# bdaiinstitute/vlfm

Hardware: AMD Instinct MI355X
Metric: env-steps/s (VLM+value-map update), 640x480 RGB-D (higher is better)
Workload: dtype f16 ViT-g (f32 accumulate) + f32 Q-Former (split-f16, 22-bit); f32 confidence + f64 value maps; 1 GPU; configs[1] step x resident envs: BLIP-2 ITC + ValueMap+ObstacleMap+sort_waypoints; envs_per_gpu=256, global_envs=256, map=1000x1000 @ 20 px/m, parallelism=env-sharded x1, tuned_gemms=True, vit_gemm=hip:fc1, attention=hip

## Files before the change

include/vlfm_amd.h:

```cpp
#ifndef VLFM_AMD_H
#define VLFM_AMD_H

#include <stddef.h>
#include <stdint.h>

#ifdef __cplusplus
extern "C" {
#endif

typedef enum {
    VLFM_OK = 0,
    VLFM_ERR_INVALID = -1,
    VLFM_ERR_OUTSIDE_MAP = -2,
    VLFM_ERR_INDEX = -3,
    VLFM_ERR_HIP = -4,
    VLFM_ERR_CAPACITY = -5
} vlfm_status;

enum { VLFM_FUSE_DEFAULT = 0, VLFM_FUSE_REPLACE = 1, VLFM_FUSE_EQUAL_WEIGHTING = 2 };

const char* vlfm_last_error(void);
int vlfm_abi_version(void);

int vlfm_profile_enable(int on);
int vlfm_profile_read(const char* kernel_name, double* mean_ms, int* launches);

int vlfm_host_wait_mode(int blocking);

typedef struct {
    double inv_affine[6];
    int32_t row0, col0;
    int32_t env;
    int32_t reserved;
} vlfm_vm_pose;

int vlfm_value_map_pose_params(const double* h_tf, const double* h_yaw, const int32_t* h_env, int n, int map_size,
                               int pixels_per_meter, int template_size, vlfm_vm_pose* h_out, int* bad_index);

int vlfm_cone_template_host(double fov, double max_depth, int pixels_per_meter, double min_confidence,
                            float* h_conf, int conf_capacity, int64_t* h_poly_xy, int poly_capacity,
                            int* n_poly);

int vlfm_tan_table_host(double fov, int width, double* h_out);

int vlfm_cone_template_build(const float* d_conf, const int64_t* d_poly_xy, int n_poly, int template_size,
                             float* d_template, uint32_t* d_template_bits, void* stream);

typedef struct {
    double tf[12];
    float depth_scale;
    float depth_offset;
    float depth_max;
    float reserved0;
    double fx, fy;
    double min_height, max_height;
    int32_t env;
    int32_t scatter;
} vlfm_ingest_params;

typedef struct {
    uint32_t* d_cells;
    int32_t* d_count;
    int32_t capacity;
    int32_t reserved;
} vlfm_scatter_journal;

int vlfm_depth_ingest_batched(const float* d_depth, int n, int height, int width,
                              const vlfm_ingest_params* d_params,
                              uint32_t* d_colmax_keys ,
                              uint32_t* d_obstacle , int map_size, int pixels_per_meter,
                              int32_t* d_status ,
                              uint32_t* d_hole_bits ,
                              const uint32_t* d_filled_bits ,
                              const vlfm_scatter_journal* journal ,
                              void* stream);

int vlfm_selftest_div_exact(const double* d_numerators, int n, double divisor, int32_t* d_mismatches, void* stream);

size_t vlfm_hole_scratch_bytes(int n, int height, int width, int cap_pts, int cap_contours);
int vlfm_fill_small_holes_batched(const uint32_t* d_hole_bits, const int32_t* d_status, int n, int height, int width,
                                  double area_thresh, void* d_scratch, size_t scratch_bytes, int cap_pts,
                                  int cap_contours, uint32_t* d_filled_bits, int32_t* d_counts,
                                  const vlfm_ingest_params* d_params, uint32_t* d_obstacle, int map_size,
                                  const vlfm_scatter_journal* journal, void* stream);
int vlfm_depth_scatter_holes_batched(const vlfm_ingest_params* d_params, int n, int height, int width,
                                     const uint32_t* d_hole_bits, const uint32_t* d_filled_bits,
                                     const int32_t* d_hole_counts ,
                                     uint32_t* d_obstacle, int map_size, int pixels_per_meter, int32_t* d_status,
                                     const float* d_depth ,
                                     void* stream);

int vlfm_fill_small_holes_rig_batched(const uint32_t* d_hole_bits, const int32_t* d_status, int n, int height, int width,
                                      double area_thresh, void* d_scratch, size_t scratch_bytes, int cap_pts,
                                      int cap_contours, uint32_t* d_filled_bits, int32_t* d_counts,
                                      const vlfm_ingest_params* d_params, uint32_t* d_obstacle, int map_size,
                                      const vlfm_scatter_journal* journal, int32_t* d_slot_undone, int n_envs, void* stream);
int vlfm_depth_scatter_holes_rig_batched(const vlfm_ingest_params* d_params, int n, int height, int width,
                                         const uint32_t* d_hole_bits, const uint32_t* d_filled_bits,
                                         const int32_t* d_hole_counts, uint32_t* d_obstacle, int map_size,
                                         int pixels_per_meter, int32_t* d_status, const float* d_depth,
                                         const int32_t* d_slot_undone, void* stream);

int vlfm_value_map_update_fused_batched(uint32_t* d_colmax_keys, int width, const double* d_tan,
                                        const float* d_template, const uint32_t* d_template_bits, int template_size,
                                        const vlfm_vm_pose* d_pose, const double* d_values, int n,
                                        float* d_conf, double* d_value, int map_size, int channels, int pixels_per_meter,
                                        double min_depth, double max_depth, int use_max_confidence, int fusion_type,
                                        const uint32_t* d_explored_bits, uint32_t* d_written_bits, int32_t* d_counters,
                                        const float* d_conf_quadrant, void* stream);

typedef struct {
    const float* d_template;
    const uint32_t* d_template_bits;
    const float* d_conf_quadrant;
    const double* d_tan;
    float depth_scale;
    float depth_offset;
    int32_t template_size;
    int32_t reserved;
} vlfm_vm_optics;

int vlfm_value_map_update_rig_batched(uint32_t* d_colmax_keys, int width, const vlfm_vm_pose* d_pose,
                                      const vlfm_vm_optics* d_optics, const int32_t* d_slots, int n_slots, int n,
                                      int max_template_size, const double* d_values, float* d_conf, double* d_value,
                                      int map_size, int channels, int pixels_per_meter, int use_max_confidence,
                                      int fusion_type, const uint32_t* d_explored_bits, uint32_t* d_written_bits,
                                      int32_t* d_counters, void* stream);

int vlfm_disc_rows_host(int radius, int32_t* h_halfwidth );
int vlfm_value_map_sort_waypoints_batched(const double* d_value, int map_size, int channels,
                                          const int32_t* d_cells, int m, int radius, const int32_t* d_disc,
                                          int value_is_f32, double* d_out, void* stream);



int vlfm_resample_coeffs_host(int in_size, int out_size, int32_t* h_bounds, int32_t* h_kk, int kk_capacity,
                              int* ksize_out);

int vlfm_resample_coeffs_filter_host(int in_size, int out_size, int filter, int32_t* h_bounds, int32_t* h_kk,
                                     int kk_capacity, int* ksize_out);

int vlfm_preprocess_sam_batched(const uint8_t* d_rgb, int n, int height, int width, int out_h, int out_w,
                                const int32_t* d_hbounds, const int32_t* d_hk, int hksize,
                                const int32_t* d_vbounds, const int32_t* d_vk, int vksize,
                                const float* h_mean3, const float* h_std3, int pad_size, uint8_t* d_tmp, float* d_out,
                                void* stream);

int vlfm_preprocess_rgb_batched(const uint8_t* d_rgb, int n, int height, int width, int out_size,
                                const int32_t* d_hbounds, const int32_t* d_hk, int hksize,
                                const int32_t* d_vbounds, const int32_t* d_vk, int vksize,
                                const float* h_mean3, const float* h_std3, uint8_t* d_tmp, void* d_out,
                                int out_dtype, int patch_size, void* stream);

int vlfm_itc_head_batched(const float* d_proj, int batch, int n_query, int proj_dim,
                          const float* d_text, float* d_out, void* stream);

#define VLFM_ITC_MAX_PROMPTS 8
int vlfm_itc_head_multi(const float* d_proj, int batch, int n_query, int proj_dim, const float* d_text_table, int n_text,
                        const int32_t* d_text_index, int n_prompts, float* d_out, void* stream);

int vlfm_layernorm_bias_f16(const void* d_x, const float* d_channel_bias, const void* d_gamma, const void* d_beta,
                            void* d_y, int rows, int dim, float eps, void* stream);

int vlfm_vit_attention_f16(const void* d_qkv, void* d_out, int batch, int tokens, int heads, int head_dim, float scale,
                           void* stream);

int vlfm_gemm_f16_nt(const void* d_x, const void* d_w, const void* d_bias, void* d_c, int m, int n, int k, int epilogue,
                     void* stream);

int vlfm_gemm_f16_pair_f32_nt(const void* d_x, const void* d_w_pair, const void* d_bias_f32, void* d_out, int m, int n_out, int k,
                              void* stream);

int vlfm_qformer_cross_attention_f32(const void* d_q, const void* d_kv_blocks, void* d_out, int batch, int tokens, int queries,
                                     int heads, int k_block0, int v_block0, int m_total, float scale, void* stream);

int vlfm_gemm_f16_tile_order(int m, int n, int group_m, int* out, int capacity_pairs);
int vlfm_gemm_f16_work_items(int m, int n, int grid, int* out, int capacity_pairs);

int vlfm_split_f32_to_f16_pair(const float* d_src, void* d_hi, void* d_lo, long long count, int* d_overflow, void* stream);
int vlfm_gemm_f32_nt(const float* d_x, const float* d_w, const float* d_bias, const float* d_residual, float* d_c, int m, int n,
                     int k, int activation, int precision, const void* d_w_hi, const void* d_w_lo, int* d_overflow, void* stream);


int vlfm_layernorm_rows_f32(const float* d_x, const float* d_gamma, const float* d_beta, float* d_out, int batch, int height,
                            int width, int channels, int window, float eps, void* stream);
int vlfm_window_reverse_add_f32(float* d_x, const float* d_windows, int batch, int height, int width, int channels, int window,
                                void* stream);
int vlfm_dwconv3x3_nhwc_f32(const float* d_x, const float* d_w9c, const float* d_bias, float* d_out, int batch, int height, int width,
                            int channels, void* stream);
int vlfm_window_attention_f32(const float* d_qkv, const float* d_bias_t, float* d_out, long long windows, int tokens, int heads,
                              float scale, void* stream);
int vlfm_layernorm_rows_shifted_f32(const float* d_x, const float* d_gamma, const float* d_beta, float* d_out, int batch, int height,
                                    int width, int channels, int window, float eps, int shift, int pad_zero, void* stream);
int vlfm_window_reverse_add_shifted_f32(float* d_x, const float* d_windows, int batch, int height, int width, int channels, int window,
                                        int shift, void* stream);
int vlfm_window_attention_masked_f32(const float* d_qkv, const float* d_bias_t, const float* d_mask_t, int windows_per_image, float* d_out,
                                     long long windows, int tokens, int heads, float scale, void* stream);

int vlfm_maxpool2x2_nhwc_f16(const void* d_x, void* d_out, int batch, int height, int width, int channels, void* stream);
int vlfm_conv_nhwc_tile(int pixels, int cin, int cout, int ksize, int* tile_pixels, int* tile_channels);
int vlfm_conv_nhwc_f16(const void* d_x, const void* d_w, const void* d_bias, void* d_out, const void* d_zero, int batch,
                       int height, int width, int cin, int cout, int ksize, int stride, int x_pix_stride,
                       int out_pix_stride, int act, void* stream);

int vlfm_resize_area_tab_host(int ssize, int dsize, int32_t* h_first, int32_t* h_count, float* h_w, int ktaps_capacity);

int vlfm_resize_area_batched(const uint8_t* d_rgb, int n, int height, int width, int out_h, int out_w,
                             const int32_t* d_xfirst, const int32_t* d_xcount, const float* d_xw, int xktaps,
                             const int32_t* d_yfirst, const int32_t* d_ycount, const float* d_yw, int yktaps,
                             void* d_out, int out_dtype, void* stream);

int vlfm_to_tensor_normalize_batched(const uint8_t* d_rgb, int n, int height, int width, const float* h_mean3,
                                     const float* h_std3, float* d_out, void* stream);

size_t vlfm_nms_scratch_bytes(int n);
int vlfm_nms(const float* d_boxes_xyxy, const int32_t* d_order, int n, float iou_threshold, void* d_scratch,
             size_t scratch_bytes, int32_t* d_keep, int32_t* d_num_keep, int max_keep, void* stream);

int vlfm_ms_deform_attn(const float* d_value, const int32_t* d_spatial_shapes, const int32_t* d_level_start,
                        const float* d_sampling_loc, const float* d_attn_weight, int batch, int n_query, int n_heads,
                        int head_dim, int n_levels, int n_points, int total_len, float* d_out, void* stream);
int vlfm_ms_deform_attn_fused(const float* d_value, const int32_t* d_spatial_shapes, const int32_t* d_level_start,
                              const float* d_offsets_logits, const float* d_reference, int batch, int n_query, int n_heads,
                              int head_dim, int n_levels, int n_points, int ref_coords, int total_len, float* d_out, void* stream);

int vlfm_dwconv3x3_f32(const float* d_x, const float* d_w, const float* d_bias, float* d_y, int n, int channels, int height,
                       int width, int stride, int gelu, void* stream);

int vlfm_bias_act_nchw(void* d_y, const void* d_bias, int n, int channels, long long hw, int dtype, int act, void* stream);


size_t vlfm_object_cloud_batch_scratch_bytes(int jobs, int height, int width);
int vlfm_object_cloud_batch_stats(const uint8_t* d_masks, const int32_t* d_erosion, int jobs, int max_erosion, int height, int width,
                                  void* d_scratch, int32_t* d_stats, void* stream);
int vlfm_object_cloud_batch_expand(const float* d_depth, int frames, int height, int width, double min_depth, double max_depth,
                                   double fx, double fy, const void* d_scratch, int scratch_jobs, const int32_t* d_jobs, int n_jobs,
                                   int max_points, const int32_t* d_ranks, int n_ranks, double* d_points, int capacity, void* stream);
size_t vlfm_dbscan_batch_scratch_bytes(int n);
int vlfm_dbscan_largest_cluster_batch(const double* d_points, int capacity, const int64_t* d_jobs, int n_jobs, int max_n, double eps,
                                      int min_points, void* d_scratch, size_t scratch_bytes, double* d_kept, int32_t* d_num_keep,
                                      void* stream);
long long vlfm_object_cloud_launch_count(void);


typedef struct {
    const double* d_rows;
    const int32_t* d_slots;
    double p[3];
    double heading, half_fov, range;
    int32_t n, k, flag_offset, n_slots;
} vlfm_cloud_query;

int vlfm_cloud_cone_flags(const vlfm_cloud_query* d_queries, int n_queries, int max_points, int32_t* d_flags, void* stream);

size_t vlfm_cloud_closest_scratch_bytes(int n_queries, int max_points);
int vlfm_cloud_closest(const vlfm_cloud_query* d_queries, int n_queries, int max_points, void* d_scratch, size_t scratch_bytes,
                       int32_t* d_result, void* stream);
int vlfm_cloud_query_chunk(void);
long long vlfm_cloud_query_launch_count(void);

int vlfm_bits_pack(const uint8_t* d_src, uint32_t* d_dst, int planes, int rows, int cols, void* stream);
int vlfm_bits_unpack(const uint32_t* d_src, uint8_t* d_dst, int planes, int rows, int cols, void* stream);

int vlfm_bits_dilate(const uint32_t* d_src, uint32_t* d_dst, int planes, int rows, int cols, int kernel_w,
                     int kernel_h, void* stream);

int vlfm_find_contours_external(const uint32_t* d_img, int planes, int rows, int cols, int method,
                                uint32_t* d_scratch , int32_t* d_pts, int cap_pts,
                                int32_t* d_starts, int32_t* d_lens, int cap_contours, int32_t* d_counts, void* stream);

size_t vlfm_find_contours_wg_scratch_bytes(int planes, int rows, int cols, int cap_pts);
int vlfm_walk_path_counters(long long* h_out4, int reset);
int vlfm_find_contours_external_wg(const uint32_t* d_img, int planes, int rows, int cols, int method, void* d_scratch,
                                   size_t scratch_bytes, int32_t* d_pts, int cap_pts, int32_t* d_starts, int32_t* d_lens,
                                   int cap_contours, int32_t* d_counts, void* stream);

#define VLFM_FOG_MAX_POLY 80
typedef struct {
    int32_t env;
    int32_t ax, ay;
    int32_t radius;
    int32_t n_poly;
    int32_t reserved;
    double rot_c, rot_s;
    double line_len;
    long long poly[2 * VLFM_FOG_MAX_POLY];
} vlfm_fog_params;

int vlfm_fog_params_host(const int32_t* h_agent_px, const double* h_angle_cv2_deg, const double* h_rot_cs,
                         double fov_deg, double max_line_len, const int32_t* h_env, const int32_t* h_explore, int n,
                         vlfm_fog_params* h_out);

size_t vlfm_obstacle_scratch_bytes(int n_envs, int map_size, int cap_pts, int cap_contours);

int vlfm_obstacle_map_update_batched(const vlfm_fog_params* d_prm, int n, const uint32_t* d_obstacle,
                                     uint32_t* d_navigable, uint32_t* d_explored, int32_t* d_bbox, int n_envs,
                                     int map_size, int kernel_size, int fog_radius, double area_thresh_px,
                                     void* d_scratch, size_t scratch_bytes, int cap_pts, int cap_contours,
                                     double* d_frontiers, int cap_frontiers, int32_t* d_counts, int update_obstacles,
                                     int explore, const int32_t* d_windows, int window_blocks_navigable,
                                     int window_blocks_prepare, void* stream);

int vlfm_obstacle_status(const void* d_scratch, int n_envs, int map_size, int cap_pts, int cap_contours,
                         int32_t* h_out);

enum { VLFM_REDUCE_MAX = 0,
       VLFM_REDUCE_EXPLORE = 1,
       VLFM_REDUCE_PLANE = 2 };
enum { VLFM_PRIM_CIRCLE_FILL = 0,
       VLFM_PRIM_CIRCLE = 1,
       VLFM_PRIM_LINE = 2,
       VLFM_PRIM_POLYLINE = 3 };
#define VLFM_RENDER_FLIP_ROWS 1
#define VLFM_RENDER_UNDER_PATH 2
typedef struct {
    int32_t frame;
    int32_t kind;
    int32_t flags;
    int32_t thickness;
    int32_t x0, y0, x1, y1;
    int32_t vtx_off, n_vtx;
    uint8_t bgr[4];
    int32_t reserved;
} vlfm_render_prim;

size_t vlfm_value_render_scratch_bytes(int n, int map_size);

int vlfm_value_map_render(const double* d_value, int n_envs, int map_size, int channels, const int32_t* d_frames, int n,
                          int reduce_mode, double explore_thresh, const double* d_plane, const uint32_t* d_explored,
                          const uint32_t* d_path, const int32_t* d_prim_off, const vlfm_render_prim* d_prims,
                          const int64_t* d_vtx, int rgb, void* d_scratch, size_t scratch_bytes, uint8_t* d_out,
                          void* stream);

int vlfm_obstacle_map_render(const uint32_t* d_obstacle, const uint32_t* d_navigable, const uint32_t* d_explored,
                             int n_envs, int map_size, const int32_t* d_frames, int n, uint32_t pad_bgr,
                             const uint32_t* d_path, const int32_t* d_prim_off, const vlfm_render_prim* d_prims,
                             const int64_t* d_vtx, int rgb, uint8_t* d_out, void* stream);

int vlfm_traj_append(uint32_t* d_path, int n_envs, int map_size, const int32_t* d_segs, int m, int thickness,
                     void* stream);

int vlfm_circle_polygon_host(const int32_t* h_circles, int n, int64_t* h_xy, int32_t* h_off, int capacity);

int vlfm_jpeg_quant_tables_host(int quality, uint16_t* h_tables);
size_t vlfm_jpeg_scratch_bytes(int n, int H, int W);
int vlfm_jpeg_roundtrip_batched(const uint8_t* d_in, uint8_t* d_out, int n, int H, int W, const uint16_t* h_tables,
                                void* d_scratch, size_t scratch_bytes, void* stream);

int vlfm_jpeg_header_host(int quality, int H, int W, uint8_t* h_out, size_t cap, size_t* len);
size_t vlfm_jpeg_encode_bound(int H, int W);
size_t vlfm_jpeg_encode_scratch_bytes(int n, int H, int W);
int vlfm_jpeg_encode_batched(const uint8_t* d_in, int n, int H, int W, int rgb_order, const uint16_t* h_tables,
                             uint8_t* d_out, size_t capacity, uint32_t* d_lengths, void* d_scratch, size_t scratch_bytes,
                             void* stream);

typedef struct vlfm_jpeg_huff {
    uint32_t limit[16];
    int32_t delta[16];
    uint8_t vals[256];
} vlfm_jpeg_huff;
typedef struct vlfm_jpeg_table_set {
    uint16_t quant[3][64];
    vlfm_jpeg_huff dc[3];
    vlfm_jpeg_huff ac[3];
} vlfm_jpeg_table_set;
typedef struct vlfm_jpeg_frame {
    int32_t height, width, restart_interval, scan_offset, table_set, reserved[3];
} vlfm_jpeg_frame;
enum {
    VLFM_JPEG_BAD_HEADER = 1,
    VLFM_JPEG_BAD_LENGTH = 2,
    VLFM_JPEG_BAD_EOI = 3,
    VLFM_JPEG_BAD_RESTART = 4,
    VLFM_JPEG_BAD_CODE = 5,
    VLFM_JPEG_BAD_SIZE = 6,
    VLFM_JPEG_BAD_INDEX = 7,
    VLFM_JPEG_BAD_BITS = 8
};
int vlfm_jpeg_parse_host(const uint8_t* h_file, size_t len, vlfm_jpeg_frame* frame, vlfm_jpeg_table_set* set);
const char* vlfm_jpeg_parse_reason(int code);
size_t vlfm_jpeg_decode_chunk_bytes(void);
size_t vlfm_jpeg_decode_scratch_bytes(int n, int H, int W, size_t max_file_bytes);
int vlfm_jpeg_decode_batched(const uint8_t* d_files, size_t files_bytes, const int64_t* d_offsets, size_t stride,
                             const int32_t* d_lengths, int n, int H, int W, const vlfm_jpeg_frame* d_frames,
                             const vlfm_jpeg_table_set* d_sets, int n_sets, const uint8_t* d_header, int header_bytes,
                             int max_segments, size_t max_file_bytes, int rgb_order, uint8_t* d_out, int32_t* d_status,
                             void* d_scratch, size_t scratch_bytes, void* stream);

int vlfm_worlds_raycast(const double* d_cameras, int n, const double* d_world_boxes, const int32_t* d_box_counts, int n_worlds,
                        int max_boxes, const int32_t* d_world_of, const double* d_objects, const int32_t* d_env_of, int n_envs,
                        int H, int W, float* d_depth, uint8_t* d_ids, int32_t* d_stats, const int32_t* d_object_colours,
                        const int32_t* d_palette, uint8_t* d_rgb, void* stream);

#define VLFM_GRID_MAX_CELLS 1024
int vlfm_worlds_raycast_grids(const double* d_cameras, int n, const double* d_world_boxes, const int32_t* d_box_counts,
                              int n_worlds, int max_boxes, const int32_t* d_world_of, const double* d_objects,
                              const int32_t* d_env_of, int n_envs, int H, int W, float* d_depth, uint8_t* d_ids, int32_t* d_stats,
                              const int32_t* d_object_colours, const int32_t* d_palette, uint8_t* d_rgb,
                              const uint32_t* d_grid_bits, const double* d_grid_edges, const int32_t* d_grid_dims, int max_nx,
                              int max_ny, void* stream);

int vlfm_geodesic_fields(const double* d_world_boxes, const int32_t* d_box_counts, int n_worlds, int max_boxes,
                         const int32_t* d_world_of, double margin, const double* d_objects, const double* d_sources,
                         const int32_t* d_source_counts, int n, int max_sources, double* d_rects, double* d_nodes,
                         double* d_dist, int32_t* d_counts, void* stream);
int vlfm_geodesic_query(const double* d_points, const int32_t* d_field_of, int m, int n_fields, int n_boxes,
                        const double* d_rects, const double* d_nodes, const double* d_dist, const int32_t* d_counts,
                        const double* d_sources, const int32_t* d_source_counts, int max_sources, double* d_out, void* stream);

enum { VLFM_PLAN_OK = 0, VLFM_PLAN_UNREACHABLE = 1, VLFM_PLAN_TOO_LONG = 2, VLFM_PLAN_INVALID = 3 };
enum { VLFM_PLAN_IN_LDS = 0, VLFM_PLAN_IN_SCRATCH = 1 };
typedef struct VlfmPlanJob {
    int32_t env, y0, y1, x0, x1;
    int32_t sx, sy, start_free;
    int32_t gx, gy, goal_free;
    int32_t reserved;
} VlfmPlanJob;
typedef struct VlfmPlanResult {
    int32_t status, cost, waypoint_x, waypoint_y, steps;
    int32_t reserved[3];
} VlfmPlanResult;
size_t vlfm_plan_scratch_bytes(int n_jobs, int size);
int vlfm_plan_paths(const int32_t* d_navigable, int n_envs, int size, const VlfmPlanJob* d_jobs, int n_jobs, int lookahead,
                    int max_cost, uint16_t* d_fields, int field_h, int field_w, VlfmPlanResult* d_results, void* d_scratch,
                    size_t scratch_bytes, void* stream);

#define VLFM_LATTICE_MAX_NODES 1024
enum { VLFM_LATTICE_IN_LDS = 0, VLFM_LATTICE_IN_SCRATCH = 1, VLFM_LATTICE_ALL_IN_SCRATCH = 2 };
int vlfm_lattice_free(const double* d_world_boxes, const int32_t* d_box_counts, int n_worlds, int max_boxes,
                      const uint32_t* d_grid_bits, const double* d_grid_edges, const int32_t* d_grid_dims, int max_nx, int max_ny,
                      const int32_t* d_world_of, double margin, const double* d_objects, const int32_t* d_dims, int n,
                      int cells_per_metre, int max_nb, int max_na, uint32_t* d_free, void* stream);
size_t vlfm_lattice_scratch_bytes(int n, int max_nb, int max_na);
int vlfm_lattice_fields(const uint32_t* d_free, const int32_t* d_dims, int n, int max_nb, int max_na, const int32_t* d_sources,
                        const int32_t* d_source_counts, int max_sources, int max_cost, uint16_t* d_dist, void* d_scratch,
                        size_t scratch_bytes, void* stream);
int vlfm_lattice_query(const double* d_points, const int32_t* d_field_of, int m, int n_fields, const uint16_t* d_dist,
                       const int32_t* d_dims, int max_nb, int max_na, int cells_per_metre, double* d_out, void* stream);

int vlfm_depth_sensor(const float* d_clean, float* d_out, int n, int H, int W, const uint32_t* d_keys, const float* d_range,
                      float sigma0_m, float sigma2_per_m, float disparity_k, uint32_t drop_threshold, uint32_t patch_threshold,
                      float edge_m, float min_range_m, float max_range_m, int32_t* d_invalid, int band_rows, void* stream);

#ifdef __cplusplus
}
#endif
#endif
```

vlfm_amd/_lib.py:

```python
from __future__ import annotations

import ctypes
import os
import subprocess
from typing import Optional

_HERE = os.path.dirname(os.path.abspath(__file__))
LIB_PATH = os.path.join(_HERE, "libvlfm_amd.so")
SOURCES = ["value_map.hip", "depth_ingest.hip", "depth_holes.hip", "obstacle_map.hip", "vlm_ops.hip", "vit_attention.hip", "qformer_attention.hip", "detect_ops.hip", "object_cloud.hip", "cloud_query.hip", "gemm_f16.hip", "gemm_f32.hip", "conv_nhwc.hip", "sam_ops.hip", "map_render.hip", "jpeg_codec.hip", "jpeg_entropy.hip", "jpeg_decode.hip", "world_render.hip", "depth_sensor.hip", "geodesic.hip", "map_planner.hip", "lattice_geodesic.hip", "host.cpp"]

VLFM_OK = 0
VLFM_ERR_INVALID = -1
VLFM_ERR_OUTSIDE_MAP = -2
VLFM_ERR_INDEX = -3
VLFM_ERR_HIP = -4
VLFM_ERR_CAPACITY = -5

FUSION_TYPES = {"default": 0, "replace": 1, "equal_weighting": 2}


class VmPose(ctypes.Structure):
    _fields_ = [("inv_affine", ctypes.c_double * 6), ("row0", ctypes.c_int32), ("col0", ctypes.c_int32),
                ("env", ctypes.c_int32), ("reserved", ctypes.c_int32)]


class IngestParams(ctypes.Structure):
    _fields_ = [("tf", ctypes.c_double * 12), ("depth_scale", ctypes.c_float), ("depth_offset", ctypes.c_float),
                ("depth_max", ctypes.c_float), ("reserved0", ctypes.c_float), ("fx", ctypes.c_double),
                ("fy", ctypes.c_double), ("min_height", ctypes.c_double), ("max_height", ctypes.c_double),
                ("env", ctypes.c_int32), ("scatter", ctypes.c_int32)]


FOG_MAX_POLY = 80


class FogParams(ctypes.Structure):
    _fields_ = [("env", ctypes.c_int32), ("ax", ctypes.c_int32), ("ay", ctypes.c_int32), ("radius", ctypes.c_int32),
                ("n_poly", ctypes.c_int32), ("reserved", ctypes.c_int32), ("rot_c", ctypes.c_double),
                ("rot_s", ctypes.c_double), ("line_len", ctypes.c_double), ("poly", ctypes.c_longlong * (2 * FOG_MAX_POLY))]


class ScatterJournal(ctypes.Structure):
    _fields_ = [("d_cells", ctypes.c_void_p), ("d_count", ctypes.c_void_p), ("capacity", ctypes.c_int32),
                ("reserved", ctypes.c_int32)]


class VmOptics(ctypes.Structure):
    _fields_ = [("d_template", ctypes.c_void_p), ("d_template_bits", ctypes.c_void_p), ("d_conf_quadrant", ctypes.c_void_p),
                ("d_tan", ctypes.c_void_p), ("depth_scale", ctypes.c_float), ("depth_offset", ctypes.c_float),
                ("template_size", ctypes.c_int32), ("reserved", ctypes.c_int32)]


class CloudQuery(ctypes.Structure):
    _fields_ = [("d_rows", ctypes.c_void_p), ("d_slots", ctypes.c_void_p), ("p", ctypes.c_double * 3),
                ("heading", ctypes.c_double), ("half_fov", ctypes.c_double), ("range", ctypes.c_double),
                ("n", ctypes.c_int32), ("k", ctypes.c_int32), ("flag_offset", ctypes.c_int32), ("n_slots", ctypes.c_int32)]


class PlanJob(ctypes.Structure):
    _fields_ = [("env", ctypes.c_int32), ("y0", ctypes.c_int32), ("y1", ctypes.c_int32), ("x0", ctypes.c_int32),
                ("x1", ctypes.c_int32), ("sx", ctypes.c_int32), ("sy", ctypes.c_int32), ("start_free", ctypes.c_int32),
                ("gx", ctypes.c_int32), ("gy", ctypes.c_int32), ("goal_free", ctypes.c_int32), ("reserved", ctypes.c_int32)]


class PlanResult(ctypes.Structure):
    _fields_ = [("status", ctypes.c_int32), ("cost", ctypes.c_int32), ("waypoint_x", ctypes.c_int32),
                ("waypoint_y", ctypes.c_int32), ("steps", ctypes.c_int32), ("reserved", ctypes.c_int32 * 3)]


PLAN_OK, PLAN_UNREACHABLE, PLAN_TOO_LONG, PLAN_INVALID = 0, 1, 2, 3
PLAN_IN_LDS, PLAN_IN_SCRATCH = 0, 1
LATTICE_IN_LDS, LATTICE_IN_SCRATCH, LATTICE_ALL_IN_SCRATCH = 0, 1, 2

assert ctypes.sizeof(PlanJob) == 48 and ctypes.sizeof(PlanResult) == 32
assert ctypes.sizeof(CloudQuery) == 80
assert ctypes.sizeof(ScatterJournal) == 24 and ctypes.sizeof(VmOptics) == 48
assert ctypes.sizeof(VmPose) == 64 and ctypes.sizeof(IngestParams) == 152 and ctypes.sizeof(FogParams) == 48 + 16 * FOG_MAX_POLY


def build(verbose: bool = False) -> str:
    from concurrent.futures import ThreadPoolExecutor

    csrc = os.path.join(_HERE, "csrc")
    srcs = [os.path.join(csrc, s) for s in SOURCES if os.path.exists(os.path.join(csrc, s))]
    hdrs = [os.path.join(csrc, h) for h in os.listdir(csrc) if h.endswith(".h")] + [
        os.path.join(_HERE, "..", "include", "vlfm_amd.h")]
    hdr_time = max(os.path.getmtime(h) for h in hdrs)
    objdir = os.path.join(csrc, "build")
    os.makedirs(objdir, exist_ok=True)
    flags = ["--offload-arch=gfx950", "-O3", "-std=c++17", "-fPIC", "-ffp-contract=off"]

    def compile_one(src: str) -> str:
        obj = os.path.join(objdir, os.path.basename(src) + ".o")
        if not os.path.exists(obj) or os.path.getmtime(obj) < max(os.path.getmtime(src), hdr_time):
            cmd = ["hipcc"] + flags + ["-c", src, "-o", obj]
            if verbose:
                print(" ".join(cmd), flush=True)
            subprocess.check_call(cmd)
        return obj

    with ThreadPoolExecutor(max_workers=min(8, len(srcs))) as pool:
        objs = list(pool.map(compile_one, srcs))
    if os.path.exists(LIB_PATH) and all(os.path.getmtime(LIB_PATH) >= os.path.getmtime(o) for o in objs):
        return LIB_PATH
    cmd = ["hipcc", "--offload-arch=gfx950", "-shared", "-fPIC", "-o", LIB_PATH] + objs
    if verbose:
        print(" ".join(cmd), flush=True)
    subprocess.check_call(cmd)
    return LIB_PATH


_lib: Optional[ctypes.CDLL] = None


def lib() -> ctypes.CDLL:
    global _lib
    if _lib is None:
        if not os.path.exists(LIB_PATH):
            raise ImportError(
                f"{LIB_PATH} is missing: build it with `python -c 'import __graft_entry__ as g; g.build()'` "
                "(hipcc --offload-arch=gfx950).  vlfm_amd has no CPU fallback.")
        L = ctypes.CDLL(LIB_PATH)
        vp, ci, cd = ctypes.c_void_p, ctypes.c_int, ctypes.c_double
        L.vlfm_last_error.restype = ctypes.c_char_p
        L.vlfm_abi_version.restype = ci
        L.vlfm_profile_enable.argtypes = [ci]
        L.vlfm_host_wait_mode.argtypes = [ci]
        L.vlfm_profile_read.argtypes = [ctypes.c_char_p, ctypes.POINTER(cd), ctypes.POINTER(ci)]
        L.vlfm_value_map_pose_params.argtypes = [vp, vp, vp, ci, ci, ci, ci, vp, ctypes.POINTER(ci)]
        L.vlfm_cone_template_host.argtypes = [cd, cd, ci, cd, vp, ci, vp, ci, ctypes.POINTER(ci)]
        L.vlfm_tan_table_host.argtypes = [cd, ci, vp]
        L.vlfm_disc_rows_host.argtypes = [ci, vp]
        L.vlfm_cone_template_build.argtypes = [vp, vp, ci, ci, vp, vp, vp]
        L.vlfm_depth_ingest_batched.argtypes = [vp, ci, ci, ci, vp, vp, vp, ci, ci, vp, vp, vp, vp, vp]
        L.vlfm_selftest_div_exact.argtypes = [vp, ci, cd, vp, vp]
        L.vlfm_hole_scratch_bytes.argtypes = [ci, ci, ci, ci, ci]
        L.vlfm_hole_scratch_bytes.restype = ctypes.c_size_t
        L.vlfm_fill_small_holes_batched.argtypes = [vp, vp, ci, ci, ci, cd, vp, ctypes.c_size_t, ci, ci, vp, vp, vp, vp,
                                                    ci, vp, vp]
        L.vlfm_depth_scatter_holes_batched.argtypes = [vp, ci, ci, ci, vp, vp, vp, vp, ci, ci, vp, vp, vp]
        L.vlfm_fill_small_holes_rig_batched.argtypes = [vp, vp, ci, ci, ci, cd, vp, ctypes.c_size_t, ci, ci, vp, vp, vp, vp,
                                                        ci, vp, vp, ci, vp]
        L.vlfm_depth_scatter_holes_rig_batched.argtypes = [vp, ci, ci, ci, vp, vp, vp, vp, ci, ci, vp, vp, vp, vp]
        L.vlfm_layernorm_bias_f16.argtypes = [vp, vp, vp, vp, vp, ci, ci, ctypes.c_float, vp]
        L.vlfm_vit_attention_f16.argtypes = [vp, vp, ci, ci, ci, ci, ctypes.c_float, vp]
        L.vlfm_gemm_f16_nt.argtypes = [vp, vp, vp, vp, ci, ci, ci, ci, vp]
        L.vlfm_gemm_f16_pair_f32_nt.argtypes = [vp, vp, vp, vp, ci, ci, ci, vp]
        L.vlfm_qformer_cross_attention_f32.argtypes = [vp, vp, vp, ci, ci, ci, ci, ci, ci, ci, ctypes.c_float, vp]
        L.vlfm_gemm_f32_nt.argtypes = [vp, vp, vp, vp, vp, ci, ci, ci, ci, ci, vp, vp, vp, vp]
        L.vlfm_split_f32_to_f16_pair.argtypes = [vp, vp, vp, ctypes.c_longlong, vp, vp]
        L.vlfm_layernorm_rows_f32.argtypes = [vp, vp, vp, vp, ci, ci, ci, ci, ci, ctypes.c_float, vp]
        L.vlfm_window_reverse_add_f32.argtypes = [vp, vp, ci, ci, ci, ci, ci, vp]
        L.vlfm_dwconv3x3_nhwc_f32.argtypes = [vp, vp, vp, vp, ci, ci, ci, ci, vp]
        L.vlfm_window_attention_f32.argtypes = [vp, vp, vp, ctypes.c_longlong, ci, ci, ctypes.c_float, vp]
        L.vlfm_layernorm_rows_shifted_f32.argtypes = [vp, vp, vp, vp, ci, ci, ci, ci, ci, ctypes.c_float, ci, ci, vp]
        L.vlfm_window_reverse_add_shifted_f32.argtypes = [vp, vp, ci, ci, ci, ci, ci, ci, vp]
        L.vlfm_window_attention_masked_f32.argtypes = [vp, vp, vp, ci, vp, ctypes.c_longlong, ci, ci, ctypes.c_float, vp]
        L.vlfm_maxpool2x2_nhwc_f16.argtypes = [vp, vp, ci, ci, ci, ci, vp]
        L.vlfm_conv_nhwc_tile.argtypes = [ci, ci, ci, ci, ctypes.POINTER(ci), ctypes.POINTER(ci)]
        L.vlfm_conv_nhwc_f16.argtypes = [vp, vp, vp, vp, vp, ci, ci, ci, ci, ci, ci, ci, ci, ci, ci, vp]
        L.vlfm_value_map_update_fused_batched.argtypes = [vp, ci, vp, vp, vp, ci, vp, vp, ci, vp, vp, ci, ci, ci, cd, cd,
                                                          ci, ci, vp, vp, vp, vp, vp]
        L.vlfm_value_map_update_rig_batched.argtypes = [vp, ci, vp, vp, vp, ci, ci, ci, vp, vp, vp, ci, ci, ci, ci, ci, vp, vp,
                                                        vp, vp]
        L.vlfm_value_map_sort_waypoints_batched.argtypes = [vp, ci, ci, vp, ci, ci, vp, ci, vp, vp]
        L.vlfm_resample_coeffs_host.argtypes = [ci, ci, vp, vp, ci, ctypes.POINTER(ci)]
        L.vlfm_resample_coeffs_filter_host.argtypes = [ci, ci, ci, vp, vp, ci, ctypes.POINTER(ci)]
        L.vlfm_preprocess_sam_batched.argtypes = [vp, ci, ci, ci, ci, ci, vp, vp, ci, vp, vp, ci, vp, vp, ci, vp, vp, vp]
        L.vlfm_preprocess_rgb_batched.argtypes = [vp, ci, ci, ci, ci, vp, vp, ci, vp, vp, ci, vp, vp, vp, vp, ci, ci, vp]
        L.vlfm_itc_head_batched.argtypes = [vp, ci, ci, ci, vp, vp, vp]
        L.vlfm_itc_head_multi.argtypes = [vp, ci, ci, ci, vp, ci, vp, ci, vp, vp]
        cf = ctypes.c_float
        L.vlfm_resize_area_tab_host.argtypes = [ci, ci, vp, vp, vp, ci]
        L.vlfm_resize_area_batched.argtypes = [vp, ci, ci, ci, ci, ci, vp, vp, vp, ci, vp, vp, vp, ci, vp, ci, vp]
        L.vlfm_to_tensor_normalize_batched.argtypes = [vp, ci, ci, ci, vp, vp, vp, vp]
        L.vlfm_nms_scratch_bytes.argtypes = [ci]
        L.vlfm_nms_scratch_bytes.restype = ctypes.c_size_t
        L.vlfm_nms.argtypes = [vp, vp, ci, cf, vp, ctypes.c_size_t, vp, vp, ci, vp]
        L.vlfm_ms_deform_attn.argtypes = [vp, vp, vp, vp, vp, ci, ci, ci, ci, ci, ci, ci, vp, vp]
        L.vlfm_ms_deform_attn_fused.argtypes = [vp, vp, vp, vp, vp, ci, ci, ci, ci, ci, ci, ci, ci, vp, vp]
        L.vlfm_object_cloud_batch_scratch_bytes.argtypes = [ci, ci, ci]
        L.vlfm_object_cloud_batch_scratch_bytes.restype = ctypes.c_size_t
        L.vlfm_object_cloud_batch_stats.argtypes = [vp, vp, ci, ci, ci, ci, vp, vp, vp]
        L.vlfm_object_cloud_batch_expand.argtypes = [vp, ci, ci, ci, cd, cd, cd, cd, vp, ci, vp, ci, ci, vp, ci, vp, ci, vp]
        L.vlfm_dbscan_batch_scratch_bytes.argtypes = [ci]
        L.vlfm_dbscan_batch_scratch_bytes.restype = ctypes.c_size_t
        L.vlfm_dbscan_largest_cluster_batch.argtypes = [vp, ci, vp, ci, ci, cd, ci, vp, ctypes.c_size_t, vp, vp, vp]
        L.vlfm_object_cloud_launch_count.argtypes = []
        L.vlfm_object_cloud_launch_count.restype = ctypes.c_longlong
        L.vlfm_cloud_cone_flags.argtypes = [vp, ci, ci, vp, vp]
        L.vlfm_cloud_closest_scratch_bytes.argtypes = [ci, ci]
        L.vlfm_cloud_closest_scratch_bytes.restype = ctypes.c_size_t
        L.vlfm_cloud_closest.argtypes = [vp, ci, ci, vp, ctypes.c_size_t, vp, vp]
        L.vlfm_cloud_query_chunk.argtypes = []
        L.vlfm_cloud_query_launch_count.argtypes = []
        L.vlfm_cloud_query_launch_count.restype = ctypes.c_longlong
        L.vlfm_bits_pack.argtypes = [vp, vp, ci, ci, ci, vp]
        L.vlfm_bits_unpack.argtypes = [vp, vp, ci, ci, ci, vp]
        L.vlfm_bits_dilate.argtypes = [vp, vp, ci, ci, ci, ci, ci, vp]
        L.vlfm_find_contours_external.argtypes = [vp, ci, ci, ci, ci, vp, vp, ci, vp, vp, ci, vp, vp]
        L.vlfm_dwconv3x3_f32.argtypes = [vp, vp, vp, vp, ci, ci, ci, ci, ci, ci, vp]
        L.vlfm_bias_act_nchw.argtypes = [vp, vp, ci, ci, ctypes.c_longlong, ci, ci, vp]
        L.vlfm_find_contours_wg_scratch_bytes.argtypes = [ci, ci, ci, ci]
        L.vlfm_find_contours_wg_scratch_bytes.restype = ctypes.c_size_t
        L.vlfm_find_contours_external_wg.argtypes = [vp, ci, ci, ci, ci, vp, ctypes.c_size_t, vp, ci, vp, vp, ci, vp, vp]
        L.vlfm_walk_path_counters.argtypes = [vp, ci]
        L.vlfm_fog_params_host.argtypes = [vp, vp, vp, cd, cd, vp, vp, ci, vp]
        L.vlfm_obstacle_scratch_bytes.argtypes = [ci, ci, ci, ci]
        L.vlfm_obstacle_scratch_bytes.restype = ctypes.c_size_t
        L.vlfm_obstacle_map_update_batched.argtypes = [vp, ci, vp, vp, vp, vp, ci, ci, ci, ci, cd, vp, ctypes.c_size_t,
                                                       ci, ci, vp, ci, vp, ci, ci, vp, ci, ci, vp]
        L.vlfm_obstacle_status.argtypes = [vp, ci, ci, ci, ci, vp]
        L.vlfm_value_render_scratch_bytes.argtypes = [ci, ci]
        L.vlfm_value_render_scratch_bytes.restype = ctypes.c_size_t
        L.vlfm_value_map_render.argtypes = [vp, ci, ci, ci, vp, ci, ci, cd, vp, vp, vp, vp, vp, vp, ci, vp,
                                            ctypes.c_size_t, vp, vp]
        L.vlfm_obstacle_map_render.argtypes = [vp, vp, vp, ci, ci, vp, ci, ctypes.c_uint32, vp, vp, vp, vp, ci, vp, vp]
        L.vlfm_traj_append.argtypes = [vp, ci, ci, vp, ci, ci, vp]
        L.vlfm_circle_polygon_host.argtypes = [vp, ci, vp, vp, ci]
        L.vlfm_jpeg_quant_tables_host.argtypes = [ci, vp]
        L.vlfm_jpeg_scratch_bytes.argtypes = [ci, ci, ci]
        L.vlfm_jpeg_scratch_bytes.restype = ctypes.c_size_t
        L.vlfm_jpeg_roundtrip_batched.argtypes = [vp, vp, ci, ci, ci, vp, vp, ctypes.c_size_t, vp]
        L.vlfm_jpeg_header_host.argtypes = [ci, ci, ci, vp, ctypes.c_size_t, ctypes.POINTER(ctypes.c_size_t)]
        L.vlfm_jpeg_encode_bound.argtypes = [ci, ci]
        L.vlfm_jpeg_encode_bound.restype = ctypes.c_size_t
        L.vlfm_jpeg_encode_scratch_bytes.argtypes = [ci, ci, ci]
        L.vlfm_jpeg_encode_scratch_bytes.restype = ctypes.c_size_t
        L.vlfm_jpeg_encode_batched.argtypes = [vp, ci, ci, ci, ci, vp, vp, ctypes.c_size_t, vp, vp, ctypes.c_size_t, vp]
        L.vlfm_jpeg_parse_host.argtypes = [vp, ctypes.c_size_t, vp, vp]
        L.vlfm_jpeg_parse_reason.argtypes = [ci]
        L.vlfm_jpeg_parse_reason.restype = ctypes.c_char_p
        L.vlfm_jpeg_decode_chunk_bytes.restype = ctypes.c_size_t
        L.vlfm_jpeg_decode_scratch_bytes.argtypes = [ci, ci, ci, ctypes.c_size_t]
        L.vlfm_jpeg_decode_scratch_bytes.restype = ctypes.c_size_t
        L.vlfm_jpeg_decode_batched.argtypes = [vp, ctypes.c_size_t, vp, ctypes.c_size_t, vp, ci, ci, ci, vp, vp, ci, vp, ci, ci,
                                               ctypes.c_size_t, ci, vp, vp, vp, ctypes.c_size_t, vp]
        L.vlfm_worlds_raycast.argtypes = [vp, ci, vp, vp, ci, ci, vp, vp, vp, ci, ci, ci, vp, vp, vp, vp, vp, vp, vp]
        L.vlfm_worlds_raycast_grids.argtypes = L.vlfm_worlds_raycast.argtypes[:-1] + [vp, vp, vp, ci, ci, vp]
        L.vlfm_geodesic_fields.argtypes = [vp, vp, ci, ci, vp, cd, vp, vp, vp, ci, ci, vp, vp, vp, vp, vp]
        L.vlfm_geodesic_query.argtypes = [vp, vp, ci, ci, ci, vp, vp, vp, vp, vp, vp, ci, vp, vp]
        L.vlfm_plan_scratch_bytes.argtypes = [ci, ci]
        L.vlfm_plan_scratch_bytes.restype = ctypes.c_size_t
        L.vlfm_plan_paths.argtypes = [vp, ci, ci, vp, ci, ci, ci, vp, ci, ci, vp, vp, ctypes.c_size_t, vp]
        L.vlfm_lattice_free.argtypes = [vp, vp, ci, ci, vp, vp, vp, ci, ci, vp, cd, vp, vp, ci, ci, ci, ci, vp, vp]
        L.vlfm_lattice_scratch_bytes.argtypes = [ci, ci, ci]
        L.vlfm_lattice_scratch_bytes.restype = ctypes.c_size_t
        L.vlfm_lattice_fields.argtypes = [vp, vp, ci, ci, ci, vp, vp, ci, ci, vp, vp, ctypes.c_size_t, vp]
        L.vlfm_lattice_query.argtypes = [vp, vp, ci, ci, vp, vp, ci, ci, ci, vp, vp]
        u32 = ctypes.c_uint32
        L.vlfm_depth_sensor.argtypes = [vp, vp, ci, ci, ci, vp, vp, cf, cf, cf, u32, u32, cf, cf, cf, vp, ci, vp]
        _lib = L
    return _lib


def profile_read(kernel: str):
    ms, n = ctypes.c_double(0.0), ctypes.c_int(0)
    lib().vlfm_profile_read(kernel.encode(), ctypes.byref(ms), ctypes.byref(n))
    return ms.value, n.value


def last_error() -> str:
    return lib().vlfm_last_error().decode()


def host_wait_blocking(device=None, blocking: bool = True) -> None:
    import torch

    with torch.cuda.device(device if device is not None else torch.cuda.current_device()):
        check(lib().vlfm_host_wait_mode(int(bool(blocking))), "host_wait_mode")


def try_host_wait_blocking(device=None) -> bool:
    import os
    import warnings

    if os.environ.get("VLFM_HOST_WAIT", "blocking") == "spin":
        return False
    try:
        host_wait_blocking(device)
        return True
    except Exception as exc:
        warnings.warn(f"blocking host waits not enabled on {device}: {exc} (call vlfm_amd._lib.host_wait_blocking before the "
                      f"device's first allocation; waits will spin on a host core)")
        return False


def check(rc: int, what: str = "") -> int:
    if rc >= 0:
        return rc
    msg = last_error()
    if rc == VLFM_ERR_OUTSIDE_MAP:
        raise AssertionError(msg or "Pixel location is outside the image.")
    if rc == VLFM_ERR_INDEX:
        raise IndexError(msg or "index out of bounds for obstacle map")
    raise RuntimeError(f"libvlfm_amd {what} failed ({rc}): {msg}")
```

vlfm_amd/csrc/host.cpp:

```cpp
#include <cmath>
#include <cstdint>
#include <cstring>
#include <mutex>
#include <string>

#include "../../include/vlfm_amd.h"
#include "status.h"

namespace vlfm {
static thread_local std::string g_last_error;
void set_last_error(const char* msg) { g_last_error = msg ? msg : ""; }
}

extern "C" const char* vlfm_last_error(void) { return vlfm::g_last_error.c_str(); }
extern "C" int vlfm_abi_version(void) { return 27; }

namespace {

const double kPi = 3.141592653589793238462643383279502884;

inline long round_half_even(double v) { return std::lrint(v); }

float sin_deg_table(int deg) {
    static float tab[451];
    static std::once_flag once;
    std::call_once(once, [] {
        for (int i = 0; i <= 450; i++) tab[i] = (float)(std::round(std::sin(i * kPi / 180.0) * 1e7) / 1e7);
    });
    return tab[deg];
}

}

extern "C" int vlfm_value_map_pose_params(const double* h_tf, const double* h_yaw, const int32_t* h_env, int n,
                                          int map_size, int pixels_per_meter, int template_size,
                                          vlfm_vm_pose* h_out, int* bad_index) {
    if (!h_tf || !h_out || n < 0 || map_size <= 0 || template_size <= 0)
        return vlfm::fail(VLFM_ERR_INVALID, "value_map_pose_params: bad argument");
    const double ppm = (double)pixels_per_meter;
    const int half = template_size / 2;
    for (int k = 0; k < n; k++) {
        const double* tf = h_tf + 16 * k;
        const double yaw = h_yaw ? h_yaw[k] : std::atan2(tf[4], tf[0]);
        const double degrees = (-yaw) * (180.0 / kPi);
        const double ang = degrees * (kPi / 180);
        const double alpha = std::cos(ang), beta = std::sin(ang);
        const double cx = (double)(float)half, cy = (double)(float)half;
        double M[6] = {alpha, beta, (1 - alpha) * cx - beta * cy, -beta, alpha, beta * cx + (1 - alpha) * cy};
        double D = M[0] * M[4] - M[1] * M[3];
        D = D != 0 ? 1. / D : 0;
        const double A11 = M[4] * D, A22 = M[0] * D;
        M[0] = A11; M[1] *= -D;
        M[3] *= -D; M[4] = A22;
        const double b1 = -M[0] * M[2] - M[1] * M[5];
        const double b2 = -M[3] * M[2] - M[4] * M[5];
        M[2] = b1; M[5] = b2;
        vlfm_vm_pose& p = h_out[k];
        std::memcpy(p.inv_affine, M, sizeof(M));
        const double cam_x = tf[3] / tf[15], cam_y = tf[7] / tf[15];
        const long px = (long)(cam_x * ppm) + map_size / 2;
        const long py = (long)(-cam_y * ppm) + map_size / 2;
        if (px < 0 || px >= map_size || py < 0 || py >= map_size) {
            if (bad_index) *bad_index = k;
            return vlfm::fail(VLFM_ERR_OUTSIDE_MAP, "Pixel location is outside the image.");
        }
        p.row0 = (int32_t)(px - half);
        p.col0 = (int32_t)(py - half);
        p.env = h_env ? h_env[k] : k;
        p.reserved = 0;
    }
    return VLFM_OK;
}

static int ellipse_sector_polygon(int cx, int cy, int radius, double start_angle, double end_angle, int64_t* out_xy,
                                  int capacity) {
    int a0 = (int)round_half_even(start_angle), a1 = (int)round_half_even(end_angle);
    const bool full = (a1 - a0) >= 360;
    if (a0 > a1) { int t = a0; a0 = a1; a1 = t; }
    while (a0 < 0) { a0 += 360; a1 += 360; }
    while (a1 > 360) { a1 -= 360; a0 -= 360; }
    if (a1 - a0 > 360) { a0 = 0; a1 = 360; }
    const int step = radius < 3 ? 90 : radius < 10 ? 30 : radius < 15 ? 18 : 5;
    const double ccx = (double)((int64_t)cx << 16), ccy = (double)((int64_t)cy << 16);
    const double axis = (double)((int64_t)radius << 16);
    int m = 0;
    int64_t last_x = -1, last_y = -1;
    for (int a = a0; a < a1 + step; a += step) {
        int t = a > a1 ? a1 : a;
        if (t < 0) t += 360;
        const double ex = axis * sin_deg_table(450 - t), ey = axis * sin_deg_table(t);
        const double vx = ccx + ex * sin_deg_table(90) - ey * sin_deg_table(0);
        const double vy = ccy + ex * sin_deg_table(0) + ey * sin_deg_table(90);
        int64_t qx = (int64_t)round_half_even(vx / 65536.0) << 16, qy = (int64_t)round_half_even(vy / 65536.0) << 16;
        qx += round_half_even(vx - (double)qx);
        qy += round_half_even(vy - (double)qy);
        if (qx == last_x && qy == last_y) continue;
        if (m >= capacity) return VLFM_ERR_CAPACITY;
        out_xy[2 * m] = qx; out_xy[2 * m + 1] = qy; m++;
        last_x = qx; last_y = qy;
    }
    if (!full) {
        if (m >= capacity) return VLFM_ERR_CAPACITY;
        out_xy[2 * m] = (int64_t)cx << 16; out_xy[2 * m + 1] = (int64_t)cy << 16; m++;
    }
    return m;
}

extern "C" int vlfm_fog_params_host(const int32_t* h_agent_px, const double* h_angle_cv2_deg, const double* h_rot_cs,
                                    double fov_deg, double max_line_len, const int32_t* h_env,
                                    const int32_t* h_explore, int n, vlfm_fog_params* h_out) {
    if (!h_agent_px || !h_angle_cv2_deg || !h_rot_cs || !h_out || n < 0)
        return vlfm::fail(VLFM_ERR_INVALID, "fog_params_host: bad argument");
    for (int k = 0; k < n; k++) {
        vlfm_fog_params& p = h_out[k];
        std::memset(&p, 0, sizeof(p));
        p.env = h_env ? h_env[k] : k;
        p.ax = h_agent_px[2 * k]; p.ay = h_agent_px[2 * k + 1];
        p.radius = (int)max_line_len;
        p.rot_c = h_rot_cs[2 * k]; p.rot_s = h_rot_cs[2 * k + 1];
        p.line_len = max_line_len * 1.05;
        if (h_explore && !h_explore[k]) { p.n_poly = 0; continue; }
        const int m = ellipse_sector_polygon(p.ax, p.ay, p.radius, h_angle_cv2_deg[k] - fov_deg / 2,
                                             h_angle_cv2_deg[k] + fov_deg / 2, (int64_t*)p.poly, VLFM_FOG_MAX_POLY);
        if (m < 0) return vlfm::fail(m, "fog_params_host: sector polygon does not fit VLFM_FOG_MAX_POLY");
        p.n_poly = m;
    }
    return VLFM_OK;
}

extern "C" int vlfm_circle_polygon_host(const int32_t* h_circles, int n, int64_t* h_xy, int32_t* h_off, int capacity) {
    if (!h_circles || !h_xy || !h_off || n < 0 || capacity < 0)
        return vlfm::fail(VLFM_ERR_INVALID, "circle_polygon_host: bad argument");
    int total = 0;
    h_off[0] = 0;
    for (int k = 0; k < n; k++) {
        const int cx = h_circles[3 * k], cy = h_circles[3 * k + 1], r = h_circles[3 * k + 2];
        if (r < 0) return vlfm::fail(VLFM_ERR_INVALID, "circle_polygon_host: negative radius");
        const int m = ellipse_sector_polygon(cx, cy, r, 0.0, 360.0, h_xy + 2 * (size_t)total, capacity - total);
        if (m < 0) return vlfm::fail(m, "circle_polygon_host: vertex capacity");
        if (m == 1) {
            if (total + 2 > capacity) return vlfm::fail(VLFM_ERR_CAPACITY, "circle_polygon_host: vertex capacity");
            for (int i = 0; i < 2; i++) {
                h_xy[2 * (size_t)(total + i)] = (int64_t)cx << 16;
                h_xy[2 * (size_t)(total + i) + 1] = (int64_t)cy << 16;
            }
            total += 2;
        } else {
            total += m;
        }
        h_off[k + 1] = total;
    }
    return total;
}

extern "C" int vlfm_cone_template_host(double fov, double max_depth, int pixels_per_meter, double min_confidence,
                                       float* h_conf, int conf_capacity, int64_t* h_poly_xy, int poly_capacity,
                                       int* n_poly) {
    if (!h_conf || !h_poly_xy || !n_poly || pixels_per_meter <= 0)
        return vlfm::fail(VLFM_ERR_INVALID, "cone_template_host: bad argument");
    const int size = (int)(max_depth * pixels_per_meter);
    const int T = 2 * size + 1;
    if (size <= 0) return vlfm::fail(VLFM_ERR_INVALID, "cone_template_host: empty template");
    if ((long)T * T > conf_capacity) return vlfm::fail(VLFM_ERR_CAPACITY, "cone_template_host: conf capacity");
    const int mid = T / 2;
    for (int r = 0; r < T; r++) {
        const double fwd = std::abs(r - mid);
        for (int c = 0; c < T; c++) {
            const double lat = std::abs(c - mid);
            double ang = std::atan2(lat, fwd);
            ang = (ang - 0) * (kPi / 2 - 0) / (fov / 2 - 0) + 0;
            double cf = std::pow(std::cos(ang), 2.0);
            cf = (cf - 0) * (1 - min_confidence) / (1 - 0) + min_confidence;
            h_conf[(size_t)r * T + c] = (float)cf;
        }
    }
    const double deg = fov * (180.0 / kPi);
    const int m = ellipse_sector_polygon(size, size, size, -deg / 2 + 90, deg / 2 + 90, h_poly_xy, poly_capacity);
    if (m < 0) return vlfm::fail(m, "cone_template_host: polygon capacity");
    *n_poly = m;
    return T;
}

extern "C" int vlfm_tan_table_host(double fov, int width, double* h_out) {
    if (!h_out || width <= 0) return vlfm::fail(VLFM_ERR_INVALID, "tan_table_host: bad argument");
    const double start = -fov / 2, stop = fov / 2;
    const int div = width - 1;
    const double step = div > 0 ? (stop - start) / div : 0.0;
    for (int i = 0; i < width; i++) {
        double a = (double)i * step + start;
        if (i == width - 1 && width > 1) a = stop;
        h_out[i] = std::tan(a);
    }
    return VLFM_OK;
}

extern "C" int vlfm_disc_rows_host(int radius, int32_t* h_halfwidth) {
    if (!h_halfwidth || radius < 0) return vlfm::fail(VLFM_ERR_INVALID, "disc_rows_host: bad argument");
    for (int i = 0; i <= 2 * radius; i++) h_halfwidth[i] = -1;
    int err = 0, dx = radius, dy = 0, plus = 1, minus = (radius << 1) - 1;
    while (dx >= dy) {
        auto widen = [&](int row_off, int hw) {
            int32_t& slot = h_halfwidth[radius + row_off];
            if (hw > slot) slot = hw;
        };
        widen(-dy, dx); widen(dy, dx); widen(-dx, dy); widen(dx, dy);
        dy++;
        err += plus;
        plus += 2;
        const int mask = (err <= 0) - 1;
        err -= minus & mask;
        dx += mask;
        minus -= 2 & mask;
    }
    return VLFM_OK;
}

#include <hip/hip_runtime.h>

#include <map>
#include <vector>

#include "profile.h"

namespace vlfm {
namespace {
struct KernelLog { std::vector<std::pair<hipEvent_t, hipEvent_t>> spans; long launches = 0; };
std::mutex g_prof_mu;
int g_prof_every = 0;
std::map<std::string, KernelLog> g_prof;
const size_t kMaxSpans = 8192;
}

static thread_local ProfileScope* g_scope = nullptr;
ProfileScope* current_profile_scope() { return g_scope; }

ProfileScope::ProfileScope(const char* name, hipStream_t stream) : name_(name), stream_(stream) {
    prev_ = g_scope;
    g_scope = this;
    if (!g_prof_every) return;
    if (g_prof_every > 1) {
        std::lock_guard<std::mutex> lk(g_prof_mu);
        if (g_prof[name_].launches++ % g_prof_every != 0) return;
    }
    if (hipEventCreate(&start_) != hipSuccess || hipEventCreate(&stop_) != hipSuccess) return;
    active_ = true;
}
ProfileScope::~ProfileScope() {
    g_scope = prev_;
    if (!active_) return;
    if (!used_) { (void)hipEventDestroy(start_); (void)hipEventDestroy(stop_); return; }
    std::lock_guard<std::mutex> lk(g_prof_mu);
    KernelLog& log = g_prof[name_];
    if (log.spans.size() < kMaxSpans) log.spans.emplace_back(start_, stop_);
    else { (void)hipEventDestroy(start_); (void)hipEventDestroy(stop_); }
}
}

extern "C" int vlfm_host_wait_mode(int blocking) {
    hipError_t e = hipSetDeviceFlags(blocking ? hipDeviceScheduleBlockingSync : hipDeviceScheduleAuto);
    if (e != hipSuccess) {
        (void)hipGetLastError();
        vlfm::set_last_error((std::string("hipSetDeviceFlags: ") + hipGetErrorString(e)).c_str());
        return VLFM_ERR_HIP;
    }
    return VLFM_OK;
}

extern "C" int vlfm_profile_enable(int on) {
    std::lock_guard<std::mutex> lk(vlfm::g_prof_mu);
    for (auto& kv : vlfm::g_prof)
        for (auto& sp : kv.second.spans) { (void)hipEventDestroy(sp.first); (void)hipEventDestroy(sp.second); }
    vlfm::g_prof.clear();
    vlfm::g_prof_every = on > 0 ? on : 0;
    return VLFM_OK;
}

extern "C" int vlfm_profile_read(const char* kernel_name, double* mean_ms, int* launches) {
    if (!kernel_name || !mean_ms || !launches) return vlfm::fail(VLFM_ERR_INVALID, "profile_read: bad argument");
    std::lock_guard<std::mutex> lk(vlfm::g_prof_mu);
    auto it = vlfm::g_prof.find(kernel_name);
    *mean_ms = 0.0; *launches = 0;
    if (it == vlfm::g_prof.end()) return VLFM_OK;
    double total = 0.0; int n = 0;
    for (auto& sp : it->second.spans) {
        if (hipEventSynchronize(sp.second) != hipSuccess) continue;
        float ms = 0.f;
        if (hipEventElapsedTime(&ms, sp.first, sp.second) == hipSuccess) { total += ms; n++; }
    }
    *launches = n;
    *mean_ms = n ? total / n : 0.0;
    return VLFM_OK;
}
```

vlfm_amd/csrc/qformer_attention.hip:

```cpp
#include <hip/hip_runtime.h>
#include <stdint.h>

#include "../../include/vlfm_amd.h"
#include "mfma.h"
#include "profile.h"
#include "status.h"

namespace vlfm {

constexpr int QA_ROWB = 256;
constexpr int QA_MERGE_REGS = 34;
constexpr int QA_MERGE = 3 * QA_MERGE_REGS * 64 * 4;
constexpr int QA_MAX_T = 257, QA_MAX_Q = 32;

struct QaArgs {
    const float* q;
    const float* kv;
    float* out;
    int B, T, Q, heads, k_block0, v_block0, M_total;
    int rows_pad;
    float scale_log2e;
};

struct QaKernel {
    const QaArgs& a;
    unsigned char* smem;
    lds_ptr lds;
    int lane, wave, col, g, voff;

    __device__ QaKernel(const QaArgs& a_, unsigned char* smem_) : a(a_), smem(smem_), lds((lds_ptr)smem_) {
        lane = threadIdx.x & 63;
        wave = __builtin_amdgcn_readfirstlane(threadIdx.x >> 6);
        col = lane & 31;
        g = lane >> 5;
        voff = a.rows_pad * QA_ROWB;
    }
    __device__ inline const unsigned char* block(int block0, int b, int h) const {
        return reinterpret_cast<const unsigned char*>(a.kv + ((size_t)(block0 + h) * (size_t)a.M_total + (size_t)b * (size_t)a.T) * 64);
    }
    __device__ inline void issue_k(const unsigned char* kg, int row0, int n_ins) const {
        const int r4 = lane >> 4, p = lane & 15;
        for (int ins = 0; ins < n_ins; ins++) {
            const int row = row0 + 4 * ins + r4, src_row = min(row, a.T - 1);
            const int dst = __builtin_amdgcn_readfirstlane((row0 + 4 * ins) * QA_ROWB);
            __builtin_amdgcn_global_load_lds((gbl_ptr)(kg + (size_t)src_row * QA_ROWB + ((p ^ (row & 15)) << 4)), lds + dst, 16, 0, 0);
        }
    }
    __device__ inline void issue_v(const unsigned char* vg, int row0, int n_ins) const {
        const int r4 = lane >> 4, p = lane & 15;
        for (int ins = 0; ins < n_ins; ins++) {
            const int row = row0 + 4 * ins + r4, src_row = min(row, a.T - 1);
            const int dst = __builtin_amdgcn_readfirstlane(voff + (row0 + 4 * ins) * QA_ROWB);
            __builtin_amdgcn_global_load_lds((gbl_ptr)(vg + (size_t)src_row * QA_ROWB + ((p ^ (((row >> 2) & 1) << 3)) << 4)),
                                             lds + dst, 16, 0, 0);
        }
    }
    __device__ inline void issue_rows(const unsigned char* kg, const unsigned char* vg, int row0, int n_ins) const {
        issue_k(kg, row0, n_ins);
        issue_v(vg, row0, n_ins);
    }
    __device__ inline void load_q(int b, int h, float (&qn)[32]) const {
        const float* src = a.q + ((size_t)b * a.Q + min(col, a.Q - 1)) * ((size_t)a.heads * 64) + (size_t)h * 64 + 32 * g;
#pragma unroll
        for (int c = 0; c < 8; c++) {
            const floatx4 v = *reinterpret_cast<const floatx4*>(src + 4 * c);
            qn[4 * c] = v[0]; qn[4 * c + 1] = v[1]; qn[4 * c + 2] = v[2]; qn[4 * c + 3] = v[3];
        }
    }
};

__device__ __forceinline__ void qa_item(int w, int heads, int& b, int& h) {
    const int xcd = w & 7, idx = w >> 3;
    b = (idx / heads) * 8 + xcd;
    h = idx % heads;
}

__global__ __launch_bounds__(256) void qformer_cross_attention_kernel(QaArgs a) {
    extern __shared__ __attribute__((aligned(16))) unsigned char smem[];
    QaKernel k(a, smem);
    const int lane = k.lane, wave = k.wave, col = k.col, g = k.g;
    const int n_full = a.T >> 5, n_left = a.T & 31, left_wave = n_full & 3, left_ins = (n_left + 3) >> 2;
    const int stride = gridDim.x;
    const int moff = 2 * k.voff;
    int w = blockIdx.x, b, h;
    qa_item(w, a.heads, b, h);
    if (b >= a.B) return;

    float qn[32];
    k.load_q(b, h, qn);
    {
        const unsigned char* kg = k.block(a.k_block0, b, h);
        const unsigned char* vg = k.block(a.v_block0, b, h);
        for (int t = wave; t < n_full; t += 4) k.issue_rows(kg, vg, 32 * t, 8);
        if (n_left != 0 && wave == left_wave) k.issue_rows(kg, vg, 32 * n_full, left_ins);
    }
    for (;;) {
        wait_vmcnt<0>();
        asm volatile("" ::: "memory");
        float qf[32];
#pragma unroll
        for (int s = 0; s < 32; s++) qf[s] = qn[s];
        const int nw = w + stride;
        int nb, nh;
        qa_item(nw, a.heads, nb, nh);
        const bool more = nb < a.B;
        const unsigned char* kg = k.block(a.k_block0, more ? nb : b, more ? nh : h);
        const unsigned char* vg = k.block(a.v_block0, more ? nb : b, more ? nh : h);
        if (more) k.load_q(nb, nh, qn);

        float m = -INFINITY, l = 0.f;
        floatx16 o0, o1;
#pragma unroll
        for (int r = 0; r < 16; r++) { o0[r] = 0.f; o1[r] = 0.f; }
        for (int t = wave; t < n_full; t += 4) {
            const unsigned char* kb = smem + (32 * t + col) * QA_ROWB;
            float kf[32];
#pragma unroll
            for (int c = 0; c < 8; c++) {
                const floatx4 v = *reinterpret_cast<const floatx4*>(kb + (((8 * g + c) ^ (col & 15)) << 4));
                kf[4 * c] = v[0]; kf[4 * c + 1] = v[1]; kf[4 * c + 2] = v[2]; kf[4 * c + 3] = v[3];
            }
            wait_lgkmcnt0();
            __builtin_amdgcn_sched_barrier(0);
            asm volatile("" ::: "memory");
            if (more) k.issue_k(kg, 32 * t, 8);
            floatx16 acc;
#pragma unroll
            for (int r = 0; r < 16; r++) acc[r] = 0.f;
#pragma unroll
            for (int s = 0; s < 32; s++) acc = __builtin_amdgcn_mfma_f32_32x32x2f32(kf[s], qf[s], acc, 0, 0, 0);
#pragma unroll
            for (int r = 0; r < 16; r++) acc[r] *= a.scale_log2e;
            float tm = acc[0];
#pragma unroll
            for (int r = 1; r < 16; r++) tm = fmaxf(tm, acc[r]);
            tm = fmaxf(tm, __shfl_xor(tm, 32, 64));
            const float mn = fmaxf(m, tm);
            const float alpha = __builtin_amdgcn_exp2f(m - mn);
            m = mn;
            l *= alpha;
#pragma unroll
            for (int r = 0; r < 16; r++) { o0[r] *= alpha; o1[r] *= alpha; }
#pragma unroll
            for (int r = 0; r < 16; r++) { const float pj = __builtin_amdgcn_exp2f(acc[r] - mn); l += pj; acc[r] = pj; }
            const float* vb = reinterpret_cast<const float*>(smem + k.voff + (32 * t + 4 * g) * QA_ROWB);
            const int c0 = (((col >> 2) ^ (8 * g)) << 2) + (col & 3), c1 = (((8 + (col >> 2)) ^ (8 * g)) << 2) + (col & 3);
#pragma unroll
            for (int r = 0; r < 16; r++) {
                const int ro = ((r & 3) + 8 * (r >> 2)) * 64;
                o0 = __builtin_amdgcn_mfma_f32_32x32x2f32(vb[ro + c0], acc[r], o0, 0, 0, 0);
                o1 = __builtin_amdgcn_mfma_f32_32x32x2f32(vb[ro + c1], acc[r], o1, 0, 0, 0);
            }
            wait_lgkmcnt0();
            __builtin_amdgcn_sched_barrier(0);
            asm volatile("" ::: "memory");
            if (more) k.issue_v(vg, 32 * t, 8);
        }
        if (n_left != 0 && wave == left_wave) {
            for (int j = 32 * n_full; j < a.T; j++) {
                const unsigned char* kr = smem + j * QA_ROWB;
                float part = 0.f;
#pragma unroll
                for (int c = 0; c < 8; c++) {
                    const floatx4 v = *reinterpret_cast<const floatx4*>(kr + (((8 * g + c) ^ (j & 15)) << 4));
#pragma unroll
                    for (int e = 0; e < 4; e++) part = fmaf(v[e], qf[4 * c + e], part);
                }
                const float s = (part + __shfl_xor(part, 32, 64)) * a.scale_log2e;
                const float mn = fmaxf(m, s);
                const float alpha = __builtin_amdgcn_exp2f(m - mn), pj = __builtin_amdgcn_exp2f(s - mn);
                m = mn;
                l = l * alpha + (g == 0 ? pj : 0.f);
                const unsigned char* vr = smem + k.voff + j * QA_ROWB;
                const int sw = ((j >> 2) & 1) << 3;
#pragma unroll
                for (int q4 = 0; q4 < 4; q4++) {
                    const floatx4 v0 = *reinterpret_cast<const floatx4*>(vr + (((2 * q4 + g) ^ sw) << 4));
                    const floatx4 v1 = *reinterpret_cast<const floatx4*>(vr + (((8 + 2 * q4 + g) ^ sw) << 4));
#pragma unroll
                    for (int e = 0; e < 4; e++) {
                        o0[4 * q4 + e] = fmaf(pj, v0[e], o0[4 * q4 + e] * alpha);
                        o1[4 * q4 + e] = fmaf(pj, v1[e], o1[4 * q4 + e] * alpha);
                    }
                }
            }
            wait_lgkmcnt0();
            __builtin_amdgcn_sched_barrier(0);
            asm volatile("" ::: "memory");
            if (more) k.issue_rows(kg, vg, 32 * n_full, left_ins);
        }
        l += __shfl_xor(l, 32, 64);

        float* sc = reinterpret_cast<float*>(smem + moff);
        if (wave != 0) {
            float* mine = sc + (wave - 1) * QA_MERGE_REGS * 64 + lane;
#pragma unroll
            for (int r = 0; r < 16; r++) { mine[r * 64] = o0[r]; mine[(16 + r) * 64] = o1[r]; }
            mine[32 * 64] = m;
            mine[33 * 64] = l;
            wait_lgkmcnt0();
        }
        asm volatile("" ::: "memory");
        __builtin_amdgcn_s_barrier();
        asm volatile("" ::: "memory");
        if (wave == 0) {
#pragma unroll
            for (int v = 0; v < 3; v++) {
                const float* src = sc + v * QA_MERGE_REGS * 64 + lane;
                const float m2 = src[32 * 64], l2 = src[33 * 64];
                const float mn = fmaxf(m, m2);
                const float a1 = __builtin_amdgcn_exp2f(m - mn), a2 = __builtin_amdgcn_exp2f(m2 - mn);
                m = mn;
                l = l * a1 + l2 * a2;
#pragma unroll
                for (int r = 0; r < 16; r++) {
                    o0[r] = o0[r] * a1 + src[r * 64] * a2;
                    o1[r] = o1[r] * a1 + src[(16 + r) * 64] * a2;
                }
            }
            if (col < a.Q) {
                const float inv = 1.0f / l;
                float* orow = a.out + ((size_t)b * a.Q + col) * ((size_t)a.heads * 64) + (size_t)h * 64 + 4 * g;
#pragma unroll
                for (int q4 = 0; q4 < 4; q4++) {
                    const floatx4 s0 = {o0[4 * q4] * inv, o0[4 * q4 + 1] * inv, o0[4 * q4 + 2] * inv, o0[4 * q4 + 3] * inv};
                    const floatx4 s1 = {o1[4 * q4] * inv, o1[4 * q4 + 1] * inv, o1[4 * q4 + 2] * inv, o1[4 * q4 + 3] * inv};
                    *reinterpret_cast<floatx4*>(orow + 8 * q4) = s0;
                    *reinterpret_cast<floatx4*>(orow + 32 + 8 * q4) = s1;
                }
            }
            wait_lgkmcnt0();
        }
        asm volatile("" ::: "memory");
        __builtin_amdgcn_s_barrier();
        asm volatile("" ::: "memory");
        if (!more) break;
        w = nw; b = nb; h = nh;
    }
}

}

using namespace vlfm;

extern "C" int vlfm_qformer_cross_attention_f32(const void* d_q, const void* d_kv_blocks, void* d_out, int batch, int tokens,
                                                int queries, int heads, int k_block0, int v_block0, int m_total, float scale,
                                                void* stream) {
    if (batch == 0) return VLFM_OK;
    if (!d_q || !d_kv_blocks || !d_out || batch < 0 || tokens < 1 || tokens > QA_MAX_T || queries < 1 || queries > QA_MAX_Q || heads < 1 ||
        k_block0 < 0 || v_block0 < 0 || (long long)batch * tokens > (long long)m_total)
        return fail(VLFM_ERR_INVALID, "qformer_cross_attention_f32: head width 64, 1-32 queries, 1-257 tokens, batch * tokens <= m_total");
    if ((((uintptr_t)d_q | (uintptr_t)d_kv_blocks | (uintptr_t)d_out) & 15) != 0)
        return fail(VLFM_ERR_INVALID, "qformer_cross_attention_f32: pointers must be 16-byte aligned");
    QaArgs a;
    a.q = (const float*)d_q; a.kv = (const float*)d_kv_blocks; a.out = (float*)d_out;
    a.B = batch; a.T = tokens; a.Q = queries; a.heads = heads; a.k_block0 = k_block0; a.v_block0 = v_block0; a.M_total = m_total;
    a.rows_pad = (tokens + 3) & ~3;
    a.scale_log2e = scale * 1.4426950408889634f;
    const size_t lds = 2 * (size_t)a.rows_pad * QA_ROWB + QA_MERGE;
    const void* fn = reinterpret_cast<const void*>(qformer_cross_attention_kernel);
    static LdsOptIn opt;
    if (!opt.ensure(fn, lds)) return fail(VLFM_ERR_HIP, "qformer_cross_attention_f32: cannot opt in to the LDS size");
    const long long items = (long long)((batch + 7) / 8) * 8 * heads;
    const int n_cu = device_cu_count() & ~7;
    const dim3 grid((unsigned)(items < n_cu ? items : n_cu)), block(256);
    VLFM_TIMED("qformer_cross_attention_kernel", stream);
    VLFM_KLAUNCH(qformer_cross_attention_kernel, grid, block, lds, stream, a);
    return check_launch("qformer_cross_attention_kernel");
}
```

vlfm_amd/csrc/vlm_ops.hip:

```cpp
#include <hip/hip_fp16.h>
#include <hip/hip_bf16.h>
#include <hip/hip_runtime.h>
#include <stdint.h>

#include <cmath>
#include <cstdlib>
#include <vector>

#include "../../include/vlfm_amd.h"
#include "profile.h"
#include "status.h"

namespace vlfm {

constexpr int PRECISION_BITS = 32 - 8 - 2;

__device__ inline unsigned char clip8(int v) {
    v >>= PRECISION_BITS;
    return (unsigned char)(v < 0 ? 0 : v > 255 ? 255 : v);
}

__global__ __launch_bounds__(256) void resample_h_kernel(const unsigned char* __restrict__ src, int H, int W, int O,
                                                         const int* __restrict__ bounds, const int* __restrict__ kk,
                                                         int ksize, unsigned char* __restrict__ dst) {
    extern __shared__ __attribute__((aligned(16))) unsigned char smem[];
    const int y = blockIdx.x, n = blockIdx.y;
    const unsigned char* row = src + ((size_t)n * H + y) * W * 3;
    const int row_bytes = W * 3;
    if ((row_bytes & 15) == 0 && ((size_t)row & 15) == 0) {
        for (int i = threadIdx.x; i < row_bytes / 16; i += blockDim.x)
            reinterpret_cast<uint4*>(smem)[i] = reinterpret_cast<const uint4*>(row)[i];
    } else {
        for (int i = threadIdx.x; i < row_bytes; i += blockDim.x) smem[i] = row[i];
    }
    __syncthreads();
    unsigned char* out = dst + ((size_t)n * H + y) * O * 3;
    for (int o = threadIdx.x; o < O * 3; o += blockDim.x) {
        const int xx = o / 3, c = o - xx * 3;
        const int xmin = bounds[2 * xx], cnt = bounds[2 * xx + 1];
        const int* k = kk + xx * ksize;
        int ss = 1 << (PRECISION_BITS - 1);
        for (int x = 0; x < cnt; x++) ss += (int)smem[(xmin + x) * 3 + c] * k[x];
        out[o] = clip8(ss);
    }
}

template <typename OutT>
__device__ inline OutT cast_out(float v);
template <> __device__ inline float cast_out<float>(float v) { return v; }
template <> __device__ inline __half cast_out<__half>(float v) { return __float2half_rn(v); }
template <> __device__ inline __hip_bfloat16 cast_out<__hip_bfloat16>(float v) { return __float2bfloat16(v); }

struct Norm3 { float mean[3]; float std[3]; };

template <typename OutT>
__global__ __launch_bounds__(256) void resample_v_norm_kernel(const unsigned char* __restrict__ src, int H, int O,
                                                              const int* __restrict__ bounds,
                                                              const int* __restrict__ kk, int ksize, Norm3 nrm,
                                                              OutT* __restrict__ dst, int patch) {
    const int yy = blockIdx.x, n = blockIdx.y;
    const int ymin = bounds[2 * yy], cnt = bounds[2 * yy + 1];
    const int* k = kk + yy * ksize;
    const unsigned char* img = src + (size_t)n * H * O * 3;
    for (int o = threadIdx.x; o < 3 * O; o += blockDim.x) {
        const int c = o / O, xx = o - c * O;
        int ss = 1 << (PRECISION_BITS - 1);
        for (int y = 0; y < cnt; y++) ss += (int)img[((size_t)(ymin + y) * O + xx) * 3 + c] * k[y];
        const float px = (float)clip8(ss);
        const float v = __fdiv_rn(__fsub_rn(__fdiv_rn(px, 255.0f), nrm.mean[c]), nrm.std[c]);
        if (patch == 0) {
            dst[(((size_t)n * 3 + c) * O + yy) * O + xx] = cast_out<OutT>(v);
        } else {
            const int g = O / patch, py = yy / patch, px_ = xx / patch;
            const size_t cell = ((size_t)n * g * g + (size_t)py * g + px_) * (3 * patch * patch);
            dst[cell + (size_t)c * patch * patch + (yy - py * patch) * patch + (xx - px_ * patch)] = cast_out<OutT>(v);
        }
    }
}

constexpr int PF_THREADS = 768;
constexpr int PF_GROUPS = PF_THREADS / 256;
constexpr int PF_VGROUP = 192;
constexpr int PF_ROW_BYTES = 4096 + 128;

template <typename OutT> struct alignas(2 * sizeof(OutT)) Pair { OutT a, b; };

template <int KS, typename OutT>
__global__ __launch_bounds__(PF_THREADS) void preprocess_fused_kernel(const unsigned char* __restrict__ src, int H, int W, int O, int R,
                                                                      int TR, const int* __restrict__ hbounds,
                                                                      const int* __restrict__ hk, int hksize,
                                                                      const int* __restrict__ vbounds,
                                                                      const int* __restrict__ vk, int vksize, Norm3 nrm,
                                                                      OutT* __restrict__ dst, int patch) {
    extern __shared__ __attribute__((aligned(16))) unsigned char smem[];
    const int OP = (O + 3) & ~3;
    float* lut = reinterpret_cast<float*>(smem);
    unsigned char* rowbuf = smem + 3 * 256 * 4;
    unsigned char* tmp = rowbuf + 2 * PF_GROUPS * PF_ROW_BYTES;
    const int tid = threadIdx.x, n = blockIdx.y;
    const int yy0 = blockIdx.x * R, yy1 = min(O, yy0 + R);
    const int r0 = vbounds[2 * yy0], r1 = vbounds[2 * (yy1 - 1)] + vbounds[2 * (yy1 - 1) + 1];
    if (r1 - r0 > TR) __builtin_trap();
    {
        const int c = tid >> 8, v = tid & 255;
        lut[tid] = __fdiv_rn(__fsub_rn(__fdiv_rn((float)v, 255.0f), nrm.mean[c]), nrm.std[c]);
    }
    const int g = tid >> 8, xx = tid & 255;
    const bool live = xx < O;
    int k[KS];
    int d0 = 0, b0 = 0;
    if (live) {
        const int xmin = hbounds[2 * xx];
        d0 = (xmin * 3) >> 2;
        b0 = (xmin * 3) & 3;
    }
#pragma unroll
    for (int x = 0; x < KS; x++) k[x] = (live && x < hksize) ? hk[xx * hksize + x] : 0;
    const int row_bytes = W * 3;
    const unsigned char* img = src + (size_t)n * H * row_bytes;
    const int steps = (r1 - r0 + PF_GROUPS - 1) / PF_GROUPS;
    const bool loader = xx * 16 < row_bytes;
    uint4 pre = make_uint4(0u, 0u, 0u, 0u);
    if (loader && r0 + g < r1) pre = *reinterpret_cast<const uint4*>(img + (size_t)(r0 + g) * row_bytes + xx * 16);
    if (loader) *reinterpret_cast<uint4*>(rowbuf + (size_t)g * PF_ROW_BYTES + xx * 16) = pre;
    for (int st = 0; st < steps; st++) {
        const int r = r0 + st * PF_GROUPS + g, rn = r + PF_GROUPS;
        if (loader && rn < r1) pre = *reinterpret_cast<const uint4*>(img + (size_t)rn * row_bytes + xx * 16);
        __syncthreads();
        if (live && r < r1) {
            const unsigned* rowdw = reinterpret_cast<const unsigned*>(rowbuf + (size_t)((st & 1) * PF_GROUPS + g) * PF_ROW_BYTES);
            constexpr int NA = (3 * KS + 3) / 4;
            unsigned w[NA + 1], a[NA];
#pragma unroll
            for (int i = 0; i <= NA; i++) w[i] = rowdw[d0 + i];
#pragma unroll
            for (int i = 0; i < NA; i++) a[i] = __builtin_amdgcn_alignbyte(w[i + 1], w[i], (unsigned)b0);
            int s0 = 1 << (PRECISION_BITS - 1), s1 = s0, s2 = s0;
#pragma unroll
            for (int x = 0; x < KS; x++) {
                const int j = 3 * x;
                s0 = __mul24((int)((a[j >> 2] >> (8 * (j & 3))) & 0xFFu), k[x]) + s0;
                s1 = __mul24((int)((a[(j + 1) >> 2] >> (8 * ((j + 1) & 3))) & 0xFFu), k[x]) + s1;
                s2 = __mul24((int)((a[(j + 2) >> 2] >> (8 * ((j + 2) & 3))) & 0xFFu), k[x]) + s2;
            }
            unsigned char* t = tmp + (size_t)(r - r0) * OP + xx;
            t[0] = clip8(s0);
            t[(size_t)TR * OP] = clip8(s1);
            t[(size_t)2 * TR * OP] = clip8(s2);
        }
        if (loader) *reinterpret_cast<uint4*>(rowbuf + (size_t)(((st + 1) & 1) * PF_GROUPS + g) * PF_ROW_BYTES + xx * 16) = pre;
    }
    __syncthreads();
    const int vg = tid / PF_VGROUP, vt = tid - vg * PF_VGROUP;
    const int opd = OP >> 2;
    const bool vlive = vt < 3 * opd;
    const bool pair_ok = (O & 1) == 0 && (patch & 1) == 0;
    const int c = vlive ? vt / opd : 0, dc = vt - c * opd, x4 = 4 * dc;
    const int cell = 3 * patch * patch, gp = patch ? O / patch : 0;
    int coloff[4];
#pragma unroll
    for (int i = 0; i < 4; i++) {
        const int x = x4 + i;
        coloff[i] = patch ? (x / patch) * cell + (x % patch) : x;
    }
    const int chan_off = c * (patch ? patch * patch : O * O);
    const unsigned* col0 = reinterpret_cast<const unsigned*>(tmp) + (size_t)c * TR * opd + dc;
    const float* lut_c = lut + c * 256;
    for (int yy = yy0 + vg; yy < yy1; yy += PF_THREADS / PF_VGROUP) {
        const int yu = __builtin_amdgcn_readfirstlane(yy);
        const int ymin = vbounds[2 * yu], cnt = vbounds[2 * yu + 1];
        const int* kv = vk + (size_t)yu * vksize;
        size_t row_off;
        if (patch == 0) {
            row_off = ((size_t)n * 3 * O + yu) * O;
        } else {
            const int py = yu / patch;
            row_off = ((size_t)n * gp * gp + (size_t)py * gp) * cell + (size_t)(yu - py * patch) * patch;
        }
        if (!vlive) continue;
        const unsigned* col = col0 + (size_t)(ymin - r0) * opd;
        int s[4];
#pragma unroll
        for (int i = 0; i < 4; i++) s[i] = 1 << (PRECISION_BITS - 1);
        for (int y = 0; y < cnt; y++) {
            const unsigned wv = col[(size_t)y * opd];
            const int kq = kv[y];
            s[0] = __mul24((int)(wv & 0xFFu), kq) + s[0];
            s[1] = __mul24((int)((wv >> 8) & 0xFFu), kq) + s[1];
            s[2] = __mul24((int)((wv >> 16) & 0xFFu), kq) + s[2];
            s[3] = __mul24((int)(wv >> 24), kq) + s[3];
        }
        OutT v[4];
#pragma unroll
        for (int i = 0; i < 4; i++) v[i] = cast_out<OutT>(lut_c[clip8(s[i])]);
        OutT* o = dst + row_off + chan_off;
        if (pair_ok && x4 + 3 < O) {
            *reinterpret_cast<Pair<OutT>*>(o + coloff[0]) = Pair<OutT>{v[0], v[1]};
            *reinterpret_cast<Pair<OutT>*>(o + coloff[2]) = Pair<OutT>{v[2], v[3]};
        } else {
#pragma unroll
            for (int i = 0; i < 4; i++)
                if (x4 + i < O) o[coloff[i]] = v[i];
        }
    }
}

__global__ __launch_bounds__(256) void resample_v_sam_kernel(const unsigned char* __restrict__ src, int H, int OH, int OW,
                                                             int P, const int* __restrict__ bounds,
                                                             const int* __restrict__ kk, int ksize, Norm3 nrm,
                                                             float* __restrict__ dst) {
    const int yy = blockIdx.x, n = blockIdx.y;
    const unsigned char* img = src + (size_t)n * H * OW * 3;
    const bool row_in = yy < OH;
    const int ymin = row_in ? bounds[2 * yy] : 0, cnt = row_in ? bounds[2 * yy + 1] : 0;
    const int* k = kk + (size_t)(row_in ? yy : 0) * ksize;
    for (int o = threadIdx.x; o < 3 * P; o += blockDim.x) {
        const int c = o / P, xx = o - c * P;
        float v = 0.0f;
        if (row_in && xx < OW) {
            int ss = 1 << (PRECISION_BITS - 1);
            for (int y = 0; y < cnt; y++) ss += (int)img[((size_t)(ymin + y) * OW + xx) * 3 + c] * k[y];
            v = __fdiv_rn(__fsub_rn((float)clip8(ss), nrm.mean[c]), nrm.std[c]);
        }
        dst[(((size_t)n * 3 + c) * P + yy) * P + xx] = v;
    }
}

constexpr int LN_MAXV = 4;
constexpr int LN_ROWS = 8;

struct alignas(16) Half8 { __half2 h[4]; };

template <int NV>
__global__ __launch_bounds__(256) void layernorm_bias_f16_kernel(const __half* __restrict__ x, const float* __restrict__ cb,
                                                                 const __half* __restrict__ gamma,
                                                                 const __half* __restrict__ beta, __half* __restrict__ y,
                                                                 int rows, int D, float eps, int rows_per_wave) {
    const int lane = threadIdx.x & 63, wave = (blockIdx.x * blockDim.x + threadIdx.x) >> 6;
    const int nvec = D >> 3;
    const int r0 = wave * rows_per_wave;
    if (r0 >= rows) return;
    Half8 gm[NV], bt[NV];
    float4 c0[NV], c1[NV];
#pragma unroll
    for (int i = 0; i < NV; i++) {
        const int v = lane + 64 * i;
        if (v < nvec) {
            gm[i] = reinterpret_cast<const Half8*>(gamma)[v];
            bt[i] = reinterpret_cast<const Half8*>(beta)[v];
            c0[i] = cb ? reinterpret_cast<const float4*>(cb)[2 * v] : make_float4(0.f, 0.f, 0.f, 0.f);
            c1[i] = cb ? reinterpret_cast<const float4*>(cb)[2 * v + 1] : make_float4(0.f, 0.f, 0.f, 0.f);
        }
    }
    Half8 cur[NV], nxt[NV], nx2[NV];
    auto load_row = [&](int r, Half8* dst) {
#pragma unroll
        for (int i = 0; i < NV; i++) {
            const int v = lane + 64 * i;
            if (v < nvec) dst[i] = reinterpret_cast<const Half8*>(x + (size_t)r * D)[v];
        }
    };
    auto val = [&](const Half8* row, int i, int j) -> float {
        const float2 t = __half22float2(row[i].h[j >> 1]);
        const float cc = j < 4 ? (&c0[i].x)[j] : (&c1[i].x)[j - 4];
        return ((j & 1) ? t.y : t.x) + cc;
    };
    const int r_end = min(rows, r0 + rows_per_wave);
    load_row(r0, cur);
    if (r0 + 1 < r_end) load_row(r0 + 1, nxt);
    const float inv_d = 1.0f / (float)D;
    for (int r = r0; r < r_end; r++) {
        if (r + 2 < r_end) load_row(r + 2, nx2);
        float sum = 0.0f;
#pragma unroll
        for (int i = 0; i < NV; i++) {
            if (lane + 64 * i < nvec) {
#pragma unroll
                for (int j = 0; j < 8; j++) sum += val(cur, i, j);
            }
        }
#pragma unroll
        for (int off = 32; off > 0; off >>= 1) sum += __shfl_xor(sum, off, 64);
        const float mean = sum * inv_d;
        float sq = 0.0f;
#pragma unroll
        for (int i = 0; i < NV; i++) {
            if (lane + 64 * i < nvec) {
#pragma unroll
                for (int j = 0; j < 8; j++) {
                    const float dlt = val(cur, i, j) - mean;
                    sq = fmaf(dlt, dlt, sq);
                }
            }
        }
#pragma unroll
        for (int off = 32; off > 0; off >>= 1) sq += __shfl_xor(sq, off, 64);
        const float rstd = rsqrtf(sq * inv_d + eps);
#pragma unroll
        for (int i = 0; i < NV; i++) {
            const int v = lane + 64 * i;
            if (v < nvec) {
                Half8 o;
#pragma unroll
                for (int j = 0; j < 4; j++) {
                    const float2 g2 = __half22float2(gm[i].h[j]), b2 = __half22float2(bt[i].h[j]);
                    o.h[j] = __floats2half2_rn((val(cur, i, 2 * j) - mean) * rstd * g2.x + b2.x,
                                               (val(cur, i, 2 * j + 1) - mean) * rstd * g2.y + b2.y);
                }
                reinterpret_cast<Half8*>(y + (size_t)r * D)[v] = o;
            }
        }
#pragma unroll
        for (int i = 0; i < NV; i++) { cur[i] = nxt[i]; nxt[i] = nx2[i]; }
    }
}

__global__ __launch_bounds__(512) void itc_head_kernel(const float* __restrict__ proj, int NQ, int P,
                                                       const float* __restrict__ text, float* __restrict__ out) {
    __shared__ float cos_q[64];
    const int b = blockIdx.x, lane = threadIdx.x & 63, wave = threadIdx.x >> 6, n_waves = blockDim.x >> 6;
    const float* t = text + (size_t)b * P;
    for (int q = wave; q < NQ; q += n_waves) {
        const float* p = proj + ((size_t)b * NQ + q) * P;
        float n2 = 0.0f, dt = 0.0f;
        for (int j = lane; j < P; j += 64) {
            const float v = p[j];
            n2 = fmaf(v, v, n2);
            dt = fmaf(v, t[j], dt);
        }
        for (int off = 32; off > 0; off >>= 1) {
            n2 += __shfl_down(n2, off, 64);
            dt += __shfl_down(dt, off, 64);
        }
        if (lane == 0) cos_q[q] = dt / fmaxf(sqrtf(n2), 1e-12f);
    }
    __syncthreads();
    if (wave == 0) {
        float c = lane < NQ ? cos_q[lane] : -__builtin_huge_valf();
        for (int off = 32; off > 0; off >>= 1) c = fmaxf(c, __shfl_down(c, off, 64));
        if (lane == 0) out[b] = c;
    }
}

template <int T>
__global__ __launch_bounds__(512) void itc_head_multi_kernel(const float* __restrict__ proj, int NQ, int P,
                                                             const float* __restrict__ text, int U,
                                                             const int* __restrict__ idx, float* __restrict__ out) {
    __shared__ float cos_q[T][64];
    const int b = blockIdx.x, lane = threadIdx.x & 63, wave = threadIdx.x >> 6, n_waves = blockDim.x >> 6;
    const float* tp[T];
    unsigned ok = 0;
#pragma unroll
    for (int t = 0; t < T; t++) {
        const int u = idx[(size_t)b * T + t];
        const bool in = u >= 0 && u < U;
        ok |= (unsigned)in << t;
        tp[t] = text + (size_t)(in ? u : 0) * P;
    }
    for (int q = wave; q < NQ; q += n_waves) {
        const float* p = proj + ((size_t)b * NQ + q) * P;
        float n2 = 0.0f, dt[T];
#pragma unroll
        for (int t = 0; t < T; t++) dt[t] = 0.0f;
        for (int j = lane; j < P; j += 64) {
            const float v = p[j];
            n2 = fmaf(v, v, n2);
#pragma unroll
            for (int t = 0; t < T; t++) dt[t] = fmaf(v, tp[t][j], dt[t]);
        }
        for (int off = 32; off > 0; off >>= 1) {
            n2 += __shfl_down(n2, off, 64);
#pragma unroll
            for (int t = 0; t < T; t++) dt[t] += __shfl_down(dt[t], off, 64);
        }
        if (lane == 0) {
            const float nrm = fmaxf(sqrtf(n2), 1e-12f);
#pragma unroll
            for (int t = 0; t < T; t++) cos_q[t][q] = dt[t] / nrm;
        }
    }
    __syncthreads();
    if (wave < T) {
        float c = lane < NQ ? cos_q[wave][lane] : -__builtin_huge_valf();
        for (int off = 32; off > 0; off >>= 1) c = fmaxf(c, __shfl_down(c, off, 64));
        if (lane == 0) out[(size_t)b * T + wave] = (ok >> wave) & 1u ? c : __builtin_nanf("");
    }
}

}

using namespace vlfm;

extern "C" int vlfm_resample_coeffs_filter_host(int in_size, int out_size, int filter, int32_t* h_bounds, int32_t* h_kk,
                                                int kk_capacity, int* ksize_out) {
    if (in_size <= 0 || out_size <= 0 || !h_bounds || !h_kk || !ksize_out || (filter != 0 && filter != 1))
        return fail(VLFM_ERR_INVALID, "resample_coeffs_host: bad argument (filter 0 = bicubic, 1 = bilinear)");
    auto bicubic = [filter](double x) {
        if (x < 0.0) x = -x;
        if (filter == 1) return x < 1.0 ? 1.0 - x : 0.0;
        const double a = -0.5;
        if (x < 1.0) return ((a + 2.0) * x - (a + 3.0)) * x * x + 1;
        if (x < 2.0) return (((x - 5) * x + 8) * x - 4) * a;
        return 0.0;
    };
    const float in0 = 0.0f, in1 = (float)in_size;
    double scale = (double)(in1 - in0) / out_size, filterscale = scale;
    if (filterscale < 1.0) filterscale = 1.0;
    const double support = (filter == 1 ? 1.0 : 2.0) * filterscale;
    const int ksize = (int)std::ceil(support) * 2 + 1;
    *ksize_out = ksize;
    if ((long)out_size * ksize > kk_capacity) return fail(VLFM_ERR_CAPACITY, "resample_coeffs_host: kk capacity");
    std::vector<double> k(ksize);
    for (int xx = 0; xx < out_size; xx++) {
        const double center = in0 + (xx + 0.5) * scale;
        double ww = 0.0;
        const double ss = 1.0 / filterscale;
        int xmin = (int)(center - support + 0.5);
        if (xmin < 0) xmin = 0;
        int xmax = (int)(center + support + 0.5);
        if (xmax > in_size) xmax = in_size;
        xmax -= xmin;
        for (int x = 0; x < xmax; x++) {
            const double w = bicubic((x + xmin - center + 0.5) * ss);
            k[x] = w;
            ww += w;
        }
        for (int x = 0; x < xmax; x++)
            if (ww != 0.0) k[x] /= ww;
        for (int x = xmax; x < ksize; x++) k[x] = 0;
        h_bounds[2 * xx] = xmin;
        h_bounds[2 * xx + 1] = xmax;
        for (int x = 0; x < ksize; x++) {
            const double v = k[x];
            h_kk[(size_t)xx * ksize + x] = v < 0 ? (int)(-0.5 + v * (1 << PRECISION_BITS)) : (int)(0.5 + v * (1 << PRECISION_BITS));
        }
    }
    return VLFM_OK;
}

extern "C" int vlfm_resample_coeffs_host(int in_size, int out_size, int32_t* h_bounds, int32_t* h_kk, int kk_capacity,
                                         int* ksize_out) {
    return vlfm_resample_coeffs_filter_host(in_size, out_size, 0, h_bounds, h_kk, kk_capacity, ksize_out);
}

extern "C" int vlfm_preprocess_sam_batched(const uint8_t* d_rgb, int n, int height, int width, int out_h, int out_w,
                                           const int32_t* d_hbounds, const int32_t* d_hk, int hksize,
                                           const int32_t* d_vbounds, const int32_t* d_vk, int vksize,
                                           const float* h_mean3, const float* h_std3, int pad_size, uint8_t* d_tmp,
                                           float* d_out, void* stream) {
    if (n == 0) return VLFM_OK;
    if (!d_rgb || !d_hbounds || !d_hk || !d_vbounds || !d_vk || !h_mean3 || !h_std3 || !d_tmp || !d_out || n < 0 ||
        height <= 0 || width <= 0 || out_h <= 0 || out_w <= 0 || pad_size < out_h || pad_size < out_w)
        return fail(VLFM_ERR_INVALID, "preprocess_sam_batched: bad argument");
    hipStream_t s = (hipStream_t)stream;
    const size_t lds = ((size_t)width * 3 + 15) / 16 * 16;
    {
        VLFM_TIMED("resample_h_kernel", s);
        VLFM_KLAUNCH(resample_h_kernel, dim3(height, n), dim3(256), lds, s, d_rgb, height, width, out_w, d_hbounds, d_hk,
                     hksize, d_tmp);
    }
    int rc = check_launch("resample_h_kernel");
    if (rc != VLFM_OK) return rc;
    Norm3 nrm;
    for (int c = 0; c < 3; c++) { nrm.mean[c] = h_mean3[c]; nrm.std[c] = h_std3[c]; }
    VLFM_TIMED("resample_v_sam_kernel", s);
    VLFM_KLAUNCH(resample_v_sam_kernel, dim3(pad_size, n), dim3(256), 0, s, d_tmp, height, out_h, out_w, pad_size,
                 d_vbounds, d_vk, vksize, nrm, d_out);
    return check_launch("resample_v_sam_kernel");
}

extern "C" int vlfm_preprocess_rgb_batched(const uint8_t* d_rgb, int n, int height, int width, int out_size,
                                           const int32_t* d_hbounds, const int32_t* d_hk, int hksize,
                                           const int32_t* d_vbounds, const int32_t* d_vk, int vksize,
                                           const float* h_mean3, const float* h_std3, uint8_t* d_tmp, void* d_out,
                                           int out_dtype, int patch_size, void* stream) {
    if (n == 0) return VLFM_OK;
    if (!d_rgb || !d_hbounds || !d_hk || !d_vbounds || !d_vk || !h_mean3 || !h_std3 || !d_tmp || !d_out || n < 0 ||
        height <= 0 || width <= 0 || out_size <= 0 || patch_size < 0 || (patch_size > 0 && out_size % patch_size != 0))
        return fail(VLFM_ERR_INVALID, "preprocess_rgb_batched: bad argument");
    hipStream_t s = (hipStream_t)stream;
    Norm3 nrm;
    for (int c = 0; c < 3; c++) { nrm.mean[c] = h_mean3[c]; nrm.std[c] = h_std3[c]; }
    if (out_dtype < 0 || out_dtype > 2)
        return fail(VLFM_ERR_INVALID, "preprocess_rgb_batched: out_dtype must be 0 (f32), 1 (f16) or 2 (bf16)");
    const int row_bytes = width * 3;
    if (row_bytes % 16 == 0 && row_bytes <= 4096 && ((uintptr_t)d_rgb & 15) == 0 && hksize <= 32 && out_size <= 256 &&
        !getenv("VLFM_PREPROCESS_TWO_PASS")) {
        const int OP = (out_size + 3) & ~3;
        auto span = [&](int R) { return (int)(((long)(R - 1) * height + out_size - 1) / out_size) + vksize + 2; };
        auto lds_of = [&](int R) { return (size_t)3 * 256 * 4 + (size_t)2 * PF_GROUPS * PF_ROW_BYTES + (size_t)3 * span(R) * OP; };
        int R = out_size < 32 ? out_size : 32;
        while (R > 1 && lds_of(R) > 80 * 1024) R--;
        while (R > 8 && (long)((out_size + R - 1) / R) * n < 512) R = (R + 1) / 2;
        const int bands = (out_size + R - 1) / R;
        R = (out_size + bands - 1) / bands;
        const size_t lds = lds_of(R);
        const int TR = span(R);
        const dim3 grid(bands, n), block(PF_THREADS);
        VLFM_TIMED("preprocess_fused_kernel", s);
#define VLFM_PF_LAUNCH(KS, T)                                                                                          \
    do {                                                                                                               \
        static LdsOptIn opt;                                                                                           \
        if (!opt.ensure(reinterpret_cast<const void*>(preprocess_fused_kernel<KS, T>), 80 * 1024))                     \
            return fail(VLFM_ERR_HIP, "preprocess_rgb_batched: cannot opt in to 80 KB of LDS");                        \
        VLFM_KLAUNCH((preprocess_fused_kernel<KS, T>), grid, block, lds, s, d_rgb, height, width, out_size, R, TR,     \
                     d_hbounds, d_hk, hksize, d_vbounds, d_vk, vksize, nrm, (T*)d_out, patch_size);                    \
    } while (0)
#define VLFM_PF_DTYPE(KS)                                                                                              \
    do {                                                                                                               \
        if (out_dtype == 0) VLFM_PF_LAUNCH(KS, float);                                                                 \
        else if (out_dtype == 1) VLFM_PF_LAUNCH(KS, __half);                                                           \
        else VLFM_PF_LAUNCH(KS, __hip_bfloat16);                                                                       \
    } while (0)
        if (hksize <= 8) VLFM_PF_DTYPE(8);
        else if (hksize <= 13) VLFM_PF_DTYPE(13);
        else if (hksize <= 16) VLFM_PF_DTYPE(16);
        else if (hksize <= 25) VLFM_PF_DTYPE(25);
        else VLFM_PF_DTYPE(32);
#undef VLFM_PF_DTYPE
#undef VLFM_PF_LAUNCH
        return check_launch("preprocess_fused_kernel");
    }
    const size_t lds = ((size_t)width * 3 + 15) / 16 * 16;
    {
        VLFM_TIMED("resample_h_kernel", s);
    VLFM_KLAUNCH(resample_h_kernel, dim3(height, n), dim3(256), lds, s, d_rgb, height, width, out_size,
                       d_hbounds, d_hk, hksize, d_tmp);
    }
    int rc = check_launch("resample_h_kernel");
    if (rc != VLFM_OK) return rc;
    VLFM_TIMED("resample_v_norm_kernel", s);
    if (out_dtype == 0)
        VLFM_KLAUNCH(resample_v_norm_kernel<float>, dim3(out_size, n), dim3(256), 0, s, d_tmp, height, out_size,
                           d_vbounds, d_vk, vksize, nrm, (float*)d_out, patch_size);
    else if (out_dtype == 1)
        VLFM_KLAUNCH(resample_v_norm_kernel<__half>, dim3(out_size, n), dim3(256), 0, s, d_tmp, height,
                           out_size, d_vbounds, d_vk, vksize, nrm, (__half*)d_out, patch_size);
    else
        VLFM_KLAUNCH(resample_v_norm_kernel<__hip_bfloat16>, dim3(out_size, n), dim3(256), 0, s, d_tmp, height,
                           out_size, d_vbounds, d_vk, vksize, nrm, (__hip_bfloat16*)d_out, patch_size);
    return check_launch("resample_v_norm_kernel");
}

extern "C" int vlfm_itc_head_batched(const float* d_proj, int batch, int n_query, int proj_dim, const float* d_text,
                                     float* d_out, void* stream) {
    if (batch == 0) return VLFM_OK;
    if (!d_proj || !d_text || !d_out || batch < 0 || n_query <= 0 || n_query > 64 || proj_dim <= 0)
        return fail(VLFM_ERR_INVALID, "itc_head_batched: bad argument (n_query <= 64)");
    VLFM_TIMED("itc_head_kernel", stream);
    VLFM_KLAUNCH(itc_head_kernel, dim3(batch), dim3(512), 0, (hipStream_t)stream, d_proj, n_query, proj_dim,
                       d_text, d_out);
    return check_launch("itc_head_kernel");
}

extern "C" int vlfm_itc_head_multi(const float* d_proj, int batch, int n_query, int proj_dim, const float* d_text_table,
                                   int n_text, const int32_t* d_text_index, int n_prompts, float* d_out, void* stream) {
    if (!d_proj || !d_text_table || !d_text_index || !d_out || batch < 0 || n_query <= 0 || n_query > 64 || proj_dim <= 0 ||
        n_text < 1 || n_prompts < 1 || n_prompts > VLFM_ITC_MAX_PROMPTS)
        return fail(VLFM_ERR_INVALID, "itc_head_multi: bad argument (n_query <= 64, 1 <= n_prompts <= 8, n_text >= 1)");
    if (batch == 0) return VLFM_OK;
    VLFM_TIMED("itc_head_multi_kernel", stream);
#define VLFM_ITC_MULTI(T)                                                                                              \
    case T:                                                                                                            \
        VLFM_KLAUNCH(itc_head_multi_kernel<T>, dim3(batch), dim3(512), 0, (hipStream_t)stream, d_proj, n_query,        \
                     proj_dim, d_text_table, n_text, d_text_index, d_out);                                             \
        break
    switch (n_prompts) {
        VLFM_ITC_MULTI(1); VLFM_ITC_MULTI(2); VLFM_ITC_MULTI(3); VLFM_ITC_MULTI(4);
        VLFM_ITC_MULTI(5); VLFM_ITC_MULTI(6); VLFM_ITC_MULTI(7); VLFM_ITC_MULTI(8);
    }
#undef VLFM_ITC_MULTI
    return check_launch("itc_head_multi_kernel");
}

extern "C" int vlfm_layernorm_bias_f16(const void* d_x, const float* d_channel_bias, const void* d_gamma, const void* d_beta,
                                       void* d_y, int rows, int dim, float eps, void* stream) {
    if (rows == 0) return VLFM_OK;
    if (!d_x || !d_gamma || !d_beta || !d_y || rows < 0 || dim <= 0 || dim % 8 != 0 || dim > 64 * 8 * LN_MAXV)
        return fail(VLFM_ERR_INVALID, "layernorm_bias_f16: dim must be a multiple of 8 and <= 2048");
    const int nvec = dim / 8, nv = (nvec + 63) / 64;
    int rpw = rows / 8192;
    rpw = rpw < 1 ? 1 : rpw > LN_ROWS ? LN_ROWS : rpw;
    const int waves = (rows + rpw - 1) / rpw;
    const dim3 grid((waves + 3) / 4), block(256);
    const __half* x = (const __half*)d_x; const __half* g = (const __half*)d_gamma; const __half* b = (const __half*)d_beta;
    __half* y = (__half*)d_y;
    VLFM_TIMED("layernorm_bias_f16_kernel", stream);
    switch (nv) {
        case 1: VLFM_KLAUNCH(layernorm_bias_f16_kernel<1>, grid, block, 0, (hipStream_t)stream, x, d_channel_bias, g, b, y, rows, dim, eps, rpw); break;
        case 2: VLFM_KLAUNCH(layernorm_bias_f16_kernel<2>, grid, block, 0, (hipStream_t)stream, x, d_channel_bias, g, b, y, rows, dim, eps, rpw); break;
        case 3: VLFM_KLAUNCH(layernorm_bias_f16_kernel<3>, grid, block, 0, (hipStream_t)stream, x, d_channel_bias, g, b, y, rows, dim, eps, rpw); break;
        default: VLFM_KLAUNCH(layernorm_bias_f16_kernel<4>, grid, block, 0, (hipStream_t)stream, x, d_channel_bias, g, b, y, rows, dim, eps, rpw); break;
    }
    return check_launch("layernorm_bias_f16_kernel");
}
```

vlfm_amd/vlm/blip2itm.py:

```python
from __future__ import annotations

import hashlib
import math
import os
import re
from dataclasses import dataclass
from typing import Dict, List, Optional, Sequence, Tuple

import numpy as np
import torch
import torch.nn as nn
import torch.nn.functional as F


@dataclass
class Blip2ITCConfig:
    image_size: int = 224
    patch_size: int = 14
    v_hidden: int = 1408
    v_layers: int = 39
    v_heads: int = 16
    v_mlp: int = 6144
    v_ln_eps: float = 1e-6
    q_hidden: int = 768
    q_layers: int = 12
    q_heads: int = 12
    q_mlp: int = 3072
    q_ln_eps: float = 1e-12
    cross_attention_frequency: int = 2
    vocab_size: int = 30523
    max_position_embeddings: int = 512
    num_query_tokens: int = 32
    proj_dim: int = 256
    max_txt_len: int = 32

    @staticmethod
    def tiny() -> "Blip2ITCConfig":
        return Blip2ITCConfig(image_size=28, patch_size=14, v_hidden=32, v_layers=2, v_heads=4, v_mlp=64,
                              q_hidden=24, q_layers=4, q_heads=4, q_mlp=48, vocab_size=97,
                              max_position_embeddings=40, num_query_tokens=5, proj_dim=8)


DEFAULT_HIP_GEMMS = ("fc1",)


def x_is_contiguous_f16(t: torch.Tensor) -> bool:
    return t.dtype == torch.float16 and t.is_contiguous()


class _VitBlock(nn.Module):
    def __init__(self, c: Blip2ITCConfig):
        super().__init__()
        self.heads = c.v_heads
        self.layer_norm1 = nn.LayerNorm(c.v_hidden, eps=c.v_ln_eps)
        self.qkv = nn.Linear(c.v_hidden, 3 * c.v_hidden, bias=True)
        self.projection = nn.Linear(c.v_hidden, c.v_hidden)
        self.layer_norm2 = nn.LayerNorm(c.v_hidden, eps=c.v_ln_eps)
        self.fc1 = nn.Linear(c.v_hidden, c.v_mlp)
        self.fc2 = nn.Linear(c.v_mlp, c.v_hidden)

        self._packed = None
        self.hip_attention = True
        self.strict_hip_attention = True
        self.hip_mlp_min_rows = 32 * 257
        self.hip_gemms = frozenset(DEFAULT_HIP_GEMMS)

    def pack_heads(self, multiple: int = 32) -> None:
        h, d = self.heads, self.qkv.in_features
        hd = d // h
        hp = (hd + multiple - 1) // multiple * multiple
        if hp == hd:
            self._packed = None
            return
        w = self.qkv.weight.detach().view(3, h, hd, d)
        bq = self.qkv.bias.detach().view(3, h, hd)
        wq = torch.zeros((3, h, hp, d), dtype=w.dtype, device=w.device)
        bb = torch.zeros((3, h, hp), dtype=w.dtype, device=w.device)
        wq[:, :, :hd] = w
        bb[:, :, :hd] = bq
        pw = self.projection.weight.detach().view(d, h, hd)
        wp = torch.zeros((d, h, hp), dtype=pw.dtype, device=pw.device)
        wp[:, :, :hd] = pw
        self._packed = (wq.view(3 * h * hp, d).contiguous(), bb.view(-1).contiguous(), wp.view(d, h * hp).contiguous(),
                        hp, float(hd) ** -0.5)

    def hip_gemms_at(self, rows: int) -> frozenset:
        from . import ops

        if not (self.hip_mlp_min_rows and rows >= self.hip_mlp_min_rows):
            return frozenset()
        layers = {"qkv": self.qkv, "proj": self.projection, "fc1": self.fc1, "fc2": self.fc2}

        def ok(lin: nn.Linear) -> bool:
            w, b = lin.weight, lin.bias
            return (x_is_contiguous_f16(w) and w.shape[1] % 64 == 0 and w.shape[0] % 8 == 0 and w.numel() * 2 < (1 << 32)
                    and rows * max(w.shape) * 2 < (1 << 32) and (b is None or x_is_contiguous_f16(b)))

        return frozenset(n for n in self.hip_gemms if ok(layers[n]))

    def forward_deferred(self, x: torch.Tensor, c_in: torch.Tensor, c_mid: torch.Tensor) -> torch.Tensor:
        from . import ops

        b, n, d = x.shape
        hd = d // self.heads
        hip = self.hip_gemms_at(b * n)
        h = ops.layernorm_bias(x, c_in, self.layer_norm1.weight, self.layer_norm1.bias, self.layer_norm1.eps)
        x2 = x.view(b * n, d)
        a = None
        if self.hip_attention and n == ops.VIT_ATTENTION_TOKENS and hd in ops.VIT_ATTENTION_HEADS:
            if "qkv" in hip:
                qkv = ops.linear_f16(h.view(b * n, d), self.qkv.weight, self.qkv.bias, "bias")
            else:
                qkv = F.linear(h.view(b * n, d), self.qkv.weight, self.qkv.bias)
            try:
                a = ops.vit_attention(qkv, b, n, self.heads, hd, float(hd) ** -0.5)
            except (RuntimeError, AssertionError, IndexError) as exc:
                if self.strict_hip_attention:
                    raise
                import warnings

                warnings.warn(f"vlfm_vit_attention_f16 unavailable ({exc}); using the library attention kernel instead")
                self.hip_attention = False
        if a is not None:
            if "proj" in hip and x2.is_contiguous():
                ops.linear_f16(a, self.projection.weight, None, "accumulate", out=x2)
            else:
                x2.addmm_(a, self.projection.weight.t())
        elif self._packed is not None:
            wq, bq, wp, hp, scale = self._packed
            q = F.linear(h.view(b * n, d), wq, bq).view(b, n, 3, self.heads, hp).permute(2, 0, 3, 1, 4)
            a = F.scaled_dot_product_attention(q[0], q[1], q[2], scale=scale).transpose(1, 2).reshape(b * n, self.heads * hp)
            x2.addmm_(a, wp.t())
        else:
            q = self.qkv(h).view(b, n, 3, self.heads, hd).permute(2, 0, 3, 1, 4)
            a = F.scaled_dot_product_attention(q[0], q[1], q[2]).transpose(1, 2).reshape(b * n, d)
            x2.addmm_(a, self.projection.weight.t())
        h = ops.layernorm_bias(x, c_mid, self.layer_norm2.weight, self.layer_norm2.bias, self.layer_norm2.eps)
        if "fc1" in hip:
            act = ops.linear_gelu(h.view(b * n, d), self.fc1.weight, self.fc1.bias)
        else:
            act = F.gelu(F.linear(h, self.fc1.weight, self.fc1.bias)).view(b * n, -1)
        if "fc2" in hip and x2.is_contiguous():
            ops.linear_f16(act, self.fc2.weight, None, "accumulate", out=x2)
        else:
            x2.addmm_(act, self.fc2.weight.t())
        return x

    def forward(self, x: torch.Tensor) -> torch.Tensor:
        b, n, d = x.shape
        if self._packed is not None and self._packed[0].dtype == x.dtype:
            wq, bq, wp, hp, scale = self._packed
            qkv = F.linear(self.layer_norm1(x), wq, bq).view(b, n, 3, self.heads, hp).permute(2, 0, 3, 1, 4)
            a = F.scaled_dot_product_attention(qkv[0], qkv[1], qkv[2], scale=scale)
            x = x + F.linear(a.transpose(1, 2).reshape(b, n, self.heads * hp), wp, self.projection.bias)
        else:
            qkv = self.qkv(self.layer_norm1(x)).view(b, n, 3, self.heads, d // self.heads).permute(2, 0, 3, 1, 4)
            a = F.scaled_dot_product_attention(qkv[0], qkv[1], qkv[2])
            x = x + self.projection(a.transpose(1, 2).reshape(b, n, d))
        return x + self.fc2(F.gelu(self.fc1(self.layer_norm2(x))))


def _exact_split3(w: torch.Tensor) -> Tuple[torch.Tensor, torch.Tensor, torch.Tensor]:
    w = w.detach().float()
    w1 = w.half()
    r = (w - w1.float()) * 2048.0
    w2 = r.half()
    return w1, w2, ((r - w2.float()) * 2048.0).half()


KV_SPLIT_PIECES = 2


def _split_gemm(x16: torch.Tensor, pieces, bias: torch.Tensor, n_pieces: Optional[int] = None) -> torch.Tensor:
    w1t, w2t, w3t = pieces
    if (KV_SPLIT_PIECES if n_pieces is None else n_pieces) >= 3:
        o = torch.addmm(bias, x16, w3t, alpha=2.0 ** -22, out_dtype=torch.float32)
        torch.addmm(o, x16, w2t, alpha=2.0 ** -11, out_dtype=torch.float32, out=o)
    else:
        o = torch.addmm(bias, x16, w2t, alpha=2.0 ** -11, out_dtype=torch.float32)
    torch.addmm(o, x16, w1t, out_dtype=torch.float32, out=o)
    return o


QFORMER_SPLIT_MIN_ROWS = 2048


def _qlinear(x: torch.Tensor, lin_w: torch.Tensor, lin_b, act=None, residual=None) -> torch.Tensor:
    from . import ops

    if (x.is_cuda and x.dtype == torch.float32 and lin_w.dtype == torch.float32 and not torch.is_grad_enabled()
            and x.numel() // x.shape[-1] >= QFORMER_SPLIT_MIN_ROWS and ops.linear_f32_supported(x, lin_w)):
        return ops.linear_f32(x, lin_w, lin_b, act=act, residual=residual, precision="split", owner="blip2")
    y = F.linear(x, lin_w, lin_b)
    if act == "gelu":
        y = F.gelu(y)
    return y if residual is None else y + residual


class _BertAttention(nn.Module):
    def __init__(self, hidden: int, kv_hidden: int, heads: int, eps: float):
        super().__init__()
        self.heads = heads
        self.query = nn.Linear(hidden, hidden)
        self.key = nn.Linear(kv_hidden, hidden)
        self.value = nn.Linear(kv_hidden, hidden)
        self.dense = nn.Linear(hidden, hidden)
        self.LayerNorm = nn.LayerNorm(hidden, eps=eps)
        self._kv_split = None
        self._qkv_fused = None

    def _project_kv_f16(self, kv16: torch.Tensor) -> Tuple[torch.Tensor, torch.Tensor]:
        if self._kv_split is None or self._kv_split[0].device != kv16.device:
            w1, w2, w3 = _exact_split3(torch.cat([self.key.weight, self.value.weight]))
            bias = torch.cat([self.key.bias, self.value.bias]).detach().float()
            self._kv_split = (w1.t(), w2.t(), w3.t(), bias)
        o = _split_gemm(kv16.reshape(-1, kv16.shape[-1]), self._kv_split[:3], self._kv_split[3])
        o = o.view(*kv16.shape[:-1], -1)
        hid = self.key.out_features
        return o[..., :hid], o[..., hid:]

    def forward(self, x: torch.Tensor, kv: Optional[torch.Tensor] = None, mask: Optional[torch.Tensor] = None,
                kv_proj: Optional[Tuple[torch.Tensor, torch.Tensor]] = None, kv_blocks=None) -> torch.Tensor:
        b, n, d = x.shape
        h = self.heads
        if kv_blocks is not None:
            from . import ops

            blocks, tokens, k_block0, v_block0 = kv_blocks
            q = _qlinear(x, self.query.weight, self.query.bias).contiguous()
            a = ops.qformer_cross_attention(q, blocks, tokens, h, k_block0, v_block0, (d // h) ** -0.5)
            return self.LayerNorm(_qlinear(a, self.dense.weight, self.dense.bias, residual=x))
        if kv_proj is not None:
            q = _qlinear(x, self.query.weight, self.query.bias).view(b, n, h, d // h).transpose(1, 2)
            k = kv_proj[0].reshape(b, -1, h, d // h).transpose(1, 2)
            v = kv_proj[1].reshape(b, -1, h, d // h).transpose(1, 2)
        elif kv is None and x.is_cuda and not self.training:
            if self._qkv_fused is None or self._qkv_fused[0].device != x.device or self._qkv_fused[0].dtype != x.dtype:
                self._qkv_fused = (torch.cat([self.query.weight, self.key.weight, self.value.weight]).detach(),
                                   torch.cat([self.query.bias, self.key.bias, self.value.bias]).detach())
            qkv = _qlinear(x, *self._qkv_fused).view(b, n, 3, h, d // h).permute(2, 0, 3, 1, 4)
            q, k, v = qkv[0], qkv[1], qkv[2]
        else:
            q = self.query(x).view(b, n, h, d // h).transpose(1, 2)
            if kv is not None and kv.dtype == torch.float16 and kv.is_cuda and self.key.weight.dtype == torch.float32:
                k, v = self._project_kv_f16(kv)
                src_len = kv.shape[1]
            else:
                src = x if kv is None else kv.to(x.dtype)
                k, v, src_len = self.key(src), self.value(src), src.shape[1]
            k = k.reshape(b, src_len, h, d // h).transpose(1, 2)
            v = v.reshape(b, src_len, h, d // h).transpose(1, 2)
        a = F.scaled_dot_product_attention(q, k, v, attn_mask=mask)
        return self.LayerNorm(_qlinear(a.transpose(1, 2).reshape(b, n, d), self.dense.weight, self.dense.bias,
                                       residual=x))


class _BertFFN(nn.Module):
    def __init__(self, hidden: int, inter: int, eps: float):
        super().__init__()
        self.up = nn.Linear(hidden, inter)
        self.down = nn.Linear(inter, hidden)
        self.LayerNorm = nn.LayerNorm(hidden, eps=eps)

    def forward(self, x: torch.Tensor) -> torch.Tensor:
        hid = _qlinear(x, self.up.weight, self.up.bias, act="gelu")
        return self.LayerNorm(_qlinear(hid, self.down.weight, self.down.bias, residual=x))


class _QFormerLayer(nn.Module):
    def __init__(self, c: Blip2ITCConfig, idx: int):
        super().__init__()
        self.attention = _BertAttention(c.q_hidden, c.q_hidden, c.q_heads, c.q_ln_eps)
        self.crossattention = (_BertAttention(c.q_hidden, c.v_hidden, c.q_heads, c.q_ln_eps)
                               if idx % c.cross_attention_frequency == 0 else None)
        self.ffn_text = _BertFFN(c.q_hidden, c.q_mlp, c.q_ln_eps)
        self.ffn_query = _BertFFN(c.q_hidden, c.q_mlp, c.q_ln_eps)


class Blip2ITCModel(nn.Module):

    def __init__(self, cfg: Blip2ITCConfig):
        super().__init__()
        c = self.cfg = cfg
        n_patches = (c.image_size // c.patch_size) ** 2
        self.class_embedding = nn.Parameter(torch.zeros(1, 1, c.v_hidden))
        self.position_embedding = nn.Parameter(torch.zeros(1, n_patches + 1, c.v_hidden))
        self.patch_embedding = nn.Conv2d(3, c.v_hidden, c.patch_size, c.patch_size)
        self.blocks = nn.ModuleList([_VitBlock(c) for _ in range(c.v_layers)])
        self.post_layernorm = nn.LayerNorm(c.v_hidden, eps=c.v_ln_eps)
        self.query_tokens = nn.Parameter(torch.zeros(1, c.num_query_tokens, c.q_hidden))
        self.word_embeddings = nn.Embedding(c.vocab_size, c.q_hidden)
        self.position_embeddings = nn.Embedding(c.max_position_embeddings, c.q_hidden)
        self.q_layernorm = nn.LayerNorm(c.q_hidden, eps=c.q_ln_eps)
        self.q_layers = nn.ModuleList([_QFormerLayer(c, i) for i in range(c.q_layers)])
        self.vision_projection = nn.Linear(c.q_hidden, c.proj_dim)
        self.text_projection = nn.Linear(c.q_hidden, c.proj_dim)
        self.deferred_bias = True
        self._deferred_c: Optional[torch.Tensor] = None
        self.split_kv = True
        self.split_kv_min_rows = 32 * 257
        self._kv_all = None
        self.fused_cross_kv = True
        self._kv_pair = None

    def init_random(self, seed: int = 0) -> "Blip2ITCModel":
        dev = self.query_tokens.device
        g = torch.Generator(device=dev).manual_seed(seed)
        with torch.no_grad():
            for p in self.parameters():
                if p.dim() > 1:
                    p.copy_(torch.randn(p.shape, generator=g, device=dev) * 0.02)
                else:
                    p.zero_()
            for m in self.modules():
                if isinstance(m, nn.LayerNorm):
                    m.weight.fill_(1.0)
        self.weights_changed()
        return self

    def weights_changed(self) -> None:
        self._deferred_c = None
        self._kv_all = None
        self._kv_pair = None
        for layer in self.q_layers:
            layer.attention._qkv_fused = None
            if layer.crossattention is not None:
                layer.crossattention._kv_split = None

    def vision_dtype(self) -> torch.dtype:
        return self.patch_embedding.weight.dtype

    def set_precision(self, vision_dtype: torch.dtype = torch.float16) -> "Blip2ITCModel":
        for m in (self.patch_embedding, self.blocks, self.post_layernorm):
            m.to(vision_dtype)
        self.class_embedding.data = self.class_embedding.data.to(vision_dtype)
        self.position_embedding.data = self.position_embedding.data.to(vision_dtype)
        self.weights_changed()
        return self

    def load_hf_state_dict(self, sd: Dict[str, torch.Tensor]) -> None:
        own = dict(self.named_parameters())

        def put(name: str, src: str) -> None:
            with torch.no_grad():
                own[name].copy_(sd[src].to(own[name].dtype).reshape(own[name].shape))

        put("class_embedding", "vision_model.embeddings.class_embedding")
        put("position_embedding", "vision_model.embeddings.position_embedding")
        put("patch_embedding.weight", "vision_model.embeddings.patch_embedding.weight")
        put("patch_embedding.bias", "vision_model.embeddings.patch_embedding.bias")
        for i in range(self.cfg.v_layers):
            s, d = f"vision_model.encoder.layers.{i}.", f"blocks.{i}."
            for a, b in [("layer_norm1", "layer_norm1"), ("layer_norm2", "layer_norm2"),
                         ("self_attn.qkv", "qkv"), ("self_attn.projection", "projection"),
                         ("mlp.fc1", "fc1"), ("mlp.fc2", "fc2")]:
                put(d + b + ".weight", s + a + ".weight")
                put(d + b + ".bias", s + a + ".bias")
        put("post_layernorm.weight", "vision_model.post_layernorm.weight")
        put("post_layernorm.bias", "vision_model.post_layernorm.bias")
        put("query_tokens", "query_tokens")
        put("word_embeddings.weight", "embeddings.word_embeddings.weight")
        put("position_embeddings.weight", "embeddings.position_embeddings.weight")
        put("q_layernorm.weight", "qformer.layernorm.weight")
        put("q_layernorm.bias", "qformer.layernorm.bias")
        for i, layer in enumerate(self.q_layers):
            s, d = f"qformer.encoder.layer.{i}.", f"q_layers.{i}."
            atts = [("attention", "attention")] + ([("crossattention", "crossattention")]
                                                   if layer.crossattention is not None else [])
            for a, b in atts:
                for hf, mine in [("attention.query", "query"), ("attention.key", "key"), ("attention.value", "value"),
                                 ("output.dense", "dense"), ("output.LayerNorm", "LayerNorm")]:
                    put(f"{d}{b}.{mine}.weight", f"{s}{a}.{hf}.weight")
                    put(f"{d}{b}.{mine}.bias", f"{s}{a}.{hf}.bias")
            for hf_i, hf_o, mine in [("intermediate", "output", "ffn_text"),
                                     ("intermediate_query", "output_query", "ffn_query")]:
                put(f"{d}{mine}.up.weight", f"{s}{hf_i}.dense.weight")
                put(f"{d}{mine}.up.bias", f"{s}{hf_i}.dense.bias")
                put(f"{d}{mine}.down.weight", f"{s}{hf_o}.dense.weight")
                put(f"{d}{mine}.down.bias", f"{s}{hf_o}.dense.bias")
                put(f"{d}{mine}.LayerNorm.weight", f"{s}{hf_o}.LayerNorm.weight")
                put(f"{d}{mine}.LayerNorm.bias", f"{s}{hf_o}.LayerNorm.bias")
        for n in ("vision_projection", "text_projection"):
            put(n + ".weight", n + ".weight")
            put(n + ".bias", n + ".bias")

    def load_lavis_state_dict(self, sd: Dict[str, torch.Tensor], vit_sd: Optional[Dict[str, torch.Tensor]] = None) -> None:
        c = self.cfg
        sd = {(k[len("module."):] if k.startswith("module.") else k): v for k, v in sd.items()}
        vit = {("visual_encoder." + k): v for k, v in (vit_sd or {}).items()}
        overlap = set(vit) & set(sd)
        if overlap:
            raise KeyError(f"the vision tower is given twice (e.g. {sorted(overlap)[:2]})")
        src = {**sd, **vit}
        own = dict(self.named_parameters())
        used, fed = set(), set()

        def take(key: str) -> torch.Tensor:
            if key not in src:
                raise KeyError(f"LAVIS state dict lacks {key}" + ("" if vit_sd is not None or not key.startswith("visual_encoder.")
                                                                 else " (blip2_pretrained.pth does not carry the frozen ViT: "
                                                                      "pass eva_vit_g.pth as the vision checkpoint)"))
            used.add(key)
            return src[key]

        def put(name: str, value: torch.Tensor) -> None:
            if tuple(value.shape) != tuple(own[name].shape) and value.numel() != own[name].numel():
                raise ValueError(f"{name}: {tuple(own[name].shape)} in the graph, {tuple(value.shape)} in the file")
            with torch.no_grad():
                own[name].copy_(value.to(own[name].dtype).reshape(own[name].shape))
            fed.add(name)

        put("class_embedding", take("visual_encoder.cls_token"))
        put("position_embedding", take("visual_encoder.pos_embed"))
        put("patch_embedding.weight", take("visual_encoder.patch_embed.proj.weight"))
        put("patch_embedding.bias", take("visual_encoder.patch_embed.proj.bias"))
        for i in range(c.v_layers):
            o, d = f"visual_encoder.blocks.{i}.", f"blocks.{i}."
            for a, b in (("norm1", "layer_norm1"), ("norm2", "layer_norm2"), ("attn.proj", "projection"),
                         ("mlp.fc1", "fc1"), ("mlp.fc2", "fc2")):
                put(d + b + ".weight", take(o + a + ".weight"))
                put(d + b + ".bias", take(o + a + ".bias"))
            put(d + "qkv.weight", take(o + "attn.qkv.weight"))
            qb, vb = take(o + "attn.q_bias"), take(o + "attn.v_bias")
            put(d + "qkv.bias", torch.cat([qb, torch.zeros_like(vb), vb]))
        put("post_layernorm.weight", take("ln_vision.weight"))
        put("post_layernorm.bias", take("ln_vision.bias"))
        put("query_tokens", take("query_tokens"))
        put("word_embeddings.weight", take("Qformer.bert.embeddings.word_embeddings.weight"))
        put("position_embeddings.weight", take("Qformer.bert.embeddings.position_embeddings.weight"))
        put("q_layernorm.weight", take("Qformer.bert.embeddings.LayerNorm.weight"))
        put("q_layernorm.bias", take("Qformer.bert.embeddings.LayerNorm.bias"))
        for i, layer in enumerate(self.q_layers):
            o, d = f"Qformer.bert.encoder.layer.{i}.", f"q_layers.{i}."
            for att in ["attention"] + (["crossattention"] if layer.crossattention is not None else []):
                for theirs, mine in (("self.query", "query"), ("self.key", "key"), ("self.value", "value"),
                                     ("output.dense", "dense"), ("output.LayerNorm", "LayerNorm")):
                    put(f"{d}{att}.{mine}.weight", take(f"{o}{att}.{theirs}.weight"))
                    put(f"{d}{att}.{mine}.bias", take(f"{o}{att}.{theirs}.bias"))
            for t_i, t_o, mine in (("intermediate", "output", "ffn_text"), ("intermediate_query", "output_query", "ffn_query")):
                put(f"{d}{mine}.up.weight", take(f"{o}{t_i}.dense.weight"))
                put(f"{d}{mine}.up.bias", take(f"{o}{t_i}.dense.bias"))
                put(f"{d}{mine}.down.weight", take(f"{o}{t_o}.dense.weight"))
                put(f"{d}{mine}.down.bias", take(f"{o}{t_o}.dense.bias"))
                put(f"{d}{mine}.LayerNorm.weight", take(f"{o}{t_o}.LayerNorm.weight"))
                put(f"{d}{mine}.LayerNorm.bias", take(f"{o}{t_o}.LayerNorm.bias"))
        put("vision_projection.weight", take("vision_proj.weight"))
        put("vision_projection.bias", take("vision_proj.bias"))
        put("text_projection.weight", take("text_proj.weight"))
        put("text_projection.bias", take("text_proj.bias"))
        unfed = sorted(set(own) - fed)
        if unfed:
            raise KeyError(f"{len(unfed)} parameters of the graph were not fed, e.g. {unfed[:4]}")

        def unused_ok(k: str) -> bool:
            return (k.startswith(("Qformer.cls.", "itm_head.")) or k in ("temp", "Qformer.bert.embeddings.position_ids")
                    or k.startswith(f"visual_encoder.blocks.{c.v_layers}.")
                    or k.startswith(("visual_encoder.norm.", "visual_encoder.fc_norm.", "visual_encoder.head.")))

        left = sorted(k for k in src if k not in used and not unused_ok(k))
        if left:
            raise KeyError(f"{len(left)} tensors of the file have no place in the ITC graph, e.g. {left[:4]}")
        self.weights_changed()

    def vision_tokens(self, pixel_values: torch.Tensor) -> torch.Tensor:
        c = self.cfg
        if pixel_values.dim() == 4:
            b, g = pixel_values.shape[0], c.image_size // c.patch_size
            pixel_values = pixel_values.reshape(b, 3, g, c.patch_size, g, c.patch_size).permute(0, 2, 4, 1, 3, 5) \
                .reshape(b, g * g, 3 * c.patch_size * c.patch_size)
        w = self.patch_embedding.weight
        x = F.linear(pixel_values.to(w.dtype), w.view(w.shape[0], -1), self.patch_embedding.bias)
        x = torch.cat([self.class_embedding.expand(x.shape[0], -1, -1), x], dim=1) + self.position_embedding
        if self.deferred_bias and x.is_cuda and x.dtype == torch.float16 and c.v_hidden % 8 == 0 and c.v_hidden <= 2048:
            from . import ops

            c = self._deferred_constants()
            x = x.contiguous()
            for i, blk in enumerate(self.blocks):
                x = blk.forward_deferred(x, c[2 * i], c[2 * i + 1])
            return ops.layernorm_bias(x, c[2 * len(self.blocks)], self.post_layernorm.weight, self.post_layernorm.bias,
                                      self.post_layernorm.eps)
        for blk in self.blocks:
            x = blk(x)
        return self.post_layernorm(x)

    def _deferred_constants(self) -> torch.Tensor:
        if self._deferred_c is None or self._deferred_c.device != self.post_layernorm.weight.device:
            rows, run = [], torch.zeros(self.cfg.v_hidden, dtype=torch.float32, device=self.post_layernorm.weight.device)
            for blk in self.blocks:
                rows.append(run.clone())
                run = run + blk.projection.bias.detach().float()
                rows.append(run.clone())
                run = run + blk.fc2.bias.detach().float()
            rows.append(run.clone())
            self._deferred_c = torch.stack(rows).contiguous()
        return self._deferred_c

    def query_features(self, image_tokens: torch.Tensor) -> torch.Tensor:
        split_ok = (self.split_kv and image_tokens.dtype == torch.float16 and image_tokens.is_cuda
                    and image_tokens.shape[0] * image_tokens.shape[1] >= self.split_kv_min_rows)
        enc = image_tokens if split_ok else image_tokens.to(self.q_layernorm.weight.dtype)
        h = self.q_layernorm(self.query_tokens).expand(enc.shape[0], -1, -1)
        fused = split_ok and self._fused_cross_ok(enc)
        blocks = self._project_all_kv_blocks(enc) if fused else None
        proj = self._project_all_kv(enc) if split_ok and not fused else None
        hid, at = self.cfg.q_hidden, 0
        for layer in self.q_layers:
            h = layer.attention(h)
            if layer.crossattention is not None:
                if blocks is not None:
                    h = layer.crossattention(h, kv_blocks=(blocks, enc.shape[1], at // 64, (at + hid) // 64))
                    at += 2 * hid
                elif proj is not None:
                    h = layer.crossattention(h, kv_proj=(proj[..., at:at + hid], proj[..., at + hid:at + 2 * hid]))
                    at += 2 * hid
                else:
                    h = layer.crossattention(h, kv=enc)
            h = layer.ffn_query(h)
        return h

    def _fused_cross_ok(self, tokens16: torch.Tensor) -> bool:
        from . import ops

        c = self.cfg
        return (self.fused_cross_kv and KV_SPLIT_PIECES == 2 and not torch.is_grad_enabled()
                and self.q_layernorm.weight.dtype == torch.float32
                and c.q_hidden % c.q_heads == 0 and c.q_hidden // c.q_heads == ops.QFORMER_ATTENTION_HEAD
                and c.num_query_tokens <= ops.QFORMER_ATTENTION_MAX_QUERIES
                and 1 <= tokens16.shape[1] <= ops.QFORMER_ATTENTION_MAX_TOKENS and c.v_hidden % 64 == 0
                and tokens16.shape[0] * tokens16.shape[1] * c.v_hidden * 2 < (1 << 32))

    def _kv_all_pieces(self, device):
        if self._kv_all is None or self._kv_all[0].device != device:
            cross = [l.crossattention for l in self.q_layers if l.crossattention is not None]
            w = torch.cat([torch.cat([c.key.weight, c.value.weight]) for c in cross])
            bias = torch.cat([torch.cat([c.key.bias, c.value.bias]) for c in cross]).detach().float()
            w1, w2, w3 = _exact_split3(w)
            self._kv_all = (w1.t(), w2.t(), w3.t(), bias)
            self._kv_pair = None
        return self._kv_all

    def _project_all_kv_blocks(self, tokens16: torch.Tensor) -> torch.Tensor:
        from . import ops

        w1t, w2t, _, bias = self._kv_all_pieces(tokens16.device)
        if self._kv_pair is None:
            self._kv_pair = (ops.interleave_pair_weights(w1t.t(), w2t.t()), bias.contiguous())
        return ops.linear_pair_f32(tokens16.reshape(-1, tokens16.shape[-1]), *self._kv_pair)

    def _project_all_kv(self, tokens16: torch.Tensor) -> torch.Tensor:
        pieces = self._kv_all_pieces(tokens16.device)
        o = _split_gemm(tokens16.reshape(-1, tokens16.shape[-1]), pieces[:3], pieces[3])
        return o.view(*tokens16.shape[:-1], -1)

    def text_feature(self, input_ids: torch.Tensor, attention_mask: Optional[torch.Tensor] = None) -> torch.Tensor:
        pos = torch.arange(input_ids.shape[1], device=input_ids.device)[None]
        h = self.q_layernorm(self.word_embeddings(input_ids) + self.position_embeddings(pos))
        mask = None
        if attention_mask is not None:
            mask = (attention_mask[:, None, None, :] > 0)
        for layer in self.q_layers:
            h = layer.ffn_text(layer.attention(h, mask=mask))
        return F.normalize(self.text_projection(h[:, 0, :]), dim=-1)

    def itc_reference_head(self, query_feats: torch.Tensor, text_feat: torch.Tensor) -> torch.Tensor:
        img = F.normalize(self.vision_projection(query_feats.float()), dim=-1)
        return torch.einsum("bqd,bd->bq", img, text_feat.float().expand(img.shape[0], -1)).max(dim=1).values


_CAPTION_STRIP = re.compile(r"([.!\"()*#:;~])")


def blip_caption(text: str, max_words: int = 50) -> str:
    t = _CAPTION_STRIP.sub(" ", text.lower())
    t = re.sub(r"\s{2,}", " ", t).rstrip("\n").strip(" ")
    words = t.split(" ")
    return " ".join(words[:max_words]) if len(words) > max_words else t


class HashTokenizer:

    def __init__(self, vocab_size: int, max_len: int):
        self.vocab_size, self.max_len = vocab_size, max_len

    def __call__(self, text: str) -> List[int]:
        ids = [101 % self.vocab_size]
        for w in text.split():
            hv = int.from_bytes(hashlib.sha1(w.encode()).digest()[:4], "little")
            ids.append(1000 % self.vocab_size + hv % max(1, self.vocab_size - 1000))
        ids = ids[: self.max_len - 1] + [102 % self.vocab_size]
        return ids


class BLIP2ITM:

    def __init__(self, name: str = "blip2_image_text_matching", model_type: str = "pretrain", device=None,
                 model_dir: Optional[str] = None, config: Optional[Blip2ITCConfig] = None,
                 vision_dtype: torch.dtype = torch.float16, seed: int = 0, allow_random_init: bool = False,
                 strict_hip_attention: bool = True, checkpoint: Optional[str] = None, vit_checkpoint: Optional[str] = None,
                 tokenizer_dir: Optional[str] = None) -> None:
        from ..mapping.base_map import require_gpu
        from .. import _lib

        self.device = require_gpu(device)
        _lib.lib()
        from . import ops as _ops

        _ops.use_tuned_gemms()
        self.cfg = config or Blip2ITCConfig()
        self.tokenizer = None
        model_dir = model_dir or os.environ.get("BLIP2ITM_MODEL_DIR")
        checkpoint = checkpoint or os.environ.get("BLIP2_LAVIS_CHECKPOINT")
        vit_checkpoint = vit_checkpoint or os.environ.get("EVA_VIT_G_CHECKPOINT")
        if checkpoint and not model_dir:
            for f in (checkpoint, vit_checkpoint):
                if f and not os.path.isfile(f):
                    raise FileNotFoundError(f"BLIP-2 checkpoint {f!r} not found")
            self.model = Blip2ITCModel(self.cfg)
            ck = torch.load(checkpoint, map_location="cpu", weights_only=True)
            vit = torch.load(vit_checkpoint, map_location="cpu", weights_only=True) if vit_checkpoint else None
            self.model.load_lavis_state_dict(ck["model"] if isinstance(ck, dict) and "model" in ck else ck,
                                             vit["model"] if isinstance(vit, dict) and "model" in vit else vit)
            self.tokenizer = self._lavis_tokenizer(tokenizer_dir)
            self.weights = f"lavis:{checkpoint}" + (f" + {vit_checkpoint}" if vit_checkpoint else "")
        elif model_dir:
            self.model = Blip2ITCModel(self.cfg)
            self._load_pretrained(model_dir)
            self.weights = f"pretrained:{model_dir}"
        elif not (allow_random_init or config is not None):
            raise ValueError("BLIP2ITM needs `checkpoint` (+ `vit_checkpoint`): LAVIS' blip2_pretrained.pth and eva_vit_g.pth, what "
                             "the reference loads -- or model_dir / BLIP2ITM_MODEL_DIR (a Salesforce/blip2-itm-vit-g directory); "
                             "pass allow_random_init=True for a randomly initialised network (benchmarks / geometry tests only)")
        else:
            with torch.device(self.device):
                self.model = Blip2ITCModel(self.cfg)
            self.model.init_random(seed)
            self.weights = "random-init"
        if self.tokenizer is None:
            self.tokenizer = HashTokenizer(self.cfg.vocab_size, self.cfg.max_txt_len)
        self.model.eval().to(self.device).set_precision(vision_dtype)
        for blk in self.model.blocks:
            blk.pack_heads()
            blk.strict_hip_attention = bool(strict_hip_attention)
        self._text_cache: Dict[str, torch.Tensor] = {}
        self._prompt_cache: Dict[tuple, tuple] = {}
        self._proj_t = None
        self._graphs, self._prompt_graphs = {}, {}
        self.two_stream_min = None
        self._side_stream = None

    def _lavis_tokenizer(self, tokenizer_dir: Optional[str]):
        from transformers import BertTokenizer

        path = tokenizer_dir or os.environ.get("BLIP2_TOKENIZER")
        try:
            if path:
                vocab = path if os.path.isfile(path) else os.path.join(path, "vocab.txt")
                tok = BertTokenizer(vocab_file=vocab, do_lower_case=True)
            else:
                tok = BertTokenizer.from_pretrained("bert-base-uncased", local_files_only=True)
                if len(tok) < 30522:
                    raise FileNotFoundError("no cached bert-base-uncased vocabulary")
        except Exception as exc:
            raise ValueError("BLIP-2 weights need the bert-base-uncased vocabulary: pass tokenizer_dir (or set BLIP2_TOKENIZER) "
                             "to a directory with its vocab.txt") from exc
        tok.add_special_tokens({"bos_token": "[DEC]"})
        return lambda t: tok(t, truncation=True, max_length=self.cfg.max_txt_len)["input_ids"]

    @property
    def strict_hip_attention(self) -> bool:
        return all(blk.strict_hip_attention for blk in self.model.blocks)

    @strict_hip_attention.setter
    def strict_hip_attention(self, on: bool) -> None:
        for blk in self.model.blocks:
            blk.strict_hip_attention = bool(on)

    @property
    def attention_path(self) -> str:
        flags = {bool(blk.hip_attention) for blk in self.model.blocks}
        return "hip" if flags == {True} else "library" if flags == {False} else "mixed"

    def mlp_path(self, n_images: int) -> str:
        blk = self.model.blocks[0]
        rows = n_images * ((self.cfg.image_size // self.cfg.patch_size) ** 2 + 1)
        return "hip" if "fc1" in blk.hip_gemms_at(rows) else "library"

    def gemm_path(self, n_images: int) -> str:
        blk = self.model.blocks[0]
        rows = n_images * ((self.cfg.image_size // self.cfg.patch_size) ** 2 + 1)
        names = sorted(blk.hip_gemms_at(rows))
        return "hip:" + ",".join(names) if names else "library"

    def _load_pretrained(self, model_dir: str) -> None:
        from safetensors.torch import load_file

        sd: Dict[str, torch.Tensor] = {}
        for f in sorted(os.listdir(model_dir)):
            if f.endswith(".safetensors"):
                sd.update(load_file(os.path.join(model_dir, f)))
        self.model.load_hf_state_dict(sd)
        from transformers import BertTokenizer

        tok = BertTokenizer.from_pretrained(model_dir)
        self.tokenizer = lambda t: tok(t, truncation=True, max_length=self.cfg.max_txt_len)["input_ids"]

    @torch.inference_mode()
    def text_feature(self, txt: str) -> torch.Tensor:
        if txt not in self._text_cache:
            ids = torch.tensor([self.tokenizer(blip_caption(txt))], device=self.device)
            self._text_cache[txt] = self.model.text_feature(ids)[0].float().contiguous()
        return self._text_cache[txt]

    def cosine_batch_graphed(self, images_u8: torch.Tensor, txts: Sequence[str]) -> torch.Tensor:
        return self._replay(self._graphs, (tuple(images_u8.shape), tuple(txts)), lambda x: self.cosine_batch(x, txts), images_u8)

    def _replay(self, graphs: dict, key, forward, images_u8: torch.Tensor, keep_alive=()) -> torch.Tensor:
        if key not in graphs:
            static_in = images_u8.clone()
            for _ in range(2):
                forward(static_in)
            torch.cuda.synchronize(self.device)
            g = torch.cuda.CUDAGraph()
            with torch.cuda.graph(g):
                static_out = forward(static_in)
            graphs[key] = (g, static_in, static_out, keep_alive)
        g, static_in, static_out, _ = graphs[key]
        static_in.copy_(images_u8)
        g.replay()
        return static_out

    def _projection(self):
        if self._proj_t is None:
            self._proj_t = (self.model.vision_projection.weight.float().t().contiguous(),
                            self.model.vision_projection.bias.float().contiguous())
        return self._proj_t

    def _query_feats(self, images_u8: torch.Tensor) -> torch.Tensor:
        from . import ops

        B = images_u8.shape[0]
        pix = ops.preprocess_rgb(images_u8, self.cfg.image_size, self.model.vision_dtype(),
                                 patch_size=self.cfg.patch_size)
        if self.two_stream_min is not None and B >= self.two_stream_min and not torch.cuda.is_current_stream_capturing():
            main = torch.cuda.current_stream(self.device)
            if self._side_stream is None:
                self._side_stream = torch.cuda.Stream(self.device)
            side = self._side_stream
            half = B // 2
            side.wait_stream(main)
            with torch.cuda.stream(side):
                q_hi = self.model.query_features(self.model.vision_tokens(pix[half:])).float()
            q_lo = self.model.query_features(self.model.vision_tokens(pix[:half])).float()
            main.wait_stream(side)
            q = torch.cat([q_lo, q_hi]).contiguous()
        else:
            q = self.model.query_features(self.model.vision_tokens(pix)).float().contiguous()
        return q

    @torch.inference_mode()
    def cosine_batch(self, images_u8: torch.Tensor, txts: Sequence[str]) -> torch.Tensor:
        from . import ops

        B = images_u8.shape[0]
        q = self._query_feats(images_u8)
        if len(txts) == 1:
            text = self.text_feature(txts[0])[None].expand(B, -1).contiguous()
        else:
            assert len(txts) == B
            text = torch.stack([self.text_feature(t) for t in txts]).contiguous()
        return ops.itc_head(q, *self._projection(), text)

    def _prompt_tensors(self, prompts, B: int):
        from . import ops

        key = (B, tuple(prompts) if isinstance(prompts[0], str) else tuple(tuple(p) for p in prompts))
        hit = self._prompt_cache.get(key)
        if hit is None:
            unique, rows = prompt_table(prompts, B)
            table = torch.stack([self.text_feature(t) for t in unique]).contiguous()
            hit = self._prompt_cache[key] = (table, ops.itc_text_index(rows, len(unique), self.device), key)
        return hit

    @torch.inference_mode()
    def cosine_prompts_batch(self, images_u8: torch.Tensor, prompts) -> torch.Tensor:
        from . import ops

        B = images_u8.shape[0]
        q = self._query_feats(images_u8)
        table, index, _ = self._prompt_tensors(prompts, B)
        return ops.itc_head_multi(q, *self._projection(), table, index)

    def cosine_prompts_batch_graphed(self, images_u8: torch.Tensor, prompts) -> torch.Tensor:
        table, index, structure = self._prompt_tensors(prompts, images_u8.shape[0])
        return self._replay(self._prompt_graphs, (tuple(images_u8.shape), structure),
                            lambda x: self.cosine_prompts_batch(x, prompts), images_u8, keep_alive=(table, index))

    def check_numerics(self) -> None:
        from . import ops

        flag = ops.gemm_f32_overflow_flag(self.device, "blip2")
        if int(flag.item()):
            flag.zero_()
            ops.split_weights_bad(self.device, "blip2")
            raise FloatingPointError("BLIP-2 Q-Former: an activation left f16's range inside a split-precision f32 GEMM; set "
                                     "vlfm_amd.vlm.blip2itm.QFORMER_SPLIT_MIN_ROWS = 1 << 60 to run these layers on the library's f32 GEMMs")

    def cosine(self, image: np.ndarray, txt: str) -> float:
        img = torch.from_numpy(np.ascontiguousarray(image)).to(self.device)[None]
        return float(self.cosine_batch(img, [txt])[0].item())

    def cosines(self, image: np.ndarray, prompts: Sequence[str]) -> List[float]:
        img = torch.from_numpy(np.ascontiguousarray(image)).to(self.device)[None]
        return [float(v) for v in self.cosine_prompts_batch(img, list(prompts))[0].tolist()]


def prompt_table(prompts, n_images: int):
    if len(prompts) == 0:
        raise ValueError("at least one prompt is needed")
    per = [list(prompts)] * n_images if isinstance(prompts[0], str) else [list(p) for p in prompts]
    if len(per) != n_images:
        raise ValueError(f"{len(per)} prompt lists for {n_images} images")
    T = len(per[0]) if per else 0
    if any(len(p) != T for p in per) or (per and T == 0):
        raise ValueError("every image needs the same number (>= 1) of prompts")
    unique: Dict[str, int] = {}
    rows = [[unique.setdefault(t, len(unique)) for t in p] for p in per]
    return list(unique), rows


class BLIP2ITMClient:

    _shared: Dict[str, BLIP2ITM] = {}

    def __init__(self, port: int = 12182, device=None, emulate_jpeg: bool = False, **model_kwargs) -> None:
        key = str(device)
        if key not in BLIP2ITMClient._shared:
            BLIP2ITMClient._shared[key] = BLIP2ITM(device=device, **model_kwargs)
        self._model = BLIP2ITMClient._shared[key]
        self._emulate_jpeg = emulate_jpeg
        self.url = f"inprocess://blip2itm (port {port} ignored)"

    def cosine(self, image: np.ndarray, txt: str) -> float:
        if self._emulate_jpeg:
            from .transport import jpeg_roundtrip

            image = jpeg_roundtrip(image)
        return self._model.cosine(image, txt)

    def cosines(self, image: np.ndarray, prompts: Sequence[str]) -> List[float]:
        if self._emulate_jpeg:
            from .transport import jpeg_roundtrip

            image = jpeg_roundtrip(image)
        return self._model.cosines(image, prompts)
```

vlfm_amd/vlm/ops.py:

```python
from __future__ import annotations

import ctypes
from typing import Dict, Optional, Tuple

import numpy as np
import torch

from .. import _lib

CLIP_MEAN = (0.48145466, 0.4578275, 0.40821073)
CLIP_STD = (0.26862954, 0.26130258, 0.27577711)
_DTYPE_CODE = {torch.float32: 0, torch.float16: 1, torch.bfloat16: 2}
_coeff_cache: Dict[Tuple[str, int, int], Tuple[torch.Tensor, torch.Tensor, int]] = {}


def _stream() -> int:
    return torch._C._cuda_getCurrentRawStream(torch._C._cuda_getDevice())


def resample_coeffs(in_size: int, out_size: int, bilinear: bool = False) -> Tuple[np.ndarray, np.ndarray, int]:
    bounds = np.zeros((out_size, 2), np.int32)
    cap = out_size * (2 * int(np.ceil(2.0 * max(1.0, in_size / out_size))) + 1)
    kk = np.zeros(cap, np.int32)
    ks = ctypes.c_int(0)
    _lib.check(_lib.lib().vlfm_resample_coeffs_filter_host(in_size, out_size, int(bilinear), bounds.ctypes.data,
                                                           kk.ctypes.data, cap, ctypes.byref(ks)),
               "resample_coeffs_host")
    return bounds, kk[: out_size * ks.value].reshape(out_size, ks.value), ks.value


def _device_coeffs(device, in_size: int, out_size: int, bilinear: bool = False):
    key = (str(device), in_size, out_size, bilinear)
    if key not in _coeff_cache:
        b, k, ks = resample_coeffs(in_size, out_size, bilinear)
        _coeff_cache[key] = (torch.from_numpy(b).to(device), torch.from_numpy(np.ascontiguousarray(k)).to(device), ks)
    return _coeff_cache[key]


def preprocess_rgb(images_u8: torch.Tensor, out_size: int = 224, dtype: torch.dtype = torch.float16,
                   mean=CLIP_MEAN, std=CLIP_STD, patch_size: int = 0) -> torch.Tensor:
    assert images_u8.is_cuda and images_u8.dtype == torch.uint8 and images_u8.dim() == 4 and images_u8.shape[-1] == 3
    images_u8 = images_u8.contiguous()
    n, H, W, _ = images_u8.shape
    dev = images_u8.device
    hb, hk, hks = _device_coeffs(dev, W, out_size)
    vb, vk, vks = _device_coeffs(dev, H, out_size)
    tmp = torch.empty((n, H, out_size, 3), dtype=torch.uint8, device=dev)
    if patch_size:
        g = out_size // patch_size
        out = torch.empty((n, g * g, 3 * patch_size * patch_size), dtype=dtype, device=dev)
    else:
        out = torch.empty((n, 3, out_size, out_size), dtype=dtype, device=dev)
    m = (ctypes.c_float * 3)(*mean)
    s = (ctypes.c_float * 3)(*std)
    with torch.cuda.device(dev):
        _lib.check(_lib.lib().vlfm_preprocess_rgb_batched(images_u8.data_ptr(), n, H, W, out_size, hb.data_ptr(),
                                                         hk.data_ptr(), hks, vb.data_ptr(), vk.data_ptr(), vks,
                                                         ctypes.addressof(m), ctypes.addressof(s), tmp.data_ptr(),
                                                         out.data_ptr(), _DTYPE_CODE[dtype], int(patch_size), _stream()),
                   "preprocess_rgb")
    return out


def itc_head(query_feats: torch.Tensor, proj_t: torch.Tensor, proj_bias: torch.Tensor,
             text_feats: torch.Tensor) -> torch.Tensor:
    B, NQ, Hd = query_feats.shape
    P = proj_t.shape[1]
    for t in (query_feats, proj_t, proj_bias, text_feats):
        assert t.is_cuda and t.dtype == torch.float32 and t.is_contiguous()
    assert proj_t.shape[0] == Hd and text_feats.shape == (B, P)
    proj = torch.addmm(proj_bias, query_feats.view(B * NQ, Hd), proj_t)
    out = torch.empty(B, dtype=torch.float32, device=query_feats.device)
    with torch.cuda.device(query_feats.device):
        _lib.check(_lib.lib().vlfm_itc_head_batched(proj.data_ptr(), B, NQ, P, text_feats.data_ptr(), out.data_ptr(),
                                                   _stream()), "itc_head")
    return out


ITC_MAX_PROMPTS = 8


def itc_text_index(rows, n_text: int, device) -> torch.Tensor:
    idx = np.asarray(rows, np.int64)
    if idx.ndim != 2 or idx.shape[1] < 1 or idx.shape[1] > ITC_MAX_PROMPTS:
        raise ValueError(f"text index must be [B, T] with 1 <= T <= {ITC_MAX_PROMPTS}, got shape {idx.shape}")
    if n_text < 1 or (idx.size and (idx.min() < 0 or idx.max() >= n_text)):
        raise ValueError(f"text index outside the table of {n_text} row(s)")
    return torch.from_numpy(idx.astype(np.int32)).to(device)


def itc_head_multi(query_feats: torch.Tensor, proj_t: torch.Tensor, proj_bias: torch.Tensor, text_table: torch.Tensor,
                   text_index: torch.Tensor) -> torch.Tensor:
    B, NQ, Hd = query_feats.shape
    P = proj_t.shape[1]
    for t in (query_feats, proj_t, proj_bias, text_table):
        assert t.is_cuda and t.dtype == torch.float32 and t.is_contiguous()
    assert text_index.is_cuda and text_index.dtype == torch.int32 and text_index.is_contiguous()
    assert proj_t.shape[0] == Hd and text_table.dim() == 2 and text_table.shape[1] == P
    assert text_index.dim() == 2 and text_index.shape[0] == B
    U, T = text_table.shape[0], text_index.shape[1]
    proj = torch.addmm(proj_bias, query_feats.view(B * NQ, Hd), proj_t)
    out = torch.empty((B, T), dtype=torch.float32, device=query_feats.device)
    with torch.cuda.device(query_feats.device):
        _lib.check(_lib.lib().vlfm_itc_head_multi(proj.data_ptr(), B, NQ, P, text_table.data_ptr(), U,
                                                 text_index.data_ptr(), T, out.data_ptr(), _stream()), "itc_head_multi")
    return out


SAM_MEAN = (123.675, 116.28, 103.53)
SAM_STD = (58.395, 57.12, 57.375)


def sam_target_size(h: int, w: int, long_side: int = 1024) -> Tuple[int, int]:
    scale = long_side * 1.0 / max(h, w)
    return int(h * scale + 0.5), int(w * scale + 0.5)


def preprocess_sam(images_u8: torch.Tensor, long_side: int = 1024) -> Tuple[torch.Tensor, Tuple[int, int]]:
    assert images_u8.is_cuda and images_u8.dtype == torch.uint8 and images_u8.dim() == 4 and images_u8.shape[-1] == 3
    images_u8 = images_u8.contiguous()
    n, H, W, _ = images_u8.shape
    oh, ow = sam_target_size(H, W, long_side)
    dev = images_u8.device
    hb, hk, hks = _device_coeffs(dev, W, ow, True)
    vb, vk, vks = _device_coeffs(dev, H, oh, True)
    tmp = torch.empty((n, H, ow, 3), dtype=torch.uint8, device=dev)
    out = torch.empty((n, 3, long_side, long_side), dtype=torch.float32, device=dev)
    m, s = (ctypes.c_float * 3)(*SAM_MEAN), (ctypes.c_float * 3)(*SAM_STD)
    with torch.cuda.device(dev):
        _lib.check(_lib.lib().vlfm_preprocess_sam_batched(images_u8.data_ptr(), n, H, W, oh, ow, hb.data_ptr(),
                                                         hk.data_ptr(), hks, vb.data_ptr(), vk.data_ptr(), vks,
                                                         ctypes.addressof(m), ctypes.addressof(s), long_side,
                                                         tmp.data_ptr(), out.data_ptr(), _stream()), "preprocess_sam")
    return out, (oh, ow)


def layernorm_bias(x: torch.Tensor, channel_bias, weight: torch.Tensor, bias: torch.Tensor, eps: float) -> torch.Tensor:
    assert x.is_cuda and x.dtype == torch.float16 and x.is_contiguous() and weight.dtype == torch.float16
    dim = x.shape[-1]
    y = torch.empty_like(x)
    _lib.check(_lib.lib().vlfm_layernorm_bias_f16(x.data_ptr(), channel_bias.data_ptr() if channel_bias is not None else None,
                                                  weight.data_ptr(), bias.data_ptr(), y.data_ptr(), x.numel() // dim, dim,
                                                  float(eps), _stream()), "layernorm_bias_f16")
    return y


_ACT_CODE = {None: 0, "none": 0, "gelu": 1, "silu": 2}


def bias_act_(y: torch.Tensor, bias: torch.Tensor, act=None) -> torch.Tensor:
    assert y.is_cuda and y.dim() == 4 and y.is_contiguous() and y.dtype in (torch.float32, torch.float16)
    assert bias.dtype == y.dtype and bias.numel() == y.shape[1] and bias.is_contiguous()
    n, c, h, w = y.shape
    _lib.check(_lib.lib().vlfm_bias_act_nchw(y.data_ptr(), bias.data_ptr(), n, c, h * w, 0 if y.dtype == torch.float32 else 1,
                                             _ACT_CODE[act], _stream()), "bias_act_nchw")
    return y


_BIAS_ACT_MAX_PLANES = 65535 * 16


class BiasAct(torch.nn.Module):

    def __init__(self, bias: torch.Tensor, act=None, inplace: bool = False):
        super().__init__()
        self.bias = torch.nn.Parameter(bias.detach().clone(), requires_grad=False)
        self.act = act
        self.inplace = inplace

    def forward(self, x):
        return bias_act(x, self.bias, self.act, inplace=self.inplace)


def bias_act(x: torch.Tensor, bias: torch.Tensor, act=None, inplace: bool = False) -> torch.Tensor:
    if (inplace and x.is_cuda and x.dim() == 4 and x.dtype in (torch.float32, torch.float16) and x.is_contiguous()
            and not x.requires_grad and x.shape[0] * x.shape[1] <= _BIAS_ACT_MAX_PLANES):
        return bias_act_(x, bias if bias.dtype == x.dtype else bias.to(x.dtype), act)
    y = x + bias.to(x.dtype).view(1, -1, 1, 1)
    if act == "gelu":
        return torch.nn.functional.gelu(y)
    if act == "silu":
        return torch.nn.functional.silu(y)
    return y


def depthwise_conv3x3(x: torch.Tensor, weight: torch.Tensor, bias, stride: int = 1, gelu: bool = False) -> torch.Tensor:
    assert x.is_cuda and x.dtype == torch.float32 and x.dim() == 4 and x.is_contiguous()
    n, c, h, w = x.shape
    assert weight.shape == (c, 1, 3, 3) and weight.dtype == torch.float32 and weight.is_contiguous()
    ho, wo = (h - 1) // stride + 1, (w - 1) // stride + 1
    y = torch.empty((n, c, ho, wo), dtype=torch.float32, device=x.device)
    _lib.check(_lib.lib().vlfm_dwconv3x3_f32(x.data_ptr(), weight.data_ptr(), bias.data_ptr() if bias is not None else None,
                                             y.data_ptr(), n, c, h, w, int(stride), int(gelu), _stream()), "dwconv3x3_f32")
    return y


def layernorm_rows(x: torch.Tensor, weight: torch.Tensor, bias: torch.Tensor, eps: float, window: int = 0, shift: int = 0,
                   pad_zero: bool = False) -> torch.Tensor:
    assert x.is_cuda and x.dtype == torch.float32 and x.dim() == 4 and x.is_contiguous()
    B, H, W, C = x.shape
    assert weight.dtype == torch.float32 and bias.dtype == torch.float32 and weight.numel() == C == bias.numel()
    if window > 0:
        nwy, nwx = (H + window - 1) // window, (W + window - 1) // window
        out = torch.empty((B * nwy * nwx, window * window, C), dtype=torch.float32, device=x.device)
    else:
        out = torch.empty_like(x)
    _lib.check(_lib.lib().vlfm_layernorm_rows_shifted_f32(x.data_ptr(), weight.data_ptr(), bias.data_ptr(), out.data_ptr(), B, H, W, C,
                                                          int(window), float(eps), int(shift), int(pad_zero), _stream()),
               "layernorm_rows_f32")
    return out


def window_reverse_add_(x: torch.Tensor, windows: torch.Tensor, window: int, shift: int = 0) -> torch.Tensor:
    assert x.is_cuda and x.dtype == torch.float32 and x.dim() == 4 and x.is_contiguous()
    B, H, W, C = x.shape
    nwy, nwx = (H + window - 1) // window, (W + window - 1) // window
    assert windows.is_contiguous() and windows.dtype == torch.float32 and windows.numel() == B * nwy * nwx * window * window * C
    _lib.check(_lib.lib().vlfm_window_reverse_add_shifted_f32(x.data_ptr(), windows.data_ptr(), B, H, W, C, int(window), int(shift),
                                                              _stream()), "window_reverse_add_f32")
    return x


def depthwise_conv3x3_nhwc(x: torch.Tensor, w9c: torch.Tensor, bias) -> torch.Tensor:
    assert x.is_cuda and x.dtype == torch.float32 and x.dim() == 4 and x.is_contiguous()
    B, H, W, C = x.shape
    assert w9c.shape == (9, C) and w9c.is_contiguous() and w9c.dtype == torch.float32
    out = torch.empty_like(x)
    _lib.check(_lib.lib().vlfm_dwconv3x3_nhwc_f32(x.data_ptr(), w9c.data_ptr(), bias.data_ptr() if bias is not None else None,
                                                  out.data_ptr(), B, H, W, C, _stream()), "dwconv3x3_nhwc_f32")
    return out


def window_attention(qkv: torch.Tensor, bias_t: torch.Tensor, heads: int, scale: float, mask_t=None) -> torch.Tensor:
    assert qkv.is_cuda and qkv.dtype == torch.float32 and qkv.dim() == 3 and qkv.is_contiguous() and qkv.shape[2] == heads * 96
    nw, n, _ = qkv.shape
    assert bias_t.shape == (heads, n, n) and bias_t.is_contiguous() and bias_t.dtype == torch.float32 and n <= 256
    out = torch.empty((nw, n, heads * 32), dtype=torch.float32, device=qkv.device)
    per_image = 1
    if mask_t is not None:
        assert mask_t.dim() == 3 and mask_t.shape[1:] == (n, n) and mask_t.is_contiguous() and mask_t.dtype == torch.float32
        per_image = mask_t.shape[0]
        assert nw % per_image == 0
    _lib.check(_lib.lib().vlfm_window_attention_masked_f32(qkv.data_ptr(), bias_t.data_ptr(),
                                                           mask_t.data_ptr() if mask_t is not None else None, per_image,
                                                           out.data_ptr(), nw, n, heads, float(scale), _stream()),
               "window_attention_f32")
    return out


GEMM_F16_EPILOGUE = {"bias": 0, "bias_gelu": 1, "accumulate": 2}


def linear_f16_supported(x: torch.Tensor, weight: torch.Tensor) -> bool:
    k = weight.shape[1]
    return (x.is_cuda and x.dtype == torch.float16 and weight.dtype == torch.float16 and x.shape[-1] == k and k % 64 == 0
            and weight.shape[0] % 8 == 0 and x.numel() * 2 < (1 << 32) and weight.numel() * 2 < (1 << 32))


def linear_f16(x: torch.Tensor, weight: torch.Tensor, bias: Optional[torch.Tensor] = None, epilogue: str = "bias",
               out: Optional[torch.Tensor] = None) -> torch.Tensor:
    assert x.is_cuda and x.dtype == torch.float16 and x.is_contiguous() and x.dim() == 2
    assert weight.dtype == torch.float16 and weight.is_contiguous() and weight.shape[1] == x.shape[1]
    assert bias is None or (bias.dtype == torch.float16 and bias.is_contiguous())
    M, K = x.shape
    N = weight.shape[0]
    assert all(t is None or t.data_ptr() % 16 == 0 for t in (x, weight, bias, out)), "linear_f16: 16-byte aligned tensors only"
    if out is None:
        assert epilogue != "accumulate", "accumulate needs the tensor to accumulate into"
        out = torch.empty((M, N), dtype=torch.float16, device=x.device)
    else:
        assert out.dtype == torch.float16 and out.is_contiguous() and out.shape == (M, N) and out.device == x.device
    _lib.check(_lib.lib().vlfm_gemm_f16_nt(x.data_ptr(), weight.data_ptr(), bias.data_ptr() if bias is not None else None,
                                           out.data_ptr(), M, N, K, GEMM_F16_EPILOGUE[epilogue], _stream()), "gemm_f16_nt")
    return out


def linear_gelu(x: torch.Tensor, weight: torch.Tensor, bias: torch.Tensor) -> torch.Tensor:
    return linear_f16(x, weight, bias, "bias_gelu")


def interleave_pair_weights(w1: torch.Tensor, w2: torch.Tensor) -> torch.Tensor:
    assert w1.shape == w2.shape and w1.dtype == w2.dtype == torch.float16 and w1.dim() == 2 and w1.shape[0] % 64 == 0
    n, k = w1.shape
    return torch.stack([w1.reshape(n // 64, 64, k), w2.reshape(n // 64, 64, k)], dim=1).reshape(2 * n, k).contiguous()


def linear_pair_f32(x: torch.Tensor, w_pair: torch.Tensor, bias: Optional[torch.Tensor] = None,
                    out: Optional[torch.Tensor] = None) -> torch.Tensor:
    assert x.is_cuda and x.dtype == torch.float16 and x.is_contiguous() and x.dim() == 2
    assert w_pair.dtype == torch.float16 and w_pair.is_contiguous() and w_pair.shape[1] == x.shape[1] and w_pair.shape[0] % 128 == 0
    M, K = x.shape
    N = w_pair.shape[0] // 2
    assert bias is None or (bias.dtype == torch.float32 and bias.is_contiguous() and bias.numel() == N)
    assert all(t is None or t.data_ptr() % 16 == 0 for t in (x, w_pair, bias, out)), "linear_pair_f32: 16-byte aligned tensors only"
    if out is None:
        out = torch.empty((N // 64, M, 64), dtype=torch.float32, device=x.device)
    else:
        assert out.dtype == torch.float32 and out.is_contiguous() and out.shape == (N // 64, M, 64) and out.device == x.device
    _lib.check(_lib.lib().vlfm_gemm_f16_pair_f32_nt(x.data_ptr(), w_pair.data_ptr(), bias.data_ptr() if bias is not None else None,
                                                    out.data_ptr(), M, N, K, _stream()), "gemm_f16_pair_f32_nt")
    return out


QFORMER_ATTENTION_MAX_TOKENS, QFORMER_ATTENTION_MAX_QUERIES, QFORMER_ATTENTION_HEAD = 257, 32, 64


def qformer_cross_attention(q: torch.Tensor, kv_blocks: torch.Tensor, tokens: int, heads: int, k_block0: int, v_block0: int,
                            scale: float, out: Optional[torch.Tensor] = None) -> torch.Tensor:
    assert q.is_cuda and q.dtype == torch.float32 and q.is_contiguous() and q.dim() == 3 and q.shape[2] == heads * 64
    assert kv_blocks.dtype == torch.float32 and kv_blocks.is_contiguous() and kv_blocks.dim() == 3 and kv_blocks.shape[2] == 64
    assert kv_blocks.device == q.device and max(k_block0, v_block0) + heads <= kv_blocks.shape[0] and min(k_block0, v_block0) >= 0
    B, Q, _ = q.shape
    if out is None:
        out = torch.empty_like(q)
    else:
        assert out.dtype == torch.float32 and out.is_contiguous() and out.shape[1:] == q.shape[1:] and out.shape[0] >= B
    _lib.check(_lib.lib().vlfm_qformer_cross_attention_f32(q.data_ptr(), kv_blocks.data_ptr(), out.data_ptr(), B, tokens, Q, heads,
                                                           k_block0, v_block0, kv_blocks.shape[1], float(scale), _stream()),
               "qformer_cross_attention_f32")
    return out


VIT_ATTENTION_TOKENS, VIT_ATTENTION_HEADS = 257, (88,)


def vit_attention(qkv: torch.Tensor, batch: int, tokens: int, heads: int, head_dim: int, scale: float) -> torch.Tensor:
    assert qkv.is_cuda and qkv.dtype == torch.float16 and qkv.is_contiguous()
    assert qkv.numel() == batch * tokens * 3 * heads * head_dim
    out = torch.empty((batch * tokens, heads * head_dim), dtype=torch.float16, device=qkv.device)
    _lib.check(_lib.lib().vlfm_vit_attention_f16(qkv.data_ptr(), out.data_ptr(), batch, tokens, heads, head_dim,
                                                 float(scale), _stream()), "vit_attention_f16")
    return out


_ACT32 = {None: 0, "none": 0, "relu": 1, "gelu": 2}
GEMM_F32_PRECISION = {"exact": 0, "split": 1}
_overflow_flags: Dict[tuple, torch.Tensor] = {}
_split_cache: Dict[int, tuple] = {}


def gemm_f32_overflow_flag(device, owner: str = "") -> torch.Tensor:
    d = torch.device(device)
    index = d.index if d.index is not None else (torch.cuda.current_device() if d.type == "cuda" else 0)
    key = (d.type, index, owner)
    if key not in _overflow_flags:
        _overflow_flags[key] = torch.zeros(1, dtype=torch.int32, device=torch.device(d.type, index))
    return _overflow_flags[key]


def tensor_version(t: torch.Tensor) -> int:
    try:
        return t._version
    except RuntimeError:
        return 0


def split_weight(weight: torch.Tensor, owner: str = "") -> Tuple[torch.Tensor, torch.Tensor]:
    import weakref

    key = id(weight)
    hit = _split_cache.get(key)
    if hit is not None and hit[0]() is weight and hit[1] == tensor_version(weight) and hit[2] == weight.data_ptr():
        if hit[6]:
            gemm_f32_overflow_flag(weight.device, owner).bitwise_or_(hit[5])
        return hit[3], hit[4]
    if len(_split_cache) > 2048:
        for k in [k for k, v in _split_cache.items() if v[0]() is None]:
            del _split_cache[k]
    w = weight.detach().contiguous()
    hi = torch.empty(w.shape, dtype=torch.float16, device=w.device)
    lo = torch.empty_like(hi)
    bad = torch.zeros(1, dtype=torch.int32, device=w.device)
    _lib.check(_lib.lib().vlfm_split_f32_to_f16_pair(w.data_ptr(), hi.data_ptr(), lo.data_ptr(), w.numel(), bad.data_ptr(),
                                                     _stream()), "split_f32")
    gemm_f32_overflow_flag(w.device, owner).bitwise_or_(bad)
    _split_cache[key] = [weakref.ref(weight), tensor_version(weight), weight.data_ptr(), hi, lo, bad, False, owner]
    return hi, lo


def split_weights_bad(device, owner: str = "") -> bool:
    d = torch.device(device)
    entries = [v for v in _split_cache.values() if v[7] == owner and v[0]() is not None and v[5].device.type == d.type
               and (d.index is None or v[5].device.index == d.index)]
    if not entries:
        return False
    verdict = torch.cat([v[5] for v in entries]).cpu().tolist()
    for v, b in zip(entries, verdict):
        v[6] = bool(b)
    return any(verdict)


def linear_f32_supported(x: torch.Tensor, weight: torch.Tensor) -> bool:
    k = weight.shape[1]
    return (x.is_cuda and x.dtype == torch.float32 and weight.dtype == torch.float32 and k % 32 == 0 and x.shape[-1] == k
            and weight.shape[0] >= 32 and x.numel() // k >= 64 and not torch.is_grad_enabled())


def linear_f32(x: torch.Tensor, weight: torch.Tensor, bias=None, act=None, residual=None, precision: str = "exact",
               out=None, owner: str = "") -> torch.Tensor:
    K = weight.shape[1]
    N = weight.shape[0]
    lead = x.shape[:-1]
    x2 = x.reshape(-1, K)
    if not x2.is_contiguous() or x2.data_ptr() % 16:
        x2 = x2.contiguous()
    w = weight if weight.is_contiguous() else weight.contiguous()
    M = x2.shape[0]
    if out is None:
        out = torch.empty((M, N), dtype=torch.float32, device=x.device)
    res = None
    if residual is not None:
        res = residual.reshape(M, N)
        if not res.is_contiguous() or res.data_ptr() % 16:
            res = res.contiguous()
    b = None
    if bias is not None:
        b = bias if bias.is_contiguous() else bias.contiguous()
    prec = GEMM_F32_PRECISION[precision]
    hi = lo = None
    if prec == 1:
        hi, lo = split_weight(w, owner)
    _lib.check(_lib.lib().vlfm_gemm_f32_nt(x2.data_ptr(), w.data_ptr(), b.data_ptr() if b is not None else None,
                                           res.data_ptr() if res is not None else None, out.data_ptr(), M, N, K, _ACT32[act], prec,
                                           hi.data_ptr() if hi is not None else None, lo.data_ptr() if lo is not None else None,
                                           gemm_f32_overflow_flag(x.device, owner).data_ptr(), _stream()), "gemm_f32_nt")
    return out.view(*lead, N)


_tuned_gemms_state = None


def use_tuned_gemms() -> bool:
    global _tuned_gemms_state
    if _tuned_gemms_state is None:
        import os

        path = os.path.join(os.path.dirname(os.path.dirname(os.path.abspath(__file__))), "tunableop_results.csv")
        ok = False
        if os.environ.get("VLFM_TUNED_GEMMS", "1") != "0" and os.path.exists(path) and torch.cuda.is_available():
            try:
                import torch.cuda.tunable as tunable

                import tempfile

                tunable.enable(True)
                tunable.tuning_enable(False)
                tunable.set_filename(os.path.join(tempfile.gettempdir(), f"vlfm_amd_tunableop_{os.getpid()}.csv"))
                ok = bool(tunable.read_file(path))
            except Exception as exc:
                import warnings

                warnings.warn(f"tuned GEMM solutions not loaded ({type(exc).__name__}: {exc})")
                ok = False
        _tuned_gemms_state = ok
    return _tuned_gemms_state
```

Baseline: 1776 env-steps/s.

## Fuse ViT entrance assembly with first LayerNorm, add native Q-Former self-attention and LN

Adds a fused kernel that concatenates the class token, adds position embeddings and applies the first block's LayerNorm in one pass, so the separate cat/add and LN passes over the 257-token f16 activations are no longer needed. Adds an MFMA-based f32 self-attention kernel for the 32 Q-Former queries, replacing the permute plus SDPA path. Adds a native f32 LayerNorm kernel used for the Q-Former residual norms. These cut kernel launches and memory passes, but bring new kernels whose numerics and corner cases (queries ≤32, head width 64) have to match the old path.

New measurement: 1771 env-steps/s. About the same (-0.2%).

```diff
diff --git a/include/vlfm_amd.h b/include/vlfm_amd.h
--- a/include/vlfm_amd.h
+++ b/include/vlfm_amd.h
@@ -173,6 +173,12 @@
 
 int vlfm_qformer_cross_attention_f32(const void* d_q, const void* d_kv_blocks, void* d_out, int batch, int tokens, int queries,
                                      int heads, int k_block0, int v_block0, int m_total, float scale, void* stream);
+
+int vlfm_vit_assemble_ln_f16(const void* d_patch, const void* d_cls, const void* d_pos, const float* d_channel_bias, const void* d_gamma,
+                             const void* d_beta, void* d_x, void* d_h, int batch, int patches, int dim, float eps, void* stream);
+int vlfm_qformer_self_attention_f32(const void* d_qkv, void* d_out, int batch, int queries, int heads, float scale, void* stream);
+int vlfm_layernorm_f32(const float* d_x, const float* d_gamma, const float* d_beta, float* d_y, int rows, int dim, float eps,
+                       void* stream);
 
 int vlfm_gemm_f16_tile_order(int m, int n, int group_m, int* out, int capacity_pairs);
 int vlfm_gemm_f16_work_items(int m, int n, int grid, int* out, int capacity_pairs);
diff --git a/vlfm_amd/_lib.py b/vlfm_amd/_lib.py
--- a/vlfm_amd/_lib.py
+++ b/vlfm_amd/_lib.py
@@ -147,7 +147,10 @@
         L.vlfm_gemm_f16_nt.argtypes = [vp, vp, vp, vp, ci, ci, ci, ci, vp]
         L.vlfm_gemm_f16_pair_f32_nt.argtypes = [vp, vp, vp, vp, ci, ci, ci, vp]
         L.vlfm_qformer_cross_attention_f32.argtypes = [vp, vp, vp, ci, ci, ci, ci, ci, ci, ci, ctypes.c_float, vp]
-        L.vlfm_gemm_f32_nt.argtypes = [vp, vp, vp, vp, vp, ci, ci, ci, ci, ci, vp, vp, vp, vp]
+        L.vlfm_vit_assemble_ln_f16.argtypes = [vp, vp, vp, vp, vp, vp, vp, vp, ci, ci, ci, ctypes.c_float, vp]
+        L.vlfm_qformer_self_attention_f32.argtypes = [vp, vp, ci, ci, ci, ctypes.c_float, vp]
+        L.vlfm_layernorm_f32.argtypes = [vp, vp, vp, vp, ci, ci, ctypes.c_float, vp]
+        L.vlfm_gemm_f32_nt.argtypes =[vp, vp, vp, vp, vp, ci, ci, ci, ci, ci, vp, vp, vp, vp]
         L.vlfm_split_f32_to_f16_pair.argtypes = [vp, vp, vp, ctypes.c_longlong, vp, vp]
         L.vlfm_layernorm_rows_f32.argtypes = [vp, vp, vp, vp, ci, ci, ci, ci, ci, ctypes.c_float, vp]
         L.vlfm_window_reverse_add_f32.argtypes = [vp, vp, ci, ci, ci, ci, ci, vp]
diff --git a/vlfm_amd/csrc/host.cpp b/vlfm_amd/csrc/host.cpp
--- a/vlfm_amd/csrc/host.cpp
+++ b/vlfm_amd/csrc/host.cpp
@@ -13,7 +13,7 @@
 }
 
 extern "C" const char* vlfm_last_error(void) { return vlfm::g_last_error.c_str(); }
-extern "C" int vlfm_abi_version(void) { return 27; }
+extern "C" int vlfm_abi_version(void) { return 28; }
 
 namespace {
 
diff --git a/vlfm_amd/csrc/qformer_attention.hip b/vlfm_amd/csrc/qformer_attention.hip
--- a/vlfm_amd/csrc/qformer_attention.hip
+++ b/vlfm_amd/csrc/qformer_attention.hip
@@ -236,6 +236,75 @@
         asm volatile("" ::: "memory");
         if (!more) break;
         w = nw; b = nb; h = nh;
+    }
+}
+
+struct QsArgs {
+    const float* qkv;
+    float* out;
+    int B, n, heads;
+    float scale_log2e;
+};
+
+__global__ __launch_bounds__(256) void qformer_self_attention_kernel(QsArgs a) {
+    const int lane = threadIdx.x & 63, col = lane & 31, g = lane >> 5;
+    const long long item = (long long)blockIdx.x * 4 + (threadIdx.x >> 6);
+    if (item >= (long long)a.B * a.heads) return;
+    const int b = (int)(item / a.heads), h = (int)(item - (long long)b * a.heads);
+    const size_t d = (size_t)a.heads * 64, ld = 3 * d;
+    const float* base = a.qkv + (size_t)b * a.n * ld + (size_t)h * 64;
+    const float* qrow = base + (size_t)min(col, a.n - 1) * ld + 32 * g;
+    float qf[32], kf[32];
+#pragma unroll
+    for (int c = 0; c < 8; c++) {
+        const floatx4 q4 = *reinterpret_cast<const floatx4*>(qrow + 4 * c);
+        const floatx4 k4 = *reinterpret_cast<const floatx4*>(qrow + d + 4 * c);
+#pragma unroll
+        for (int e = 0; e < 4; e++) { qf[4 * c + e] = q4[e]; kf[4 * c + e] = k4[e]; }
+    }
+    float v0[16], v1[16];
+#pragma unroll
+    for (int r = 0; r < 16; r++) {
+        const int key = (r & 3) + 8 * (r >> 2) + 4 * g;
+        const float2 v = *reinterpret_cast<const float2*>(base + (size_t)min(key, a.n - 1) * ld + 2 * d + 2 * col);
+        v0[r] = v.x; v1[r] = v.y;
+    }
+    __builtin_amdgcn_sched_barrier(0);
+    floatx16 acc;
+#pragma unroll
+    for (int r = 0; r < 16; r++) acc[r] = 0.f;
+#pragma unroll
+    for (int s = 0; s < 32; s++) acc = __builtin_amdgcn_mfma_f32_32x32x2f32(kf[s], qf[s], acc, 0, 0, 0);
+    float m = -INFINITY;
+#pragma unroll
+    for (int r = 0; r < 16; r++) {
+        const int key = (r & 3) + 8 * (r >> 2) + 4 * g;
+        acc[r] = key < a.n ? acc[r] * a.scale_log2e : -INFINITY;
+        m = fmaxf(m, acc[r]);
+    }
+    m = fmaxf(m, __shfl_xor(m, 32, 64));
+    float l = 0.f;
+#pragma unroll
+    for (int r = 0; r < 16; r++) { const float pj = __builtin_amdgcn_exp2f(acc[r] - m); l += pj; acc[r] = pj; }
+    l += __shfl_xor(l, 32, 64);
+    floatx16 o0, o1;
+#pragma unroll
+    for (int r = 0; r < 16; r++) { o0[r] = 0.f; o1[r] = 0.f; }
+#pragma unroll
+    for (int r = 0; r < 16; r++) {
+        o0 = __builtin_amdgcn_mfma_f32_32x32x2f32(v0[r], acc[r], o0, 0, 0, 0);
+        o1 = __builtin_amdgcn_mfma_f32_32x32x2f32(v1[r], acc[r], o1, 0, 0, 0);
+    }
+    if (col < a.n) {
+        const float inv = 1.0f / l;
+        float* orow = a.out + ((size_t)b * a.n + col) * d + (size_t)h * 64 + 8 * g;
+#pragma unroll
+        for (int q4 = 0; q4 < 4; q4++) {
+            const floatx4 s0 = {o0[4 * q4] * inv, o1[4 * q4] * inv, o0[4 * q4 + 1] * inv, o1[4 * q4 + 1] * inv};
+            const floatx4 s1 = {o0[4 * q4 + 2] * inv, o1[4 * q4 + 2] * inv, o0[4 * q4 + 3] * inv, o1[4 * q4 + 3] * inv};
+            *reinterpret_cast<floatx4*>(orow + 16 * q4) = s0;
+            *reinterpret_cast<floatx4*>(orow + 16 * q4 + 4) = s1;
+        }
     }
 }
 
@@ -268,3 +337,21 @@
     VLFM_KLAUNCH(qformer_cross_attention_kernel, grid, block, lds, stream, a);
     return check_launch("qformer_cross_attention_kernel");
 }
+
+extern "C" int vlfm_qformer_self_attention_f32(const void* d_qkv, void* d_out, int batch, int queries, int heads, float scale,
+                                               void* stream) {
+    if (batch == 0) return VLFM_OK;
+    if (!d_qkv || !d_out || batch < 0 || queries < 1 || queries > QA_MAX_Q || heads < 1 ||
+        (long long)batch * heads > 0x7fffffffLL)
+        return fail(VLFM_ERR_INVALID, "qformer_self_attention_f32: head width 64, 1-32 queries");
+    if ((((uintptr_t)d_qkv | (uintptr_t)d_out) & 15) != 0)
+        return fail(VLFM_ERR_INVALID, "qformer_self_attention_f32: pointers must be 16-byte aligned");
+    QsArgs a;
+    a.qkv = (const float*)d_qkv; a.out = (float*)d_out;
+    a.B = batch; a.n = queries; a.heads = heads;
+    a.scale_log2e = scale * 1.4426950408889634f;
+    const dim3 grid((unsigned)(((long long)batch * heads + 3) / 4)), block(256);
+    VLFM_TIMED("qformer_self_attention_kernel", stream);
+    VLFM_KLAUNCH(qformer_self_attention_kernel, grid, block, 0, stream, a);
+    return check_launch("qformer_self_attention_kernel");
+}
diff --git a/vlfm_amd/csrc/vlm_ops.hip b/vlfm_amd/csrc/vlm_ops.hip
--- a/vlfm_amd/csrc/vlm_ops.hip
+++ b/vlfm_amd/csrc/vlm_ops.hip
@@ -232,86 +232,193 @@
 struct alignas(16) Half8 { __half2 h[4]; };
 
 template <int NV>
+struct LnLane {
+    Half8 gm[NV], bt[NV];
+    float4 c0[NV], c1[NV];
+    int lane, nvec;
+
+    __device__ __forceinline__ LnLane(int lane_, int nvec_, const float* __restrict__ cb, const __half* __restrict__ gamma,
+                                      const __half* __restrict__ beta) : lane(lane_), nvec(nvec_) {
+#pragma unroll
+        for (int i = 0; i < NV; i++) {
+            const int v = lane + 64 * i;
+            if (v < nvec) {
+                gm[i] = reinterpret_cast<const Half8*>(gamma)[v];
+                bt[i] = reinterpret_cast<const Half8*>(beta)[v];
+                c0[i] = cb ? reinterpret_cast<const float4*>(cb)[2 * v] : make_float4(0.f, 0.f, 0.f, 0.f);
+                c1[i] = cb ? reinterpret_cast<const float4*>(cb)[2 * v + 1] : make_float4(0.f, 0.f, 0.f, 0.f);
+            }
+        }
+    }
+    __device__ __forceinline__ void load_row(const __half* __restrict__ row, Half8* dst) const {
+#pragma unroll
+        for (int i = 0; i < NV; i++) {
+            const int v = lane + 64 * i;
+            if (v < nvec) dst[i] = reinterpret_cast<const Half8*>(row)[v];
+        }
+    }
+    __device__ __forceinline__ float val(const Half8* row, int i, int j) const {
+        const float2 t = __half22float2(row[i].h[j >> 1]);
+        const float cc = j < 4 ? (&c0[i].x)[j] : (&c1[i].x)[j - 4];
+        return ((j & 1) ? t.y : t.x) + cc;
+    }
+    __device__ __forceinline__ void normalise(const Half8* cur, float inv_d, float eps, __half* __restrict__ yrow) const {
+        float sum = 0.0f;
+#pragma unroll
+        for (int i = 0; i < NV; i++) {
+            if (lane + 64 * i < nvec) {
+#pragma unroll
+                for (int j = 0; j < 8; j++) sum += val(cur, i, j);
+            }
+        }
+#pragma unroll
+        for (int off = 32; off > 0; off >>= 1) sum += __shfl_xor(sum, off, 64);
+        const float mean = sum * inv_d;
+        float sq = 0.0f;
+#pragma unroll
+        for (int i = 0; i < NV; i++) {
+            if (lane + 64 * i < nvec) {
+#pragma unroll
+                for (int j = 0; j < 8; j++) {
+                    const float dlt = val(cur, i, j) - mean;
+                    sq = fmaf(dlt, dlt, sq);
+                }
+            }
+        }
+#pragma unroll
+        for (int off = 32; off > 0; off >>= 1) sq += __shfl_xor(sq, off, 64);
+        const float rstd = rsqrtf(sq * inv_d + eps);
+#pragma unroll
+        for (int i = 0; i < NV; i++) {
+            const int v = lane + 64 * i;
+            if (v < nvec) {
+                Half8 o;
+#pragma unroll
+                for (int j = 0; j < 4; j++) {
+                    const float2 g2 = __half22float2(gm[i].h[j]), b2 = __half22float2(bt[i].h[j]);
+                    o.h[j] = __floats2half2_rn((val(cur, i, 2 * j) - mean) * rstd * g2.x + b2.x,
+                                               (val(cur, i, 2 * j + 1) - mean) * rstd * g2.y + b2.y);
+                }
+                reinterpret_cast<Half8*>(yrow)[v] = o;
+            }
+        }
+    }
+};
+
+template <int NV>
 __global__ __launch_bounds__(256) void layernorm_bias_f16_kernel(const __half* __restrict__ x, const float* __restrict__ cb,
                                                                  const __half* __restrict__ gamma,
                                                                  const __half* __restrict__ beta, __half* __restrict__ y,
                                                                  int rows, int D, float eps, int rows_per_wave) {
     const int lane = threadIdx.x & 63, wave = (blockIdx.x * blockDim.x + threadIdx.x) >> 6;
-    const int nvec = D >> 3;
     const int r0 = wave * rows_per_wave;
     if (r0 >= rows) return;
-    Half8 gm[NV], bt[NV];
-    float4 c0[NV], c1[NV];
-#pragma unroll
-    for (int i = 0; i < NV; i++) {
-        const int v = lane + 64 * i;
-        if (v < nvec) {
-            gm[i] = reinterpret_cast<const Half8*>(gamma)[v];
-            bt[i] = reinterpret_cast<const Half8*>(beta)[v];
-            c0[i] = cb ? reinterpret_cast<const float4*>(cb)[2 * v] : make_float4(0.f, 0.f, 0.f, 0.f);
-            c1[i] = cb ? reinterpret_cast<const float4*>(cb)[2 * v + 1] : make_float4(0.f, 0.f, 0.f, 0.f);
-        }
-    }
+    const LnLane<NV> ln(lane, D >> 3, cb, gamma, beta);
     Half8 cur[NV], nxt[NV], nx2[NV];
-    auto load_row = [&](int r, Half8* dst) {
+    const int r_end = min(rows, r0 + rows_per_wave);
+    ln.load_row(x + (size_t)r0 * D, cur);
+    if (r0 + 1 < r_end) ln.load_row(x + (size_t)(r0 + 1) * D, nxt);
+    const float inv_d = 1.0f / (float)D;
+    for (int r = r0; r < r_end; r++) {
+        if (r + 2 < r_end) ln.load_row(x + (size_t)(r + 2) * D, nx2);
+        ln.normalise(cur, inv_d, eps, y + (size_t)r * D);
+#pragma unroll
+        for (int i = 0; i < NV; i++) { cur[i] = nxt[i]; nxt[i] = nx2[i]; }
+    }
+}
+
+template <int NV>
+__global__ __launch_bounds__(256) void vit_assemble_ln_f16_kernel(const __half* __restrict__ patch, const __half* __restrict__ cls,
+                                                                  const __half* __restrict__ pos, const float* __restrict__ cb,
+                                                                  const __half* __restrict__ gamma, const __half* __restrict__ beta,
+                                                                  __half* __restrict__ x, __half* __restrict__ h, int rows, int P,
+                                                                  int D, float eps, int rows_per_wave) {
+    const int lane = threadIdx.x & 63, wave = (blockIdx.x * blockDim.x + threadIdx.x) >> 6;
+    const int r0 = wave * rows_per_wave;
+    if (r0 >= rows) return;
+    const LnLane<NV> ln(lane, D >> 3, cb, gamma, beta);
+    Half8 cur[NV], nxt[NV], nx2[NV], pcur[NV], pnxt[NV];
+    auto load_src = [&](int r, Half8* dst) {
+        const int b = r / (P + 1), t = r - b * (P + 1);
+        ln.load_row(t == 0 ? cls : patch + ((size_t)b * P + (t - 1)) * D, dst);
+    };
+    auto load_pos = [&](int r, Half8* dst) { ln.load_row(pos + (size_t)(r % (P + 1)) * D, dst); };
+    const int r_end = min(rows, r0 + rows_per_wave);
+    load_src(r0, cur);
+    load_pos(r0, pcur);
+    if (r0 + 1 < r_end) { load_src(r0 + 1, nxt); load_pos(r0 + 1, pnxt); }
+    const float inv_d = 1.0f / (float)D;
+    for (int r = r0; r < r_end; r++) {
+        if (r + 2 < r_end) load_src(r + 2, nx2);
 #pragma unroll
         for (int i = 0; i < NV; i++) {
             const int v = lane + 64 * i;
-            if (v < nvec) dst[i] = reinterpret_cast<const Half8*>(x + (size_t)r * D)[v];
-        }
-    };
-    auto val = [&](const Half8* row, int i, int j) -> float {
-        const float2 t = __half22float2(row[i].h[j >> 1]);
-        const float cc = j < 4 ? (&c0[i].x)[j] : (&c1[i].x)[j - 4];
-        return ((j & 1) ? t.y : t.x) + cc;
-    };
-    const int r_end = min(rows, r0 + rows_per_wave);
-    load_row(r0, cur);
-    if (r0 + 1 < r_end) load_row(r0 + 1, nxt);
+            if (v < ln.nvec) {
+#pragma unroll
+                for (int j = 0; j < 4; j++) {
+                    const float2 a = __half22float2(cur[i].h[j]), p = __half22float2(pcur[i].h[j]);
+                    cur[i].h[j] = __floats2half2_rn(a.x + p.x, a.y + p.y);
+                }
+                reinterpret_cast<Half8*>(x + (size_t)r * D)[v] = cur[i];
+            }
+        }
+#pragma unroll
+        for (int i = 0; i < NV; i++) pcur[i] = pnxt[i];
+        if (r + 2 < r_end) load_pos(r + 2, pnxt);
+        ln.normalise(cur, inv_d, eps, h + (size_t)r * D);
+#pragma unroll
+        for (int i = 0; i < NV; i++) { cur[i] = nxt[i]; nxt[i] = nx2[i]; }
+    }
+}
+
+template <int NV>
+__global__ __launch_bounds__(256) void layernorm_f32_kernel(const float* __restrict__ x, const float* __restrict__ gamma,
+                                                            const float* __restrict__ beta, float* __restrict__ y, int rows, int D,
+                                                            float eps) {
+    const int lane = threadIdx.x & 63;
+    const int r = blockIdx.x * 4 + (threadIdx.x >> 6);
+    if (r >= rows) return;
+    const int nvec = D >> 2;
+    const float4* xr = reinterpret_cast<const float4*>(x + (size_t)r * D);
+    float4 v[NV];
+#pragma unroll
+    for (int i = 0; i < NV; i++) {
+        if (lane + 64 * i < nvec) v[i] = xr[lane + 64 * i];
+    }
+    const float k = __shfl(v[0].x, 0, 64);
+    float sum = 0.0f;
+#pragma unroll
+    for (int i = 0; i < NV; i++) {
+        if (lane + 64 * i < nvec) sum += ((v[i].x - k) + (v[i].y - k)) + ((v[i].z - k) + (v[i].w - k));
+    }
+#pragma unroll
+    for (int off = 32; off > 0; off >>= 1) sum += __shfl_xor(sum, off, 64);
     const float inv_d = 1.0f / (float)D;
-    for (int r = r0; r < r_end; r++) {
-        if (r + 2 < r_end) load_row(r + 2, nx2);
-        float sum = 0.0f;
-#pragma unroll
-        for (int i = 0; i < NV; i++) {
-            if (lane + 64 * i < nvec) {
-#pragma unroll
-                for (int j = 0; j < 8; j++) sum += val(cur, i, j);
-            }
-        }
-#pragma unroll
-        for (int off = 32; off > 0; off >>= 1) sum += __shfl_xor(sum, off, 64);
-        const float mean = sum * inv_d;
-        float sq = 0.0f;
-#pragma unroll
-        for (int i = 0; i < NV; i++) {
-            if (lane + 64 * i < nvec) {
-#pragma unroll
-                for (int j = 0; j < 8; j++) {
-                    const float dlt = val(cur, i, j) - mean;
-                    sq = fmaf(dlt, dlt, sq);
-                }
-            }
-        }
-#pragma unroll
-        for (int off = 32; off > 0; off >>= 1) sq += __shfl_xor(sq, off, 64);
-        const float rstd = rsqrtf(sq * inv_d + eps);
-#pragma unroll
-        for (int i = 0; i < NV; i++) {
-            const int v = lane + 64 * i;
-            if (v < nvec) {
-                Half8 o;
-#pragma unroll
-                for (int j = 0; j < 4; j++) {
-                    const float2 g2 = __half22float2(gm[i].h[j]), b2 = __half22float2(bt[i].h[j]);
-                    o.h[j] = __floats2half2_rn((val(cur, i, 2 * j) - mean) * rstd * g2.x + b2.x,
-                                               (val(cur, i, 2 * j + 1) - mean) * rstd * g2.y + b2.y);
-                }
-                reinterpret_cast<Half8*>(y + (size_t)r * D)[v] = o;
-            }
-        }
-#pragma unroll
-        for (int i = 0; i < NV; i++) { cur[i] = nxt[i]; nxt[i] = nx2[i]; }
+    const float mean = k + sum * inv_d;
+    float sq = 0.0f;
+#pragma unroll
+    for (int i = 0; i < NV; i++) {
+        if (lane + 64 * i < nvec) {
+            const float a = v[i].x - mean, b = v[i].y - mean, c = v[i].z - mean, d = v[i].w - mean;
+            sq += (a * a + b * b) + (c * c + d * d);
+        }
+    }
+#pragma unroll
+    for (int off = 32; off > 0; off >>= 1) sq += __shfl_xor(sq, off, 64);
+    const float rstd = rsqrtf(sq * inv_d + eps);
+    float4* yr = reinterpret_cast<float4*>(y + (size_t)r * D);
+#pragma unroll
+    for (int i = 0; i < NV; i++) {
+        const int c4 = lane + 64 * i;
+        if (c4 < nvec) {
+            const float4 g = reinterpret_cast<const float4*>(gamma)[c4], bb = reinterpret_cast<const float4*>(beta)[c4];
+            float4 o;
+            o.x = (v[i].x - mean) * rstd * g.x + bb.x;
+            o.y = (v[i].y - mean) * rstd * g.y + bb.y;
+            o.z = (v[i].z - mean) * rstd * g.z + bb.z;
+            o.w = (v[i].w - mean) * rstd * g.w + bb.w;
+            yr[c4] = o;
+        }
     }
 }
 
@@ -594,3 +701,51 @@
     }
     return check_launch("layernorm_bias_f16_kernel");
 }
+
+extern "C" int vlfm_vit_assemble_ln_f16(const void* d_patch, const void* d_cls, const void* d_pos, const float* d_channel_bias,
+                                        const void* d_gamma, const void* d_beta, void* d_x, void* d_h, int batch, int patches,
+                                        int dim, float eps, void* stream) {
+    if (batch == 0) return VLFM_OK;
+    if (!d_patch || !d_cls || !d_pos || !d_gamma || !d_beta || !d_x || !d_h || batch < 0 || patches < 1 || dim <= 0 ||
+        dim % 8 != 0 || dim > 64 * 8 * LN_MAXV || (long long)batch * (patches + 1) > 0x7fffffffLL)
+        return fail(VLFM_ERR_INVALID, "vit_assemble_ln_f16: dim must be a multiple of 8 and <= 2048, patches >= 1");
+    if ((((uintptr_t)d_patch | (uintptr_t)d_cls | (uintptr_t)d_pos | (uintptr_t)d_channel_bias | (uintptr_t)d_gamma |
+          (uintptr_t)d_beta | (uintptr_t)d_x | (uintptr_t)d_h) & 15) != 0)
+        return fail(VLFM_ERR_INVALID, "vit_assemble_ln_f16: pointers must be 16-byte aligned");
+    const int rows = batch * (patches + 1);
+    const int nvec = dim / 8, nv = (nvec + 63) / 64;
+    int rpw = rows / 8192;
+    rpw = rpw < 1 ? 1 : rpw > LN_ROWS ? LN_ROWS : rpw;
+    const int waves = (rows + rpw - 1) / rpw;
+    const dim3 grid((waves + 3) / 4), block(256);
+    const __half* pt = (const __half*)d_patch; const __half* cl = (const __half*)d_cls; const __half* ps = (const __half*)d_pos;
+    const __half* g = (const __half*)d_gamma; const __half* b = (const __half*)d_beta;
+    __half* x = (__half*)d_x; __half* h = (__half*)d_h;
+    VLFM_TIMED("vit_assemble_ln_f16_kernel", stream);
+    switch (nv) {
+        case 1: VLFM_KLAUNCH(vit_assemble_ln_f16_kernel<1>, grid, block, 0, (hipStream_t)stream, pt, cl, ps, d_channel_bias, g, b, x, h, rows, patches, dim, eps, rpw); break;
+        case 2: VLFM_KLAUNCH(vit_assemble_ln_f16_kernel<2>, grid, block, 0, (hipStream_t)stream, pt, cl, ps, d_channel_bias, g, b, x, h, rows, patches, dim, eps, rpw); break;
+        case 3: VLFM_KLAUNCH(vit_assemble_ln_f16_kernel<3>, grid, block, 0, (hipStream_t)stream, pt, cl, ps, d_channel_bias, g, b, x, h, rows, patches, dim, eps, rpw); break;
+        default: VLFM_KLAUNCH(vit_assemble_ln_f16_kernel<4>, grid, block, 0, (hipStream_t)stream, pt, cl, ps, d_channel_bias, g, b, x, h, rows, patches, dim, eps, rpw); break;
+    }
+    return check_launch("vit_assemble_ln_f16_kernel");
+}
+
+extern "C" int vlfm_layernorm_f32(const float* d_x, const float* d_gamma, const float* d_beta, float* d_y, int rows, int dim, float eps,
+                                  void* stream) {
+    if (rows == 0) return VLFM_OK;
+    if (!d_x || !d_gamma || !d_beta || !d_y || rows < 0 || dim <= 0 || dim % 4 != 0 || dim > 1024)
+        return fail(VLFM_ERR_INVALID, "layernorm_f32: dim must be a multiple of 4 and <= 1024");
+    if ((((uintptr_t)d_x | (uintptr_t)d_gamma | (uintptr_t)d_beta | (uintptr_t)d_y) & 15) != 0)
+        return fail(VLFM_ERR_INVALID, "layernorm_f32: pointers must be 16-byte aligned");
+    const int nv = (dim / 4 + 63) / 64;
+    const dim3 grid((unsigned)(((long long)rows + 3) / 4)), block(256);
+    VLFM_TIMED("layernorm_f32_kernel", stream);
+    switch (nv) {
+        case 1: VLFM_KLAUNCH(layernorm_f32_kernel<1>, grid, block, 0, (hipStream_t)stream, d_x, d_gamma, d_beta, d_y, rows, dim, eps); break;
+        case 2: VLFM_KLAUNCH(layernorm_f32_kernel<2>, grid, block, 0, (hipStream_t)stream, d_x, d_gamma, d_beta, d_y, rows, dim, eps); break;
+        case 3: VLFM_KLAUNCH(layernorm_f32_kernel<3>, grid, block, 0, (hipStream_t)stream, d_x, d_gamma, d_beta, d_y, rows, dim, eps); break;
+        default: VLFM_KLAUNCH(layernorm_f32_kernel<4>, grid, block, 0, (hipStream_t)stream, d_x, d_gamma, d_beta, d_y, rows, dim, eps); break;
+    }
+    return check_launch("layernorm_f32_kernel");
+}
diff --git a/vlfm_amd/vlm/blip2itm.py b/vlfm_amd/vlm/blip2itm.py
--- a/vlfm_amd/vlm/blip2itm.py
+++ b/vlfm_amd/vlm/blip2itm.py
@@ -98,13 +98,15 @@
 
         return frozenset(n for n in self.hip_gemms if ok(layers[n]))
 
-    def forward_deferred(self, x: torch.Tensor, c_in: torch.Tensor, c_mid: torch.Tensor) -> torch.Tensor:
+    def forward_deferred(self, x: torch.Tensor, c_in: torch.Tensor, c_mid: torch.Tensor,
+                         h: Optional[torch.Tensor] = None) -> torch.Tensor:
         from . import ops
 
         b, n, d = x.shape
         hd = d // self.heads
         hip = self.hip_gemms_at(b * n)
-        h = ops.layernorm_bias(x, c_in, self.layer_norm1.weight, self.layer_norm1.bias, self.layer_norm1.eps)
+        if h is None:
+            h = ops.layernorm_bias(x, c_in, self.layer_norm1.weight, self.layer_norm1.bias, self.layer_norm1.eps)
         x2 = x.view(b * n, d)
         a = None
         if self.hip_attention and n == ops.VIT_ATTENTION_TOKENS and hd in ops.VIT_ATTENTION_HEADS:
@@ -197,6 +199,25 @@
     return y if residual is None else y + residual
 
 
+QFORMER_NATIVE_SELF_ATTENTION = True
+QFORMER_NATIVE_LAYERNORM = True
+
+
+def _qnative(x: torch.Tensor) -> bool:
+    return (x.is_cuda and x.dtype == torch.float32 and not torch.is_grad_enabled()
+            and x.numel() // x.shape[-1] >= QFORMER_SPLIT_MIN_ROWS)
+
+
+def _qlayernorm(ln: nn.LayerNorm, x: torch.Tensor) -> torch.Tensor:
+    from . import ops
+
+    if (QFORMER_NATIVE_LAYERNORM and _qnative(x) and x.is_contiguous() and ln.weight is not None and ln.bias is not None
+            and ln.weight.dtype == torch.float32 and x.shape[-1] % 4 == 0 and x.shape[-1] <= ops.LAYERNORM_F32_MAX_DIM
+            and ln.normalized_shape == (x.shape[-1],)):
+        return ops.layernorm_f32(x, ln.weight, ln.bias, ln.eps)
+    return ln(x)
+
+
 class _BertAttention(nn.Module):
     def __init__(self, hidden: int, kv_hidden: int, heads: int, eps: float):
         super().__init__()
@@ -229,7 +250,7 @@
             blocks, tokens, k_block0, v_block0 = kv_blocks
             q = _qlinear(x, self.query.weight, self.query.bias).contiguous()
             a = ops.qformer_cross_attention(q, blocks, tokens, h, k_block0, v_block0, (d // h) ** -0.5)
-            return self.LayerNorm(_qlinear(a, self.dense.weight, self.dense.bias, residual=x))
+            return _qlayernorm(self.LayerNorm, _qlinear(a, self.dense.weight, self.dense.bias, residual=x))
         if kv_proj is not None:
             q = _qlinear(x, self.query.weight, self.query.bias).view(b, n, h, d // h).transpose(1, 2)
             k = kv_proj[0].reshape(b, -1, h, d // h).transpose(1, 2)
@@ -238,7 +259,14 @@
             if self._qkv_fused is None or self._qkv_fused[0].device != x.device or self._qkv_fused[0].dtype != x.dtype:
                 self._qkv_fused = (torch.cat([self.query.weight, self.key.weight, self.value.weight]).detach(),
                                    torch.cat([self.query.bias, self.key.bias, self.value.bias]).detach())
-            qkv = _qlinear(x, *self._qkv_fused).view(b, n, 3, h, d // h).permute(2, 0, 3, 1, 4)
+            qkv = _qlinear(x, *self._qkv_fused)
+            from . import ops
+
+            if (QFORMER_NATIVE_SELF_ATTENTION and mask is None and _qnative(x) and d == h * ops.QFORMER_ATTENTION_HEAD
+                    and n <= ops.QFORMER_ATTENTION_MAX_QUERIES and qkv.is_contiguous()):
+                a = ops.qformer_self_attention(qkv.view(b * n, 3 * d), b, n, h, (d // h) ** -0.5).view(b, n, d)
+                return _qlayernorm(self.LayerNorm, _qlinear(a, self.dense.weight, self.dense.bias, residual=x))
+            qkv = qkv.view(b, n, 3, h, d // h).permute(2, 0, 3, 1, 4)
             q, k, v = qkv[0], qkv[1], qkv[2]
         else:
             q = self.query(x).view(b, n, h, d // h).transpose(1, 2)
@@ -251,8 +279,8 @@
             k = k.reshape(b, src_len, h, d // h).transpose(1, 2)
             v = v.reshape(b, src_len, h, d // h).transpose(1, 2)
         a = F.scaled_dot_product_attention(q, k, v, attn_mask=mask)
-        return self.LayerNorm(_qlinear(a.transpose(1, 2).reshape(b, n, d), self.dense.weight, self.dense.bias,
-                                       residual=x))
+        return _qlayernorm(self.LayerNorm, _qlinear(a.transpose(1, 2).reshape(b, n, d), self.dense.weight, self.dense.bias,
+                                                    residual=x))
 
 
 class _BertFFN(nn.Module):
@@ -264,7 +292,7 @@
 
     def forward(self, x: torch.Tensor) -> torch.Tensor:
         hid = _qlinear(x, self.up.weight, self.up.bias, act="gelu")
-        return self.LayerNorm(_qlinear(hid, self.down.weight, self.down.bias, residual=x))
+        return _qlayernorm(self.LayerNorm, _qlinear(hid, self.down.weight, self.down.bias, residual=x))
 
 
 class _QFormerLayer(nn.Module):
@@ -297,6 +325,7 @@
         self.text_projection = nn.Linear(c.q_hidden, c.proj_dim)
         self.deferred_bias = True
         self._deferred_c: Optional[torch.Tensor] = None
+        self.fused_entrance = True
         self.split_kv = True
         self.split_kv_min_rows = 32 * 257
         self._kv_all = None
@@ -470,14 +499,26 @@
                 .reshape(b, g * g, 3 * c.patch_size * c.patch_size)
         w = self.patch_embedding.weight
         x = F.linear(pixel_values.to(w.dtype), w.view(w.shape[0], -1), self.patch_embedding.bias)
-        x = torch.cat([self.class_embedding.expand(x.shape[0], -1, -1), x], dim=1) + self.position_embedding
-        if self.deferred_bias and x.is_cuda and x.dtype == torch.float16 and c.v_hidden % 8 == 0 and c.v_hidden <= 2048:
+        deferred = self.deferred_bias and x.is_cuda and x.dtype == torch.float16 and c.v_hidden % 8 == 0 and c.v_hidden <= 2048
+        h0 = None
+        if (deferred and self.fused_entrance and len(self.blocks) > 0 and not torch.is_grad_enabled() and x.is_contiguous()
+                and self.class_embedding.dtype == torch.float16 and self.position_embedding.dtype == torch.float16
+                and self.class_embedding.is_contiguous() and self.position_embedding.is_contiguous()
+                and self.position_embedding.shape[1] == x.shape[1] + 1):
+            from . import ops
+
+            ln = self.blocks[0].layer_norm1
+            x, h0 = ops.vit_assemble_ln(x, self.class_embedding, self.position_embedding, self._deferred_constants()[0],
+                                        ln.weight, ln.bias, ln.eps)
+        else:
+            x = torch.cat([self.class_embedding.expand(x.shape[0], -1, -1), x], dim=1) + self.position_embedding
+        if deferred:
             from . import ops
 
             c = self._deferred_constants()
             x = x.contiguous()
             for i, blk in enumerate(self.blocks):
-                x = blk.forward_deferred(x, c[2 * i], c[2 * i + 1])
+                x = blk.forward_deferred(x, c[2 * i], c[2 * i + 1], h=h0 if i == 0 else None)
             return ops.layernorm_bias(x, c[2 * len(self.blocks)], self.post_layernorm.weight, self.post_layernorm.bias,
                                       self.post_layernorm.eps)
         for blk in self.blocks:
diff --git a/vlfm_amd/vlm/ops.py b/vlfm_amd/vlm/ops.py
--- a/vlfm_amd/vlm/ops.py
+++ b/vlfm_amd/vlm/ops.py
@@ -319,6 +319,58 @@
                                                            k_block0, v_block0, kv_blocks.shape[1], float(scale), _stream()),
                "qformer_cross_attention_f32")
     return out
+
+
+def qformer_self_attention(qkv: torch.Tensor, batch: int, queries: int, heads: int, scale: float,
+                           out: Optional[torch.Tensor] = None) -> torch.Tensor:
+    assert qkv.is_cuda and qkv.dtype == torch.float32 and qkv.is_contiguous()
+    assert qkv.numel() == batch * queries * 3 * heads * 64 and 1 <= queries <= QFORMER_ATTENTION_MAX_QUERIES
+    if out is None:
+        out = torch.empty((batch * queries, heads * 64), dtype=torch.float32, device=qkv.device)
+    else:
+        assert out.dtype == torch.float32 and out.is_contiguous() and out.numel() >= batch * queries * heads * 64
+    _lib.check(_lib.lib().vlfm_qformer_self_attention_f32(qkv.data_ptr(), out.data_ptr(), batch, queries, heads, float(scale),
+                                                          _stream()), "qformer_self_attention_f32")
+    return out
+
+
+LAYERNORM_F32_MAX_DIM = 1024
+
+
+def layernorm_f32(x: torch.Tensor, weight: torch.Tensor, bias: torch.Tensor, eps: float,
+                  out: Optional[torch.Tensor] = None) -> torch.Tensor:
+    dim = x.shape[-1]
+    assert x.is_cuda and x.dtype == torch.float32 and x.is_contiguous() and dim % 4 == 0 and dim <= LAYERNORM_F32_MAX_DIM
+    assert weight.dtype == torch.float32 and bias.dtype == torch.float32 and weight.numel() == dim and bias.numel() == dim
+    assert weight.is_contiguous() and bias.is_contiguous()
+    if out is None:
+        out = torch.empty_like(x)
+    else:
+        assert out.dtype == torch.float32 and out.is_contiguous() and out.numel() >= x.numel()
+    _lib.check(_lib.lib().vlfm_layernorm_f32(x.data_ptr(), weight.data_ptr(), bias.data_ptr(), out.data_ptr(), x.numel() // dim, dim,
+                                             float(eps), _stream()), "layernorm_f32")
+    return out
+
+
+def vit_assemble_ln(patches: torch.Tensor, cls: torch.Tensor, pos: torch.Tensor, channel_bias, weight: torch.Tensor,
+                    bias: torch.Tensor, eps: float, out=None) -> Tuple[torch.Tensor, torch.Tensor]:
+    B, P, D = patches.shape
+    for t in (patches, cls, pos, weight, bias):
+        assert t.is_cuda and t.dtype == torch.float16 and t.is_contiguous()
+    assert cls.numel() == D and pos.numel() == (P + 1) * D and weight.numel() == D and bias.numel() == D
+    assert channel_bias is None or (channel_bias.dtype == torch.float32 and channel_bias.is_contiguous() and channel_bias.numel() == D)
+    if out is None:
+        x = torch.empty((B, P + 1, D), dtype=torch.float16, device=patches.device)
+        h = torch.empty_like(x)
+    else:
+        x, h = out
+        for t in (x, h):
+            assert t.dtype == torch.float16 and t.is_contiguous() and t.numel() >= B * (P + 1) * D
+    _lib.check(_lib.lib().vlfm_vit_assemble_ln_f16(patches.data_ptr(), cls.data_ptr(), pos.data_ptr(),
+                                                   channel_bias.data_ptr() if channel_bias is not None else None,
+                                                   weight.data_ptr(), bias.data_ptr(), x.data_ptr(), h.data_ptr(), B, P, D,
+                                                   float(eps), _stream()), "vit_assemble_ln_f16")
+    return x, h
 
 
 VIT_ATTENTION_TOKENS, VIT_ATTENTION_HEADS = 257, (88,)
```
